# k2kobayashi/crank

Hardware: AMD Instinct MI355X
Metric: train frames/sec (higher is better)
Workload: dtype bf16; 1 GPU; vqvae trainer step (all sub-updates), VCC2020-shaped synthetic 80-dim mlfb, 64 utterances x 500 frames per GPU, 14 speakers; trainer=vqvae, global_batch=64, batch_len=500, parallelism=dp1

## Files before the change

crank_amd/_lib.py:

```python
import ctypes
import os
from .config import cfg
from ctypes import c_char_p, c_double, c_float, c_int, c_longlong, c_ulonglong, c_void_p

_HERE = os.path.dirname(os.path.abspath(__file__))
LIB_PATH = cfg.lib_path or os.path.join(_HERE, "libcrank_hip.so")
_lib = None

ERRORS = {1: "invalid argument", 2: "HIP runtime error", 3: "unsupported shape/configuration"}


class NetDesc(ctypes.Structure):
    _fields_ = [
        ("kind", c_int), ("in_ch", c_int), ("out_ch", c_int), ("kernel_size", c_int), ("layers", c_int),
        ("stacks", c_int), ("res_ch", c_int), ("gate_ch", c_int), ("skip_ch", c_int), ("aux_ch", c_int),
        ("conv_ch", c_int), ("causal", c_int), ("use_bias", c_int), ("slope", c_float), ("dropout", c_float),
    ]


COLLATE_MAX_STREAMS = 8


class CollateStream(ctypes.Structure):
    _fields_ = [("src", c_void_p), ("ld", c_int), ("col0", c_int), ("ncols", c_int), ("dst", c_void_p)]


class CollateDesc(ctypes.Structure):
    _fields_ = [
        ("n_streams", c_int), ("streams", CollateStream * COLLATE_MAX_STREAMS), ("utt_start", c_void_p),
        ("utt_spk", c_void_p), ("n_utt", c_int), ("n_spk", c_int), ("lcf0_raw", c_void_p),
        ("spk_lcf0_mean", c_void_p), ("spk_lcf0_std", c_void_p), ("raw", c_void_p), ("raw_start", c_void_p),
        ("fftl", c_int), ("hop", c_int),
    ]


P, I, LL, ULL, F, D = c_void_p, c_int, c_longlong, c_ulonglong, c_float, c_double

SIGNATURES = {
    "crk_net_create": (P, [ctypes.POINTER(NetDesc)]),
    "crk_net_destroy": (None, [P]),
    "crk_net_param_count": (LL, [P]),
    "crk_net_conv_count": (I, [P]),
    "crk_net_conv_info": (I, [P, I, ctypes.POINTER(c_longlong)]),
    "crk_net_saved_bytes": (LL, [P, I, I]),
    "crk_net_reserve": (I, [P, I, I]),
    "crk_net_scratch_bytes": (LL, [P, I, I]),
    "crk_debug_alloc_count": (LL, []),
    "crk_debug_net_paths": (I, [P, I, I]),
    "crk_seed_next": (I, [P, P, P]),
    "crk_nets_wnorm_bwd": (I, [I, P, P]),
    "crk_nets_prepare": (I, [I, P, P, ULL, P, P]),
    "crk_net_forward": (I, [P, P, ULL, P, I, P, I, P, I, P, I, I, I, ULL, P]),
    "crk_net_backward": (I, [P, P, ULL, P, P, I, P, I, P, I, P, I, F, P, I, P, I, I, I, ULL, P]),
    "crk_net_backward_scaled": (I, [P, P, ULL, P, P, I, P, I, P, I, P, I, F, P, I, P, I, I, I, ULL, P, P, P]),
    "crk_net_embed_grad_supported": (I, [P, I, I, I]),
    "crk_net_backward_embed": (I, [P, P, ULL, P, P, I, P, I, P, I, P, I, F, P, I, I, I, ULL, P, LL, I, I, I, P, P]),
    "crk_vq_forward": (I, [P, I, P, I, I, I, P, P, I, P, I, P]),
    "crk_vq_forward_fused": (I, [P, I, P, I, P, I, P, I, I, I, P, P, I, P, I, P, P, P, P, P]),
    "crk_vq_image_bytes": (LL, [I, I]),
    "crk_vq_image_build_multi": (I, [I, P, P, I, P, P]),
    "crk_vq_ema_scratch_bytes": (LL, [I, I, I]),
    "crk_vq_ema_stats": (I, [P, I, P, I, I, I, P, P, P, P]),
    "crk_vq_ema_apply": (I, [P, P, P, P, P, I, I, D, D, P]),
    "crk_vq_ema_partial": (I, [P, I, P, I, I, I, P, P]),
    "crk_vq_ema_reduce_multi": (I, [I, P, P, P, P, P, P, P]),
    "crk_vq_ema_apply_multi": (I, [I, P, P, P, P, P, P, P, D, D, P]),
    "crk_vq_ema_partial_multi": (I, [I, P, P, P, P, P, P, P, P]),
    "crk_vq_ema_reduce_size_multi": (I, [I, P, P, P, P, P, P, P, D, D, P]),
    "crk_vq_ema_blend_multi": (I, [I, P, P, P, P, P, P, D, P]),
    "crk_vq_ema_blend_image_multi": (I, [I, P, P, P, P, P, P, D, P, P]),
    "crk_stft_loss_multi_fwd": (I, [P, I, P, I, I, I, I, I, P, P, P, P, F, P, P, P]),
    "crk_stft_loss_multi_fwd_grad": (I, [P, I, P, I, I, I, I, I, P, P, P, P, F, P, P, I, P, P]),
    "crk_stft_loss_multi_bwd": (I, [P, I, P, I, I, I, I, I, P, P, P, P, F, P, P, I, P]),
    "crk_loss_scratch_floats": (I, []),
    "crk_masked_loss_fwd": (I, [P, I, P, I, F, P, LL, I, I, P, P, P]),
    "crk_masked_loss_bwd": (I, [P, I, P, I, F, P, LL, I, I, P, P, P, I, P, I, P]),
    "crk_masked_loss_both_fwd": (I, [P, I, P, I, P, LL, I, P, P, P]),
    "crk_weighted_sum": (I, [I, P, P, F, P, P]),
    "crk_weighted_sum_bwd": (I, [I, P, P, P, P]),
    "crk_recon_supported": (I, [I, I, P, P, P]),
    "crk_stft_twiddle_floats": (LL, [I, I]),
    "crk_stft_twiddles": (I, [I, I, P, P, P]),
    "crk_recon_grad_floats": (LL, [I, I, I, I, P, P]),
    "crk_recon_loss_fwd": (I, [P, I, P, I, P, I, I, I, I, P, P, P, P, F, P, P, P, P]),
    "crk_recon_loss_bwd": (I, [P, I, P, I, P, I, I, I, I, P, P, P, P, P, P, P, P, P, I, P]),
    "crk_masked_loss_bwd_acc": (I, [P, I, P, I, F, P, LL, I, I, P, P, P, I, P, I, P, I, P, P]),
    "crk_vq_commit_bwd": (I, [P, I, P, I, P, LL, I, P, P, P, I, P, I, P, I, P, I, P, I, P]),
    "crk_ce_fwd": (I, [P, I, P, LL, I, I, P, P, P, P]),
    "crk_ce_bwd": (I, [P, LL, I, P, P, P, P]),
    "crk_stft_loss_fwd": (I, [P, I, P, I, I, I, I, I, I, I, P, F, F, I, P, P, P]),
    "crk_stft_loss_bwd": (I, [P, I, P, I, I, I, I, I, I, I, P, F, F, P, P, I, P]),
    "crk_adam_step": (I, [P, P, P, P, LL, P, P, F, F, F, I, P]),
    "crk_radam_step": (I, [P, P, P, P, LL, P, P, D, D, D, I, P]),
    "crk_lamb_step": (I, [P, P, P, P, P, P, I, P, I, P, P, P, P, D, D, D, I, P]),
    "crk_lamb_tile": (I, []),
    "crk_concat_embed": (I, [P, I, I, P, I, I, P, I, P, LL, P, I, P]),
    "crk_embed_bwd_scratch_floats": (LL, [LL, I, I]),
    "crk_embed_bwd": (I, [P, I, I, I, P, LL, I, P, P, P]),
    "crk_concat_embed_run": (I, [P, I, I, P, I, I, P, I, P, LL, LL, P, I, P]),
    "crk_embed_bwd_run": (I, [P, I, I, I, P, LL, LL, I, P, P, P]),
    "crk_logmel_fwd": (I, [P, I, I, I, I, I, I, I, P, P, I, F, P, P, P, I, I, P]),
    "crk_scaler_apply": (I, [P, I, P, I, LL, I, P, P, I, P]),
    "crk_scaler_workspace_bytes": (LL, [I, I]),
    "crk_scaler_moments": (I, [P, I, I, I, LL, P, P, I, P, LL, P]),
    "crk_scaler_merge": (I, [P, LL, I, I, P, P, P, P, I, P, P, P, P]),
    "crk_collate_batch": (I, [ctypes.POINTER(CollateDesc), P, I, I, P, P, P, P, P, P, P, P, P]),
    "crk_decode_f0": (I, [P, P, I, I, P, P, D, D, I, P, P, P, P, P, P]),
    "crk_mcd_scratch_bytes": (LL, [I, I, I, I, I]),
    "crk_mcd_fastdtw": (I, [P, P, P, P, I, I, I, I, I, P, P, P, LL, P, P, P]),
    "crk_voc_create": (P, [I, I, I, I, P, I, P]),
    "crk_voc_destroy": (None, [P]),
    "crk_voc_workspace_bytes": (LL, [P, I, I]),
    "crk_voc_forward": (I, [P, P, P, I, I, P, P, P, LL, I, P]),
    "crk_voc_upsample": (I, [P, P, P, I, I, P, P, LL, P]),
    "crk_world_create": (P, [I, I, D, D, I, I, I]),
    "crk_world_destroy": (None, [P]),
    "crk_world_reserve": (I, [P, LL]),
    "crk_world_workspace_bytes": (LL, [P, I, LL, LL]),
    "crk_world_synthesis": (I, [P, P, P, P, P, I, I, P, P, I, LL, LL, LL, P, P, P, LL, P]),
    "crk_world_frames": (I, [P, P, P, P, I, I, LL, P, P, P, LL, P]),
    "crk_world_pulses": (I, [P, P, P, P, I, P, P, P, P, P]),
    "crk_wana_create": (P, [I, I, D, D, I]),
    "crk_wana_destroy": (None, [P]),
    "crk_wana_reserve": (I, [P, LL]),
    "crk_wana_workspace_bytes": (LL, [I, LL, LL]),
    "crk_wana_lowcut": (I, [P, P, P, I, P, I, LL, P, P]),
    "crk_wana_lowcut_tile": (I, []),
    "crk_wana_cheaptrick": (I, [P, P, P, P, P, I, LL, LL, LL, P, P, LL, P]),
    "crk_wana_mcep": (I, [P, P, P, P, P, I, LL, LL, LL, I, P, P, P, LL, P]),
    "crk_wana_npow": (I, [P, P, P, I, LL, P, P, LL, P]),
    "crk_wana_frame_shapes": (I, [P, P, P, I, LL, P, P, P]),
    "crk_f0_create": (P, [I, I, P]),
    "crk_f0_destroy": (None, [P]),
    "crk_f0_reserve": (I, [P, LL]),
    "crk_f0_workspace_bytes": (LL, [I, LL, LL, LL]),
    "crk_f0_harvest": (I, [P, P, P, P, P, P, I, LL, LL, LL, LL, LL, P, P, P, LL, P]),
    "crk_f0_decimate": (I, [P, P, P, I, LL, P, P, LL, P]),
    "crk_f0_raw_candidates": (I, [P, P, P, P, P, P, I, LL, LL, LL, P, P, P, LL, P]),
    "crk_f0_candidates": (I, [P, P, P, I, LL, P, P, LL, P]),
    "crk_f0_refine": (I, [P, P, P, P, P, I, LL, P, P, P]),
    "crk_f0_contour": (I, [P, P, P, P, I, LL, P, P, LL, P]),
    "crk_f0_continuous": (I, [P, P, I, LL, P, P, P, P, P, P, P]),
    "crk_gl_create": (I, [I, I, I, I, I, P, ctypes.POINTER(c_void_p)]),
    "crk_gl_destroy": (None, [P]),
    "crk_gl_workspace_bytes": (LL, [I, LL, LL]),
    "crk_gl_linear_spectrum": (I, [P, P, LL, I, P, P]),
    "crk_gl_run": (I, [P, P, P, P, P, I, LL, LL, I, I, P, P, LL, P]),
    "crk_gl_stft": (I, [P, P, P, P, I, LL, LL, P, P]),
    "crk_gl_istft": (I, [P, P, P, P, I, LL, LL, P, P, LL, P]),
    "crk_prof_enable": (I, [I]),
    "crk_prof_report": (I, [I, ctypes.POINTER(c_longlong), ctypes.POINTER(c_double), ctypes.POINTER(c_double)]),
    "crk_prof_report_bytes": (I, [I, ctypes.POINTER(c_double)]),
    "crk_debug_vq_set_f16": (I, [I]),
    "crk_debug_flush_before": (I, [c_longlong]),
    "crk_debug_vq_flags": (I, [ctypes.POINTER(c_ulonglong), I]),
    "crk_version": (c_char_p, []),
}


def lib():
    global _lib
    if _lib is None:
        if not os.path.exists(LIB_PATH):
            raise RuntimeError(
                f"{LIB_PATH} is missing: build it with `python -c 'import __graft_entry__ as g; g.build()'` "
                "(or `make -C crank_amd/csrc`).  crank_amd has no fallback compute path."
            )
        cdll = ctypes.CDLL(LIB_PATH)
        for name, (res, args) in SIGNATURES.items():
            fn = getattr(cdll, name)
            fn.restype = res
            fn.argtypes = args
        _lib = cdll
    return _lib


def check(rc, what):
    if rc != 0:
        raise RuntimeError(f"libcrank_hip: {what} failed: {ERRORS.get(rc, rc)}")


_raw_stream = None


def stream_ptr():
    global _raw_stream
    if _raw_stream is None:
        import torch

        get_stream = getattr(torch._C, "_cuda_getCurrentRawStream", None)
        get_dev = getattr(torch._C, "_cuda_getDevice", None)
        if get_stream is not None and get_dev is not None:
            _raw_stream = lambda: get_stream(get_dev())
        else:
            _raw_stream = lambda: torch.cuda.current_stream().cuda_stream
    return _raw_stream()


def ptr(t):
    return 0 if t is None else t.data_ptr()
```

crank_amd/config.py:

```python
import contextlib
import os
import types

_get = os.environ.get


def _flag(name, default):
    v = _get(name)
    return default if v is None else v not in ("0", "")


def _read():
    return types.SimpleNamespace(
        precision=_get("CRANK_AMD_PRECISION", "bf16"),
        lib_path=_get("CRANK_AMD_LIB") or None,
        default_yaml=_get("CRANK_DEFAULT_YAML") or None,
        overlap_c=int(_get("CRANK_AMD_OVERLAP_C", "1") or 0),
        separate_ce=_flag("CRANK_AMD_SEPARATE_CE", False),
        separate_commit=_flag("CRANK_AMD_SEPARATE_COMMIT", False),
        recon_dense=_flag("CRANK_AMD_RECON_DENSE", False),
        stft_two_pass=_flag("CRANK_AMD_STFT_TWO_PASS", False),
        cond_sums=_flag("CRANK_AMD_COND_SUMS", True),
        force_dist=_flag("CRANK_AMD_FORCE_DIST", False),
        dist_backend=_get("CRANK_AMD_DIST_BACKEND") or None,
        dp_graph_collectives=_flag("CRANK_AMD_DP_GRAPH_COLLECTIVES", True),
        capture_mode=_get("CRANK_AMD_CAPTURE_MODE", "thread_local"),
        test_refuse_capture_rank=_get("CRANK_AMD_TEST_REFUSE_CAPTURE_RANK"),
    )


cfg = _read()


def reload():
    cfg.__dict__.update(_read().__dict__)


def torchrun():
    r = _get("RANK")
    return (None if r is None else int(r)), int(_get("LOCAL_RANK", "0")), int(_get("WORLD_SIZE", "1"))


@contextlib.contextmanager
def override(**kw):
    unknown = [k for k in kw if not hasattr(cfg, k)]
    if unknown:
        raise AttributeError(f"unknown switch(es): {unknown}")
    old = {k: getattr(cfg, k) for k in kw}
    cfg.__dict__.update(kw)
    try:
        yield cfg
    finally:
        cfg.__dict__.update(old)
```

crank_amd/csrc/conv_kernels.h:

```cpp
#pragma once
#include <vector>

#include "common.h"
#include "switches.h"

#define CRK_TM 128

enum { MODE_PLAIN = 0, MODE_RESFWD = 1, MODE_BWDA = 2 };

struct ConvP {
  const float* xa; int lda; int cinA; float scaleA;
  const float* xb; int ldb; int cinB; float scaleB;
  int act_in; float slope;
  float drop_p; unsigned long long drop_seed;
  const unsigned long long* drop_seed_ptr;
  int cin, cin_pad;
  const float* xc; int ldc; int cinC; int cinC_pad;
  const uint16_t* w_hi; const uint16_t* w_lo;
  const uint16_t* wc_hi; const uint16_t* wc_lo;
  const uint16_t* w2_hi; const uint16_t* w2_lo;
  const float* bias; const float* bias2a; const float* bias2b;
  int cout, cout_pad, ktaps, dil, off0;
  int B, T, tiles_per_utt;
  float* y; int ldy; int accumulate; int act_out; float out_scale;
  const float* dmask; int ldm; int dmask_act;
  const float* res; int ldr; float res_scale;
  float epi_drop_p; unsigned long long epi_drop_seed;
  float* skip; int skip_init; float* sv_ta; float* sv_sb; float* sv_z;
  const float* ta; const float* sb;
  int xs_stride, cs_stride, ws_stride, zs_stride;
  int o_xlo, o_chi, o_clo, o_whi, o_wlo, o_zhi, o_zlo;
  int lds_bytes;
  int dbg;
};

struct WgradP {
  const float* a1; int lda1; int ca1; float sa1;
  const float* a2; int lda2; int ca2; float sa2;
  int ca, ca_pad;
  const float* x; int ldx; int cx; int cx_pad; float sx; int act_in; float slope;
  float drop_p; unsigned long long drop_seed; const unsigned long long* drop_seed_ptr;
  const float* xc; int ldc; int cc; int cc_pad; int has_aux;
  int ktaps, dil, off0;
  int B, T;
  float* partial;
  float* partial_aux;
  float* bias_partial;
  int grp_tap0, grp_ntap, grp_aux;
  int cpg, ngroups;
  int dbg;
};

struct ConvEntry {
  int cout, cin, k;
  long long off_g, off_v, off_b;
  long long fw_off; int fw_rows, fw_kp, fw_row0;
  long long bw_off; int bw_rows, bw_kp, bw_col0;
  long long pt_off; int pt_rows, pt_row0, pt_cx, pt_taps, pt_tap0; float pt_scale;
  int pt_groups;
  long long pb_off;
  long long norm_off;
  long long fr_off; int fr_mode;
  long long bfr_off; int bfr_mode;
};

struct StackLayer {
  long long f_conv, f_aux, f_os;
  long long w_conv, w_aux, w_os;
  long long b_conv, b_out, b_skip;
  int dil, off0;
};
struct StackP {
  const float* x0;
  const float* c; int ldc; int aux_ch, aux_pad;
  float* saved;
  uint16_t *xb_hi, *xb_lo;
  uint16_t *zb_hi, *zb_lo;
  uint16_t *tb_hi, *tb_lo, *sg_hi, *sg_lo;
  uint16_t *cb_hi, *cb_lo;
  float* skip;
  const float* params;
  const uint16_t* whi; const uint16_t* wlo;
  const StackLayer* layers;
  int B, T, L, ktaps;
  int hl, hr, max_off;
  int tmo, tiles_per_utt;
  float drop_p; unsigned long long drop_seed; const unsigned long long* drop_seed_ptr;
  int o_xlo, o_zhi, o_zlo, o_chi, o_clo, o_whi, o_wlo, o_bias, o_tab, w_bytes, lds_bytes;
  int nw;
  int dbg;
  int ft, fh;
  int ft1;
  int o_zs, o_cs;
  int o_xf;
  const float* x_in; int ldx_in, in_ch, kp_first;
  long long f_first, b_first;
  long long f_h1, b_h1, f_h2, b_h2;
  float* y; int ldy, out_ch; float head_scale;
  uint16_t* fin_hi; uint16_t* head_hi;
  long long ts_stride;
  int cs_stride;
};
struct PsLayer {
  long long w_off;
  long long b_off;
  int rows, rows_pad;
  int kp;
  int k, dil, off0;
  int epi;
  int mask_w;
  long long mask_plane;
  long long save_plane;
  long long f_off;
};
struct PsP {
  const float* x; int ldx, cin; float in_scale; int in_act;
  float* y; int ldy; float out_scale;
  const float* params; const uint16_t *whi, *wlo;
  uint16_t *save_hi, *save_lo;
  const uint16_t* mask_hi;
  const PsLayer* layers; int L;
  int tail;
  int B, T; float slope;
  int hl, hr, tmo, tiles_per_utt, nw, os;
  int o_olo, o_whi, o_wlo, o_bias, o_tab, w_bytes, lds_bytes;
  double algo_bytes;
  int os_b;
  const float* in_num; const float* in_den;
  long long l0_f_off, l0_save_plane; int l0_k, l0_kp, l0_rows_pad;
};
struct PwLayer {
  long long a_hi, a_lo;
  long long b_hi, b_lo;
  int wa, wb;
  int ca, cb;
  int k, dil, off0;
  long long pt, pb;
};
#define CRK_MAX_NETS_PW 8
struct PwP {
  const PwLayer* layers;
  const uint16_t* abase;
  const uint16_t* bbase;
  float* partials;
  int B, T, cpg, G;
};
struct PwMP { PwP q[CRK_MAX_NETS_PW]; int first[CRK_MAX_NETS_PW + 1]; int n; };
int launch_pstack_wgrad_multi(const PwMP& m, int total_layers, int max_G, int max_wa, int max_wb, int max_tiles, double flops,
                              double bytes, hipStream_t s);
int pstack_wgrad_supported(int ca, int cb, int wa, int wb, int k, int dil);
int launch_pstack_wgrad(const PwP& p, int nlayers, int max_wa, int max_wb, bool precise, double flops, hipStream_t s, int max_tiles = 0);
int pstack_plan(PsP& p, const PsLayer* host_layers, bool precise);
int launch_pstack(const PsP& p, bool precise, double flops, hipStream_t s);
int pstack2_plan(PsP& p, const PsLayer* host_layers);
int launch_pstack2(const PsP& p, double flops, hipStream_t s);
int pstack2x_plan(PsP& p, const PsLayer* host_layers);
int launch_pstack2x(const PsP& p, double flops, hipStream_t s);

struct StackBLayer {
  long long w_os, w_conv, w_aux;
  int dil, off0;
  long long f_os, f_conv, f_aux;
};
struct StackBP {
  const float* dS;
  const float* saved;
  const uint16_t *tb_hi, *tb_lo, *sg_hi, *sg_lo;
  float* dX0;
  uint16_t *gb_hi, *gb_lo;
  uint16_t *dxb_hi, *dxb_lo;
  uint16_t *dsb_hi, *dsb_lo;
  float* dc; int lddc; int aux_ch;
  const uint16_t* whi; const uint16_t* wlo;
  const StackBLayer* layers;
  int B, T, L, ktaps;
  int hl, hr, max_off;
  int tmo, tiles_per_utt;
  float drop_p; unsigned long long drop_seed; const unsigned long long* drop_seed_ptr;
  int mask_l0; float slope;
  int o_glo, o_whi, o_wlo, w_bytes, lds_bytes, nw;
  const float* dy; int lddy, out_ch, kp_y;
  long long w_h2, w_h1, w_first;
  const uint16_t* hmask_hi;
  uint16_t* hb_hi;
  float head_scale;
  float* dx; int lddx, in_ch, in_rows; float dx_scale;
  long long f_h2, f_h1, f_first;
  int ft, o_dx, o_tab;
  long long ts_stride;
  int rec;
  int dbg;
};
struct StackWLayer {
  long long pt_conv, pb_conv, pt_os, pb_os, pt_aux;
  int dil, off0;
};
struct StackWP {
  const uint16_t *xb_hi, *xb_lo, *zb_hi, *zb_lo, *cb_hi, *cb_lo;
  const uint16_t *gb_hi, *gb_lo, *dxb_hi, *dxb_lo, *dsb_hi, *dsb_lo;
  const StackWLayer* layers;
  float* partials;
  int B, T, L, ktaps, aux_ch, aux_pad, cpg, G;
  int rec_g;
  float* usums; int nseg;
};
int stack_wgrad_supported(int ktaps, int max_dil, int aux_ch);
int launch_stack_wgrad(const StackWP& p, bool precise, hipStream_t s);
struct CondEmbedP {
  const float* usums; int nseg, cpg;
  const uint16_t *whi, *wlo;
  const StackBLayer* layers;
  const long long* idx; long long run;
  int B, T, L, c0, E, n_rows;
  float* dtable;
};
int launch_cond_embed_bwd(const CondEmbedP& p, hipStream_t s);
int stack_bwd_plan(StackBP& p, bool precise);
int stack2_bwd_plan(StackBP& p);
int launch_stack2_bwd(const StackBP& p, hipStream_t s);
int stack_bwd_waves(bool precise);
int launch_stack_bwd(const StackBP& p, bool precise, hipStream_t s);
int stack_fwd_plan(StackP& p, bool precise);
int launch_stack_fwd(const StackP& p, bool precise, hipStream_t s);
int stack2_fwd_plan(StackP& p);
int launch_stack2_fwd(const StackP& p, hipStream_t s);
int stack2x_fwd_plan(StackP& p);
int launch_stack2x_fwd(const StackP& p, hipStream_t s);
#define CRK_PROF_CLASSES 9
void conv_prof_begin(int cls, double flops, hipStream_t s);
void conv_prof_end(int cls, hipStream_t s);
void conv_prof_bytes(int cls, double bytes);

void conv_fill_lds(ConvP& p, int mode, bool precise);
int launch_conv(const ConvP& p, int mode, bool precise, hipStream_t s);
int wgrad_expand(const WgradP& job, bool precise, std::vector<WgradP>& out);
int launch_wgrad_table(const WgradP* d_jobs, const std::vector<WgradP>& h_jobs, int B, int T, int max_groups, bool precise,
                       hipStream_t s);
#define CRK_MAX_NETS 8
struct NetRef {
  const ConvEntry* ents; const float* params; float* grads; const float* partials; float* norms;
  uint16_t *whi, *wlo;
  int n_ents, first;
};
struct NetRefs { NetRef r[CRK_MAX_NETS]; int n; float* bump; };
int launch_weight_prep_multi(const NetRefs& R, int total_entries, int nmax, hipStream_t s);
int launch_step_bump(float* step, hipStream_t s);
int launch_wnorm_bwd_multi(const NetRefs& R, int total_entries, hipStream_t s);
int launch_weight_prep(const ConvEntry* d_entries, int n_entries, int nmax, const float* params, uint16_t* wprep_hi,
                       uint16_t* wprep_lo, float* norms, hipStream_t s);
int launch_wnorm_bwd(const ConvEntry* d_entries, int n_entries, const float* params, float* grads,
                     const float* partials, const float* norms, hipStream_t s);
int conv_kernels_init();
```

crank_amd/csrc/conv_kernels.hip:

```cpp
#include "conv_kernels.h"

#include <vector>

static inline int al16(int x) { return (x + 15) & ~15; }

static int sw_int(const char* name, int dflt) { const char* e = getenv(name); return e ? atoi(e) : dflt; }
const CrkSwitches& crk_sw() {
  static const CrkSwitches s = [] {
    CrkSwitches v;
    v.sk_v = sw_int("CRK_SK_V", 2); v.skb_v = sw_int("CRK_SKB_V", 2); v.ps_v = sw_int("CRK_PS_V", 2);
    v.no_fuse = sw_int("CRK_NO_FUSE", 0); v.s2x = sw_int("CRK_S2X", 1); v.disc_split = sw_int("CRK_DISC_SPLIT", 1);
    v.s2_cfg = sw_int("CRK_S2_CFG", 0);
    const int nw = sw_int("CRK_SK_NW", 0);
    v.sk_nw_fwd = nw > 10 ? nw / 10 : nw; v.sk_nw_bwd = nw > 10 ? nw % 10 : nw;
    v.ps_nw = sw_int("CRK_PS_NW", 0);
    v.wg_groups = sw_int("CRK_WG_GROUPS", 32); if (v.wg_groups < 1) v.wg_groups = 32;
    v.wg_cpg = sw_int("CRK_WG_CPG", 0); v.wg_fill = sw_int("CRK_WG_FILL", 1) != 0;
    v.vq_f16 = sw_int("CRK_VQ_F16", 1) != 0; v.vq_lc = sw_int("CRK_VQ_LC", 2); v.logmel_wave = sw_int("CRK_LOGMEL_WAVE", 1);
    return v;
  }();
  return s;
}

struct ProfClass {
// ... 570 lines not shown
    const int l = wgrad_entry_lds(e, precise);
    if (l > lds) lds = l;
    fl += 2.0 * (double)B * T * e.ca * (e.grp_aux ? (double)e.cc : (double)e.cx * e.grp_ntap);
  }
  static bool attr_set = false;
  if (!attr_set) {
    if (hipFuncSetAttribute((const void*)wgrad_kernel<true>, hipFuncAttributeMaxDynamicSharedMemorySize, 152 * 1024) != hipSuccess ||
        hipFuncSetAttribute((const void*)wgrad_kernel<false>, hipFuncAttributeMaxDynamicSharedMemorySize, 152 * 1024) != hipSuccess)
      return CRK_ERR_HIP;
    attr_set = true;
  }
  dim3 grid(max_groups, (unsigned)h_jobs.size()), block(256);
  prof_begin(3, fl, s);
  if (precise) hipLaunchKernelGGL(wgrad_kernel<true>, grid, block, lds, s, d_jobs, B, T);
  else hipLaunchKernelGGL(wgrad_kernel<false>, grid, block, lds, s, d_jobs, B, T);
  prof_end(3, s);
  CRK_CHECK_LAUNCH();
  return CRK_OK;
}

__device__ __forceinline__ float wave_sum(float v) {
#pragma unroll
  for (int o = 32; o > 0; o >>= 1) v += __shfl_xor(v, o, 64);
  return v;
}

#define WP_BAND 16
typedef unsigned wp_u32x4 __attribute__((ext_vector_type(4)));
template <int BAND = WP_BAND>
__device__ __forceinline__ void weight_prep_band(const ConvEntry& e, int band, const float* params, uint16_t* whi,
                                                 uint16_t* wlo, float* norms, unsigned* ws) {
  const int co0 = band * BAND;
  if (co0 >= e.cout) return;
  const int nrow = e.cout - co0 < BAND ? e.cout - co0 : BAND;
  const int k = e.k, cin = e.cin, n = cin * k;
  const int tid = threadIdx.x, lane = tid & 63, wave = tid >> 6;
  {
    const float* v0 = params + e.off_v + (long long)co0 * n;
    const int tot = nrow * n;
    constexpr int WPQ = 28;
    for (int i0 = 0; i0 < tot; i0 += 256 * WPQ) {
      float t[WPQ];
#pragma unroll
      for (int u = 0; u < WPQ; u++) { const int i = i0 + u * 256 + tid; t[u] = i < tot ? v0[i] : 0.f; }
#pragma unroll
      for (int u = 0; u < WPQ; u++) { const int i = i0 + u * 256 + tid; if (i < tot) ws[i] = __builtin_bit_cast(unsigned, t[u]); }
    }
  }
  float gv[BAND / 4];
#pragma unroll
  for (int q = 0; q < BAND / 4; q++) { const int r = wave + 4 * q; gv[q] = r < nrow ? params[e.off_g + co0 + r] : 0.f; }
  __syncthreads();
#pragma unroll
  for (int q = 0; q < BAND / 4; q++) {
    const int r = wave + 4 * q;
    if (r < nrow) {
      unsigned* row = ws + r * n;
      float ss = 0.f;
      for (int i = lane; i < n; i += 64) { const float x = __builtin_bit_cast(float, row[i]); ss += x * x; }
      ss = wave_sum(ss);
      const float nrm = sqrtf(ss);
      if (lane == 0) norms[e.norm_off + co0 + r] = nrm;
      const float sc = gv[q] / nrm;
      for (int i = lane; i < n; i += 64) {
        const float w = __builtin_bit_cast(float, row[i]) * sc;
        uint16_t h, l;
        split_bf(w, h, l);
        row[i] = (unsigned)h | ((unsigned)l << 16);
      }
    }
  }
  __syncthreads();
  {
    const int nc8 = e.fw_kp >> 3, per_tap = nrow * nc8, total = k * per_tap;
    const float i_pt = 1.f / (float)per_tap, i_nc = 1.f / (float)nc8;
    for (int pidx = tid; pidx < total; pidx += 256) {
      const int tap = (int)(((float)pidx + 0.5f) * i_pt), rem = pidx - tap * per_tap;
      const int r = (int)(((float)rem + 0.5f) * i_nc), c8 = rem - r * nc8;
      const int co = co0 + r, ci0 = c8 * 8;
      unsigned wv[8];
#pragma unroll
      for (int j = 0; j < 8; j++) wv[j] = ci0 + j < cin ? ws[r * n + (ci0 + j) * k + tap] : 0u;
      const wp_u32x4 hp = {(wv[0] & 0xffffu) | (wv[1] << 16), (wv[2] & 0xffffu) | (wv[3] << 16), (wv[4] & 0xffffu) | (wv[5] << 16),
                           (wv[6] & 0xffffu) | (wv[7] << 16)};
      const wp_u32x4 lp = {(wv[0] >> 16) | (wv[1] & 0xffff0000u), (wv[2] >> 16) | (wv[3] & 0xffff0000u),
                           (wv[4] >> 16) | (wv[5] & 0xffff0000u), (wv[6] >> 16) | (wv[7] & 0xffff0000u)};
      const long long fi = e.fw_off + ((long long)tap * e.fw_rows + e.fw_row0 + co) * e.fw_kp + ci0;
      *reinterpret_cast<wp_u32x4*>(whi + fi) = hp;
      *reinterpret_cast<wp_u32x4*>(wlo + fi) = lp;
      if (e.fr_mode) {
        const int kc = ci0 >> 4, lh = 32 * ((ci0 & 15) >> 3);
        long long fo;
        if (e.fr_mode == 6) fo = ((((long long)(co >> 5) * k + tap) * (e.fw_kp >> 4) + kc) * 64 + (co & 31) + lh) * 8;
        else if (e.fr_mode == 5) fo = ((((long long)tap * (e.fw_rows >> 5) + (co >> 5)) * (e.fw_kp >> 4) + kc) * 64 + (co & 31) + lh) * 8;
        else {
          int mt, row;
          if (e.fr_mode <= 2) { const int hc = co & 63; mt = hc >> 4; row = (hc & 15) + (co >= 64 ? 16 : 0); }
          else { mt = (co >> 5) + (e.fr_mode == 4 ? 2 : 0); row = co & 31; }
          const int tp = e.fr_mode == 1 ? tap : 0;
          fo = ((((long long)tp * 4 + mt) * 4 + kc) * 64 + row + lh) * 8;
        }
        *reinterpret_cast<wp_u32x4*>(whi + e.fr_off + fo) = hp;
        *reinterpret_cast<wp_u32x4*>(wlo + e.fr_off + fo) = lp;
      }
    }
  }
  if (e.bw_off >= 0) {
    const int ext = ((e.cout + 15) & ~15) - co0;
    const int no8 = ((co0 + BAND >= e.cout) ? ext : (ext < BAND ? ext : BAND)) >> 3;
    const int per_tap = cin * no8, total = k * per_tap;
    const float i_pt = 1.f / (float)per_tap, i_no = 1.f / (float)no8;
    for (int pidx = tid; pidx < total; pidx += 256) {
      const int tap = (int)(((float)pidx + 0.5f) * i_pt), rem = pidx - tap * per_tap;
      const int ci = (int)(((float)rem + 0.5f) * i_no), o8 = rem - ci * no8;
      unsigned wv[8];
#pragma unroll
      for (int j = 0; j < 8; j++) wv[j] = o8 * 8 + j < nrow ? ws[(o8 * 8 + j) * n + ci * k + tap] : 0u;
      const wp_u32x4 hp = {(wv[0] & 0xffffu) | (wv[1] << 16), (wv[2] & 0xffffu) | (wv[3] << 16), (wv[4] & 0xffffu) | (wv[5] << 16),
                           (wv[6] & 0xffffu) | (wv[7] << 16)};
      const wp_u32x4 lp = {(wv[0] >> 16) | (wv[1] & 0xffff0000u), (wv[2] >> 16) | (wv[3] & 0xffff0000u),
                           (wv[4] >> 16) | (wv[5] & 0xffff0000u), (wv[6] >> 16) | (wv[7] & 0xffff0000u)};
      const int kcol = e.bw_col0 + co0 + o8 * 8, tf = k - 1 - tap;
      const long long bi = e.bw_off + ((long long)tf * e.bw_rows + ci) * e.bw_kp + kcol;
      *reinterpret_cast<wp_u32x4*>(whi + bi) = hp;
      *reinterpret_cast<wp_u32x4*>(wlo + bi) = lp;
      if (e.bfr_off >= 0) {
        const int ln = (ci & 31) + 32 * ((kcol & 15) >> 3);
        const long long fo = e.bfr_mode == 1
            ? ((((long long)(ci >> 5) * k + tf) * (e.bw_kp >> 4) + (kcol >> 4)) * 64 + ln) * 8
            : ((((long long)tf * (e.bw_rows >> 5) + (ci >> 5)) * (e.bw_kp >> 4) + (kcol >> 4)) * 64 + ln) * 8;
        *reinterpret_cast<wp_u32x4*>(whi + e.bfr_off + fo) = hp;
      }
    }
  }
}

__global__ __launch_bounds__(256) void weight_prep_kernel(const ConvEntry* ents, const float* params, uint16_t* whi,
                                                          uint16_t* wlo, float* norms) {
  extern __shared__ unsigned wp_ws[];
  const ConvEntry e = ents[blockIdx.x];
  weight_prep_band(e, blockIdx.y, params, whi, wlo, norms, wp_ws);
}

__device__ __forceinline__ int net_of_block(const NetRefs& R, int bx) {
  int r = 0;
  while (r + 1 < R.n && bx >= R.r[r + 1].first) r++;
  return r;
}
template <int BAND>
__global__ __launch_bounds__(256) void weight_prep_multi_kernel(const NetRefs R) {
  extern __shared__ unsigned wp_ws[];
  const NetRef& q = R.r[net_of_block(R, blockIdx.x)];
  const ConvEntry e = q.ents[blockIdx.x - q.first];
  if (R.bump && blockIdx.x == 0 && blockIdx.y == 0 && threadIdx.x == 0) R.bump[0] += 1.f;
  weight_prep_band<BAND>(e, blockIdx.y, q.params, q.whi, q.wlo, q.norms, wp_ws);
}
__global__ void step_bump_kernel(float* step) { step[0] += 1.f; }
int launch_step_bump(float* step, hipStream_t s) {
  hipLaunchKernelGGL(step_bump_kernel, dim3(1), dim3(1), 0, s, step);
  CRK_CHECK_LAUNCH();
  return CRK_OK;
}
static int wp_set_lds(const void* fn, size_t lds) {
  if (lds > 64 * 1024 && hipFuncSetAttribute(fn, hipFuncAttributeMaxDynamicSharedMemorySize, 160 * 1024) != hipSuccess) return CRK_ERR_HIP;
  return CRK_OK;
}
int launch_weight_prep_multi(const NetRefs& R, int total_entries, int nmax, hipStream_t s) {
  const size_t lds = (size_t)WP_BAND * nmax * 4;
  if (lds > 160 * 1024) return CRK_ERR_UNSUPPORTED;
  if (total_entries <= 16) {
    if (wp_set_lds((const void*)weight_prep_multi_kernel<8>, lds / 2) != CRK_OK) return CRK_ERR_HIP;
    hipLaunchKernelGGL(weight_prep_multi_kernel<8>, dim3(total_entries, 128 / 8), dim3(256), lds / 2, s, R);
    CRK_CHECK_LAUNCH();
    return CRK_OK;
  }
  if (wp_set_lds((const void*)weight_prep_multi_kernel<WP_BAND>, lds) != CRK_OK) return CRK_ERR_HIP;
  hipLaunchKernelGGL(weight_prep_multi_kernel<WP_BAND>, dim3(total_entries, 128 / WP_BAND), dim3(256), lds, s, R);
  CRK_CHECK_LAUNCH();
  return CRK_OK;
}

int launch_weight_prep(const ConvEntry* d_entries, int n_entries, int nmax, const float* params, uint16_t* wprep_hi,
                       uint16_t* wprep_lo, float* norms, hipStream_t s) {
  const size_t lds = (size_t)WP_BAND * nmax * 4;
  if (lds > 160 * 1024) return CRK_ERR_UNSUPPORTED;
  if (wp_set_lds((const void*)weight_prep_kernel, lds) != CRK_OK) return CRK_ERR_HIP;
  dim3 grid(n_entries, 128 / WP_BAND), block(256);
  hipLaunchKernelGGL(weight_prep_kernel, grid, block, lds, s, d_entries, params, wprep_hi, wprep_lo, norms);
  CRK_CHECK_LAUNCH();
  return CRK_OK;
}

#ifndef WN_RB
#define WN_RB 8
#endif
#ifndef WN_IF
#define WN_IF 16
#endif
template <int RB> struct WnormShared { float dw[RB][128 * 8]; };
template <int RB, int IF>
__device__ __forceinline__ void wnorm_bwd_body(const ConvEntry& e, int band, const float* params, float* grads,
                                               const float* partials, const float* norms, WnormShared<RB>& sh) {
  const int co0 = band * RB;
  if (co0 >= e.cout) return;
  const int nrow = e.cout - co0 < RB ? e.cout - co0 : RB;
  const int G = e.pt_groups, k = e.k, cin = e.cin, cx = e.pt_cx;
  const int n = cin * k;
  const int tid = threadIdx.x;
  const long long gstride = (long long)e.pt_taps * e.pt_rows * e.pt_cx;
  const long long tstride = (long long)e.pt_rows * e.pt_cx;
  const float* base = partials + e.pt_off + (long long)(e.pt_row0 + co0) * cx;
  const int r = tid >> 5, l32 = tid & 31;
  const bool on = r < nrow;
  const int co = co0 + r;
  const float* __restrict__ v = params + e.off_v + (long long)co * n;
  float* __restrict__ gv = grads + e.off_v + (long long)co * n;
  constexpr int WN_PV = (128 * 8) / 32;
  float vr[WN_PV], go[WN_PV];
#pragma unroll
  for (int q = 0; q < WN_PV; q++) {
    const int i = l32 + 32 * q;
    const bool ok = on && i < n;
    vr[q] = ok ? v[i] : 0.f;
    go[q] = ok ? gv[i] : 0.f;
  }
  float sb = 0.f;
  if (on && e.off_b >= 0)
    for (int g = l32; g < e.pt_groups; g += 32) sb += partials[e.pb_off + (long long)g * e.pt_rows + e.pt_row0 + co];
  const float nrm = on ? norms[e.norm_off + co] : 1.f;
  const float gval = on ? params[e.off_g + co] : 0.f;
  const float g_old = (on && l32 == 0) ? grads[e.off_g + co] : 0.f;
  const float b_old = (on && l32 == 0 && e.off_b >= 0) ? grads[e.off_b + co] : 0.f;
  const int run = nrow * cx;
  if ((cx & 3) == 0 && ((((uintptr_t)base) & 15) == 0) && ((gstride | tstride) & 3) == 0) {
    const int run4 = run >> 2;
    for (int it = tid; it < k * run4; it += 256) {
      const int tap = it / run4, i4 = it - tap * run4;
      const float* src = base + tap * tstride + 4 * i4;
      f32x4 s4 = {0.f, 0.f, 0.f, 0.f};
      int g = 0;
      for (; g + IF <= G; g += IF) {
        f32x4 t[IF];
#pragma unroll
        for (int u = 0; u < IF; u++) t[u] = *reinterpret_cast<const f32x4*>(src + (long long)(g + u) * gstride);
#pragma unroll
        for (int u = 0; u < IF; u++) s4 += t[u];
      }
      if (IF > 16) {
        for (; g + 16 <= G; g += 16) {
          f32x4 t[16];
#pragma unroll
          for (int u = 0; u < 16; u++) t[u] = *reinterpret_cast<const f32x4*>(src + (long long)(g + u) * gstride);
#pragma unroll
          for (int u = 0; u < 16; u++) s4 += t[u];
        }
      }
      for (; g + 4 <= G; g += 4) {
        f32x4 t[4];
#pragma unroll
        for (int u = 0; u < 4; u++) t[u] = *reinterpret_cast<const f32x4*>(src + (long long)(g + u) * gstride);
#pragma unroll
        for (int u = 0; u < 4; u++) s4 += t[u];
      }
      for (; g < G; g++) s4 += *reinterpret_cast<const f32x4*>(src + (long long)g * gstride);
      const int r = (4 * i4) / cx, ci = 4 * i4 - r * cx;
#pragma unroll
      for (int j = 0; j < 4; j++) sh.dw[r][(ci + j) * k + tap] = s4[j] * e.pt_scale;
    }
  } else {
    for (int tap = 0; tap < k; tap++) {
      for (int i = tid; i < run; i += 256) {
        const float* src = base + tap * tstride + i;
        float sv = 0.f;
        int g = 0;
        for (; g + 8 <= G; g += 8) {
          float t[8];
#pragma unroll
          for (int u = 0; u < 8; u++) t[u] = src[(long long)(g + u) * gstride];
#pragma unroll
          for (int u = 0; u < 8; u++) sv += t[u];
        }
        for (; g < G; g++) sv += src[(long long)g * gstride];
        const int r = i / cx, ci = i - r * cx;
        sh.dw[r][ci * k + tap] = sv * e.pt_scale;
      }
    }
  }
  __syncthreads();
  float dot = 0.f;
#pragma unroll
  for (int q = 0; q < WN_PV; q++) {
    const int i = l32 + 32 * q;
    if (on && i < n) dot += sh.dw[r][i] * vr[q];
  }
#pragma unroll
  for (int o = 16; o > 0; o >>= 1) { dot += __shfl_xor(dot, o, 64); sb += __shfl_xor(sb, o, 64); }
  if (on) {
    const float inv = 1.f / nrm;
    if (l32 == 0) {
      grads[e.off_g + co] = g_old + dot * inv;
      if (e.off_b >= 0) grads[e.off_b + co] = b_old + sb * e.pt_scale;
    }
    const float c1 = gval * inv, c2 = dot * inv * inv;
#pragma unroll
    for (int q = 0; q < WN_PV; q++) {
      const int i = l32 + 32 * q;
      if (i < n) gv[i] = go[q] + c1 * (sh.dw[r][i] - c2 * vr[q]);
    }
  }
}

__global__ __launch_bounds__(256) void wnorm_bwd_kernel(const ConvEntry* ents, const float* params, float* grads,
// ... 29 lines not shown
```

crank_amd/csrc/loss_kernels.hip:

```cpp
#include <algorithm>
#include <type_traits>

#include "common.h"

__device__ __forceinline__ float block_sum_256(float v, float* sh) {
#pragma unroll
  for (int o = 32; o > 0; o >>= 1) v += __shfl_xor(v, o, 64);
  const int tid = threadIdx.x;
  __syncthreads();
  if ((tid & 63) == 0) sh[tid >> 6] = v;
  __syncthreads();
  return sh[0] + sh[1] + sh[2] + sh[3];
}

template <int NC>
__device__ __forceinline__ void sum_partials(const float* part, int stride, int n, float (&s)[NC], float* sh) {
#pragma unroll
  for (int j = 0; j < NC; j++) s[j] = 0.f;
  for (int i = threadIdx.x; i < n; i += 256) {
#pragma unroll
    for (int j = 0; j < NC; j++) s[j] += part[stride * i + j];
  }
#pragma unroll
  for (int j = 0; j < NC; j++) s[j] = block_sum_256(s[j], sh);
// ... 913 lines not shown
  CRK_CHECK_LAUNCH();
  return CRK_OK;
}

struct ReconBRes { const float* gc; int hop, lo, span, nf; };
struct ReconBP {
  const float* x; const float* y; const unsigned char* mask;
  int ldx, ldy, T, D, nres;
  long N;
  const float* stat; const float* g1; const float* g2; const float* g3;
  float* dx; int lddx;
  ReconBRes r[LOSS_MAX_RES];
};
template <int V>
__global__ __launch_bounds__(256) void recon_bwd_kernel(const ReconBP p) {
  const float g1 = p.g1 ? p.g1[0] / p.stat[1] : 0.f;
  const float g2 = p.g2 ? p.g2[0] / p.stat[3] : 0.f;
  const float g3 = p.g3 ? p.g3[0] : 0.f;
  const int DV = p.D / V;
  const long total = p.N * DV;
  for (long i = (long)blockIdx.x * 256 + threadIdx.x; i < total; i += (long)gridDim.x * 256) {
    const long n = i / DV;
    const int d = (int)(i - n * DV) * V;
    const int b = (int)(n / p.T), t = (int)(n - (long)b * p.T);
    float v[V];
#pragma unroll
    for (int j = 0; j < V; j++) v[j] = 0.f;
    if (p.g3) {
#pragma unroll
      for (int k = 0; k < LOSS_MAX_RES; k++) {
        if (k >= p.nres) break;
        const ReconBRes& r = p.r[k];
        const int u = t + r.lo, fr = u / r.hop, off = u - fr * r.hop;
        if (off < r.span && fr < r.nf) {
          const float* gp = r.gc + ((size_t)((long)b * r.nf + fr) * r.span + off) * p.D + d;
          if (V == 4) {
            const float4 a = *reinterpret_cast<const float4*>(gp);
            v[0] += a.x * g3; v[1 % V] += a.y * g3; v[2 % V] += a.z * g3; v[3 % V] += a.w * g3;
          } else {
            v[0] += gp[0] * g3;
          }
        }
      }
    }
    if (!p.mask || p.mask[n]) {
      float xv[V], yv[V];
      if (V == 4) {
        const float4 a = *reinterpret_cast<const float4*>(p.x + n * p.ldx + d);
        const float4 c = *reinterpret_cast<const float4*>(p.y + n * p.ldy + d);
        xv[0] = a.x; xv[1 % V] = a.y; xv[2 % V] = a.z; xv[3 % V] = a.w;
        yv[0] = c.x; yv[1 % V] = c.y; yv[2 % V] = c.z; yv[3 % V] = c.w;
      } else {
        xv[0] = p.x[n * p.ldx + d]; yv[0] = p.y[n * p.ldy + d];
      }
#pragma unroll
      for (int j = 0; j < V; j++) {
        const float df = xv[j] - yv[j];
        if (p.g1) v[j] += df > 0.f ? g1 : (df < 0.f ? -g1 : 0.f);
        if (p.g2) v[j] += 2.f * df * g2;
      }
    }
    if (V == 4) *reinterpret_cast<float4*>(p.dx + n * p.lddx + d) = make_float4(v[0], v[1 % V], v[2 % V], v[3 % V]);
    else p.dx[n * p.lddx + d] = v[0];
  }
}

extern "C" int crk_recon_loss_bwd(const float* x, int ldx, const float* y, int ldy, const unsigned char* mask, int B, int T,
                                  int D, int nres, const int* n_fft, const int* hop_length, const int* win_length,
                                  const float* out5, const float* grad, const float* g1, const float* g2, const float* g3,
                                  float* dx, int lddx, void* stream) {
  if (!x || !y || !out5 || !dx || B < 1 || T < 1 || D < 1) return CRK_ERR_ARG;
  if (g3 && (!grad || !crk_recon_supported(T, nres, n_fft, hop_length, win_length))) return CRK_ERR_ARG;
  ReconBP p;
  p.x = x; p.y = y; p.mask = mask; p.ldx = ldx; p.ldy = ldy; p.T = T; p.D = D; p.nres = g3 ? nres : 0;
  p.N = (long)B * T; p.stat = out5; p.g1 = g1; p.g2 = g2; p.g3 = g3; p.dx = dx; p.lddx = lddx;
  const float* g = grad;
  for (int r = 0; r < p.nres; r++) {
    ReconBRes& q = p.r[r];
    q.hop = hop_length[r]; q.span = win_length[r] + RC_SPAN_EXTRA; q.nf = 1 + T / q.hop;
    q.lo = n_fft[r] / 2 - (n_fft[r] - win_length[r]) / 2 + 1;
    q.gc = g;
    g += (size_t)B * q.nf * q.span * D;
  }
  const bool v4 = !((((uintptr_t)x) | ((uintptr_t)y) | ((uintptr_t)dx) | ((uintptr_t)grad)) & 15) && !((D | ldx | ldy | lddx) & 3);
  if (v4) hipLaunchKernelGGL(recon_bwd_kernel<4>, dim3(loss_blocks(p.N * (D / 4))), dim3(256), 0, (hipStream_t)stream, p);
  else hipLaunchKernelGGL(recon_bwd_kernel<1>, dim3(loss_blocks(p.N * D)), dim3(256), 0, (hipStream_t)stream, p);
  CRK_CHECK_LAUNCH();
  return CRK_OK;
}

#define WS_MAX 16
struct WsumP { const float* t[WS_MAX]; float w[WS_MAX]; int n; float c; float* out; const float* g; };
__global__ void weighted_sum_kernel(const WsumP p) {
  float s = 0.f;
#pragma unroll
  for (int i = 0; i < WS_MAX; i++)
    if (i < p.n) s += p.w[i] * p.t[i][0];
  p.out[0] = s + p.c;
}
__global__ void weighted_sum_bwd_kernel(const WsumP p) {
  const float g = p.g[0];
#pragma unroll
  for (int i = 0; i < WS_MAX; i++)
    if (i < p.n) p.out[i] = p.w[i] * g;
}
extern "C" int crk_weighted_sum(int n, const float* const* terms, const float* weights, float constant, float* out, void* stream) {
  if (n < 1 || n > WS_MAX || !terms || !weights || !out) return CRK_ERR_ARG;
  WsumP p{};
  for (int i = 0; i < n; i++) { if (!terms[i]) return CRK_ERR_ARG; p.t[i] = terms[i]; p.w[i] = weights[i]; }
  p.n = n; p.c = constant; p.out = out;
  hipLaunchKernelGGL(weighted_sum_kernel, dim3(1), dim3(1), 0, (hipStream_t)stream, p);
  CRK_CHECK_LAUNCH();
  return CRK_OK;
}
extern "C" int crk_weighted_sum_bwd(int n, const float* weights, const float* gout, float* grads, void* stream) {
  if (n < 1 || n > WS_MAX || !weights || !gout || !grads) return CRK_ERR_ARG;
  WsumP p{};
  for (int i = 0; i < n; i++) p.w[i] = weights[i];
  p.n = n; p.g = gout; p.out = grads;
  hipLaunchKernelGGL(weighted_sum_bwd_kernel, dim3(1), dim3(1), 0, (hipStream_t)stream, p);
  CRK_CHECK_LAUNCH();
  return CRK_OK;
}

template <bool CLEAR>
__global__ __launch_bounds__(256) void adam_kernel(float* __restrict__ p, float* __restrict__ g,
                                                   float* __restrict__ m, float* __restrict__ v, long n,
                                                   const float* __restrict__ lr_dev, float* __restrict__ step_dev,
                                                   float beta1, float beta2, float eps) {
  const AdamCoef c = adam_coef(lr_dev, step_dev, beta1, beta2, eps);
  for (long i = (long)blockIdx.x * 256 + threadIdx.x; i < n; i += (long)gridDim.x * 256) adam_elem<CLEAR>(p, g, m, v, i, c);
}

__global__ void adam_bump_kernel(float* step_dev) { step_dev[0] += 1.f; }

extern "C" int crk_adam_step(float* params, float* grads, float* exp_avg, float* exp_avg_sq, long long n,
                             const float* lr_dev, float* step_dev, float beta1, float beta2, float eps, int clear_grads,
                             void* stream) {
  if (!params || !grads || !exp_avg || !exp_avg_sq || !lr_dev || !step_dev) return CRK_ERR_ARG;
  hipStream_t s = (hipStream_t)stream;
  long b = (n + 255) / 256;
  if (b > 2048) b = 2048;
  if (clear_grads & 1)
    hipLaunchKernelGGL(adam_kernel<true>, dim3((int)b), dim3(256), 0, s, params, grads, exp_avg, exp_avg_sq, (long)n, lr_dev,
                       step_dev, beta1, beta2, eps);
  else
    hipLaunchKernelGGL(adam_kernel<false>, dim3((int)b), dim3(256), 0, s, params, grads, exp_avg, exp_avg_sq, (long)n, lr_dev,
                       step_dev, beta1, beta2, eps);
  if (!(clear_grads & 2)) hipLaunchKernelGGL(adam_bump_kernel, dim3(1), dim3(1), 0, s, step_dev);
  CRK_CHECK_LAUNCH();
  return CRK_OK;
}

struct RAdamCoef { float step_size; bool rect; };
__device__ __forceinline__ RAdamCoef radam_coef(const float* lr_dev, const float* step_dev, double b1, double b2) {
  const double t = (double)step_dev[0] + 1.0;
  const double b2t = pow(b2, t), bc1 = 1.0 - pow(b1, t);
  const double nmax = 2.0 / (1.0 - b2) - 1.0;
  const double nsma = nmax - 2.0 * t * b2t / (1.0 - b2t);
  RAdamCoef c;
  c.rect = nsma >= 5.0;
  const double lr = (double)lr_dev[0];
  c.step_size = (float)(c.rect ? lr * sqrt((1.0 - b2t) * (nsma - 4.0) / (nmax - 4.0) * (nsma - 2.0) / nsma * nmax / (nmax - 2.0)) / bc1
                               : lr / bc1);
  return c;
}
struct MomentCoef { float b1, omb1, b2, omb2, eps; };
static MomentCoef moment_coef(double beta1, double beta2, double eps) {
  MomentCoef k;
  k.b1 = (float)beta1; k.omb1 = (float)(1.0 - beta1); k.b2 = (float)beta2; k.omb2 = (float)(1.0 - beta2); k.eps = (float)eps;
  return k;
}
template <bool CLEAR>
__global__ __launch_bounds__(256) void radam_kernel(float* __restrict__ p, float* __restrict__ g, float* __restrict__ m,
                                                    float* __restrict__ v, long n, const float* __restrict__ lr_dev,
                                                    float* __restrict__ step_dev, double beta1, double beta2, MomentCoef k) {
#pragma clang fp contract(off)
  const RAdamCoef c = radam_coef(lr_dev, step_dev, beta1, beta2);
  for (long i = (long)blockIdx.x * 256 + threadIdx.x; i < n; i += (long)gridDim.x * 256) {
    const float gi = g[i];
    if (CLEAR) g[i] = 0.f;
    const float vi = v[i] * k.b2 + k.omb2 * gi * gi;
    const float mi = m[i] * k.b1 + k.omb1 * gi;
    v[i] = vi; m[i] = mi;
    if (c.rect) p[i] -= c.step_size * (mi / (sqrtf(vi) + k.eps));
    else p[i] -= c.step_size * mi;
  }
}

extern "C" int crk_radam_step(float* params, float* grads, float* exp_avg, float* exp_avg_sq, long long n,
                              const float* lr_dev, float* step_dev, double beta1, double beta2, double eps, int clear_grads,
                              void* stream) {
  if (!params || !grads || !exp_avg || !exp_avg_sq || !lr_dev || !step_dev) return CRK_ERR_ARG;
  hipStream_t s = (hipStream_t)stream;
  long b = (n + 255) / 256;
  if (b > 2048) b = 2048;
  if (b < 1) b = 1;
  const MomentCoef k = moment_coef(beta1, beta2, eps);
  if (clear_grads & 1)
    hipLaunchKernelGGL(radam_kernel<true>, dim3((int)b), dim3(256), 0, s, params, grads, exp_avg, exp_avg_sq, (long)n, lr_dev,
                       step_dev, beta1, beta2, k);
  else
    hipLaunchKernelGGL(radam_kernel<false>, dim3((int)b), dim3(256), 0, s, params, grads, exp_avg, exp_avg_sq, (long)n, lr_dev,
                       step_dev, beta1, beta2, k);
  if (!(clear_grads & 2)) hipLaunchKernelGGL(adam_bump_kernel, dim3(1), dim3(1), 0, s, step_dev);
  CRK_CHECK_LAUNCH();
  return CRK_OK;
}

#define LAMB_TILE 2048
__global__ __launch_bounds__(256) void lamb_moments_kernel(const float* __restrict__ p, float* __restrict__ g,
                                                           float* __restrict__ m, float* __restrict__ v,
                                                           float* __restrict__ upd, const int4* __restrict__ tiles,
                                                           float* __restrict__ part, MomentCoef k, int clear) {
#pragma clang fp contract(off)
  __shared__ float sh[4];
  const int4 tl = tiles[blockIdx.x];
  float sw = 0.f, su = 0.f;
  for (int j = threadIdx.x; j < tl.y; j += 256) {
    const long i = (long)tl.x + j;
    const float gi = g[i];
    if (clear) g[i] = 0.f;
    const float mi = m[i] * k.b1 + k.omb1 * gi;
    const float vi = v[i] * k.b2 + k.omb2 * gi * gi;
    m[i] = mi; v[i] = vi;
    const float u = mi / (sqrtf(vi) + k.eps);
    upd[i] = u;
    const float w = p[i];
    sw += w * w; su += u * u;
  }
  sw = block_sum_256(sw, sh);
  su = block_sum_256(su, sh);
  if (threadIdx.x == 0) { part[2 * blockIdx.x] = sw; part[2 * blockIdx.x + 1] = su; }
}

__global__ __launch_bounds__(256) void lamb_apply_kernel(float* __restrict__ p, const float* __restrict__ upd,
                                                         const int4* __restrict__ tiles, const int2* __restrict__ tensors,
                                                         const float* __restrict__ part, const float* __restrict__ lr_dev,
                                                         float* __restrict__ ratio_out) {
#pragma clang fp contract(off)
  __shared__ float sr;
  const int4 tl = tiles[blockIdx.x];
  if (threadIdx.x == 0) {
    const int2 ts = tensors[tl.z];
    double sw = 0.0, su = 0.0;
    for (int t = ts.x; t < ts.x + ts.y; t++) { sw += (double)part[2 * t]; su += (double)part[2 * t + 1]; }
    const float wn = fminf((float)sqrt(sw), 10.f), un = (float)sqrt(su);
    const float r = (wn == 0.f || un == 0.f) ? 1.f : wn / un;
    sr = r;
    if (ratio_out && blockIdx.x == ts.x) ratio_out[tl.z] = r;
  }
  __syncthreads();
  const float sc = lr_dev[0] * sr;
  for (int j = threadIdx.x; j < tl.y; j += 256) {
    const long i = (long)tl.x + j;
    p[i] -= sc * upd[i];
  }
}

extern "C" int crk_lamb_step(float* params, float* grads, float* exp_avg, float* exp_avg_sq, float* upd, const int* tiles,
                             int n_tiles, const int* tensors, int n_tensors, float* part, float* ratio_out,
                             const float* lr_dev, float* step_dev, double beta1, double beta2, double eps, int clear_grads,
                             void* stream) {
  if (!params || !grads || !exp_avg || !exp_avg_sq || !upd || !tiles || !tensors || !part || !lr_dev || !step_dev ||
      n_tiles < 0 || n_tensors < 0)
    return CRK_ERR_ARG;
  hipStream_t s = (hipStream_t)stream;
  if (n_tiles > 0) {
    hipLaunchKernelGGL(lamb_moments_kernel, dim3(n_tiles), dim3(256), 0, s, params, grads, exp_avg, exp_avg_sq, upd,
                       reinterpret_cast<const int4*>(tiles), part, moment_coef(beta1, beta2, eps), clear_grads & 1);
    hipLaunchKernelGGL(lamb_apply_kernel, dim3(n_tiles), dim3(256), 0, s, params, upd, reinterpret_cast<const int4*>(tiles),
                       reinterpret_cast<const int2*>(tensors), part, lr_dev, ratio_out);
  }
  if (!(clear_grads & 2)) hipLaunchKernelGGL(adam_bump_kernel, dim3(1), dim3(1), 0, s, step_dev);
  CRK_CHECK_LAUNCH();
  return CRK_OK;
}
extern "C" int crk_lamb_tile() { return LAMB_TILE; }

__global__ __launch_bounds__(256) void concat_embed_kernel(const float* __restrict__ a, int lda, int ca,
                                                           const float* __restrict__ b2, int ldb, int cb2,
                                                           const float* __restrict__ table, int E,
                                                           const long long* __restrict__ idx, long run, long N,
                                                           float* __restrict__ out, int ldo) {
  const int C = ca + cb2 + E;
  const long total = N * C;
  for (long i = (long)blockIdx.x * 256 + threadIdx.x; i < total; i += (long)gridDim.x * 256) {
    const long n = i / C;
    const int c = (int)(i - n * C);
    float v;
    if (c < ca) v = a[n * lda + c];
    else if (c < ca + cb2) v = b2[n * ldb + (c - ca)];
    else v = table[idx[run > 1 ? n - n % run : n] * E + (c - ca - cb2)];
    out[n * ldo + c] = v;
  }
}

extern "C" int crk_concat_embed_run(const float* a, int lda, int ca, const float* b, int ldb, int cb, const float* table,
                                    int E, const long long* idx, long long run, long long N, float* out, int ldo,
                                    void* stream) {
  if (!out || run < 1 || (ca > 0 && !a) || (cb > 0 && !b) || (E > 0 && (!table || !idx))) return CRK_ERR_ARG;
  const long total = N * (ca + cb + E);
  hipLaunchKernelGGL(concat_embed_kernel, dim3(loss_blocks(total)), dim3(256), 0, (hipStream_t)stream, a, lda, ca, b, ldb,
                     cb, table, E, idx, (long)run, (long)N, out, ldo);
  CRK_CHECK_LAUNCH();
  return CRK_OK;
// ... 91 lines not shown
```

crank_amd/csrc/net.hip:

```cpp
#include <math.h>
#include <stdlib.h>
#include <string.h>

#include <deque>
#include <vector>

#include "conv_kernels.h"

struct crk_net_desc {
  int kind;
  int in_ch, out_ch, kernel_size, layers, stacks;
  int res_ch, gate_ch, skip_ch, aux_ch;
  int conv_ch;
  int causal;
  int use_bias;
  float slope;
  float dropout;
};

enum { ROLE_FIRST = 0, ROLE_CONV = 1, ROLE_AUX = 2, ROLE_OUT = 3, ROLE_SKIP = 4, ROLE_LAST1 = 5, ROLE_LAST2 = 6, ROLE_PLAIN = 7 };

struct ConvMeta {
  int role, layer, dilation;
};
// ... 782 lines not shown
    p.sv_ta = a.saved + lay.ta + l * P; p.sv_sb = a.saved + lay.sb + l * P; p.sv_z = a.saved + lay.z + l * P;
    RUN(conv_go(p, MODE_RESFWD, k.precise, a.s));
  }
  ConvP h1 = conv_fw(n, a.B, a.T, n->ents[n->idx_last1], a.params, SKIP, 64, H1, 64);
  h1.scaleA = (float)sqrt(1.0 / L); h1.act_in = head_act;
  RUN(conv_go(h1, MODE_PLAIN, k.precise, a.s));
  ConvP h2 = conv_fw(n, a.B, a.T, n->ents[n->idx_last2], a.params, H1, 64, a.y, a.ldy);
  h2.act_in = head_act;
  return conv_go(h2, MODE_PLAIN, k.precise, a.s);
}
extern "C" int crk_net_forward(void* h, const float* params, unsigned long long version, const float* x, int ldx,
                               const float* c, int ldc, float* y, int ldy, float* saved, int B, int T, int flags,
                               unsigned long long seed, void* stream) {
  Net* n = (Net*)h;
  if (!n || !params || !x || !y || B <= 0 || T <= 0) return CRK_ERR_ARG;
  const FwdIo a = {.params = params, .x = x, .ldx = ldx, .c = c, .ldc = ldc, .y = y, .ldy = ldy, .saved = saved, .B = B, .T = T,
                   .s = (hipStream_t)stream};
  const Call k = call_facts(flags, seed, true, x, ldx, y, ldy, nullptr, nullptr);
  const Shape* r = find_shape(n, B, T);
  if (!r) return not_reserved("crk_net_forward");
  const Route& rt = r->route[k.precise];
  const bool x3f = k.mode == 2 && r->route[0].x3f;
  RUN(ensure_prepared(n, params, version, a.s));
  tag_forward(n, saved, B, T, k, x3f);
  if (n->d.kind != 2 && (!saved || (n->d.aux_ch > 0 && !c))) return CRK_ERR_ARG;
  int form;
  RUN(fwd_form(n, rt, k, x3f, &form));
  switch (form) {
    case FWD_CHAIN: return fwd_chain(n, r, k, a);
    case FWD_CHAIN_LAYERS: return fwd_chain_layers(n, k, a);
    case FWD_FOLDED: return fwd_folded(n, rt, k, a, x3f);
    case FWD_FUSED: return fwd_fused(n, r, k, a);
  }
  return fwd_layers(n, k, a);
}

static int stack_cpg(const Net* n, int B, int T) {
  const int ncpu = (T + 63) / 64;
  const int groups = crk_sw().wg_groups;
  const int gsz = (B + groups - 1) / groups;
  int cpg = gsz * ncpu;
  if (crk_sw().wg_fill && n->d.kind != 2 && n->L > 0 && 256 / n->L > groups) {
    const int fill = 256 / n->L;
    const int c = (B * ncpu + fill - 1) / fill;
    if (c >= 1 && c < cpg) cpg = c;
  }
  return cpg < 1 ? 1 : cpg;
}
static int stack_groups(const Net* n, int B, int T) {
  const int total = B * ((T + 63) / 64), cpg = stack_cpg(n, B, T);
  return (total + cpg - 1) / cpg;
}

static int usum_nseg(const Net* n, int B, int T) {
  const int ncpu = (T + 63) / 64;
  return (stack_cpg(n, B, T) + 2 * ncpu - 2) / ncpu;
}
static long long usum_floats(const Net* n, int B, int T) {
  if (n->d.kind == 2 || n->d.aux_ch <= 0) return 0;
  return (long long)stack_groups(n, B, T) * usum_nseg(n, B, T) * n->L * 128;
}
static long long usum_off(const Net* n, long long N) { return gated_f32(n, N).scratch_total + (gated_s16(n, N).total + 1) / 2; }
static ShapeNeed shape_need(const Net* n, int B, int T) {
  ShapeNeed q;
  const long long N = (long long)B * T;
  const long long cw = n->d.conv_ch > n->d.out_ch ? n->d.conv_ch : n->d.out_ch;
  q.need_s = n->d.kind == 2 ? (long long)n->L * N * cw + N * plain_gplanes_w(n)
                            : usum_off(n, N) + usum_floats(n, B, T);
  q.Gs = stack_groups(n, B, T); q.cpg_s = stack_cpg(n, B, T); q.nseg = usum_nseg(n, B, T);
  const int total_chunks = B * ((T + 63) / 64);
  const int groups = (n->d.kind == 2 && n->ents.size() <= 4) ? 64 : 32;
  q.cpg = (total_chunks + groups - 1) / groups;
  if (crk_sw().wg_cpg > 0) q.cpg = crk_sw().wg_cpg;
  q.Gg = (total_chunks + q.cpg - 1) / q.cpg;
  q.need_p = n->pt_floats_stack * q.Gs + n->pt_floats_gen * q.Gg;
  return q;
}
static int grow(Net* n, float** buf, long long* cap, long long need) {
  if (need <= *cap) return CRK_OK;
  if (*buf) n->retired.push_back(*buf);
  *buf = nullptr; *cap = 0;
  if (NET_MALLOC(buf, need * 4) != hipSuccess) return CRK_ERR_HIP;
  *cap = need;
  return CRK_OK;
}
static int build_shape(Net* n, Shape& r) {
  const crk_net_desc& d = n->d;
  r.abs = n->ents;
  for (auto& e : r.abs) {
    const bool stack = e.pt_groups != 0;
    const long long base = stack ? 0 : n->pt_floats_stack * r.q.Gs;
    const int G = stack ? r.q.Gs : r.q.Gg;
    e.pt_off = base + e.pt_off * G; e.pb_off = base + e.pb_off * G; e.pt_groups = G;
  }
  RUN(upload(&r.d_ents, r.abs.data(), r.abs.size()));
  if (n->L <= PS_MAXL) {
    ps_build(n, (long long)r.B * r.T, r.abs.data(), r.ps);
    RUN(upload(&r.d_ps, &r.ps.t[0][0], 4 * PS_MAXL));
    RUN(upload(&r.d_pw, r.ps.w, PS_MAXL));
  }
  if (d.kind != 2) {
    std::vector<StackWLayer> wt(n->L);
    for (int l = 0; l < n->L; l++) {
      const ConvEntry& ec = n->ents[n->idx_conv[l]];
      const ConvEntry& eo = n->ents[n->idx_out[l]];
      const ConvEntry& ac = r.abs[n->idx_conv[l]];
      const ConvEntry& ao = r.abs[n->idx_out[l]];
      StackWLayer& y = wt[l];
      y.pt_conv = ac.pt_off; y.pb_conv = ec.off_b >= 0 ? ac.pb_off : -1;
      y.pt_os = ao.pt_off; y.pb_os = eo.off_b >= 0 ? ao.pb_off : -1;
      y.pt_aux = d.aux_ch > 0 ? r.abs[n->idx_aux[l]].pt_off : 0;
      y.dil = n->meta[n->idx_conv[l]].dilation;
      y.off0 = fwd_off0(n, ec.k, y.dil);
    }
    RUN(upload(&r.d_wlayers, wt.data(), wt.size()));
  }
  return CRK_OK;
}
extern "C" int crk_net_reserve(void* h, int B, int T) {
  Net* n = (Net*)h;
  if (!n || B <= 0 || T <= 0) return CRK_ERR_ARG;
  if (find_shape(n, B, T)) return CRK_OK;
  AllocScope may_allocate;
  Shape r{};
  r.B = B; r.T = T; r.q = shape_need(n, B, T);
  r.route[0] = route_of(n, B, T, false);
  r.route[1] = route_of(n, B, T, true);
  RUN(grow(n, &n->scratch, &n->scratch_cap, r.q.need_s));
  RUN(grow(n, &n->partials, &n->partial_cap, r.q.need_p));
  if (!n->d_jobs && NET_MALLOC(&n->d_jobs, sizeof(WgradP) * 256) != hipSuccess) return CRK_ERR_HIP;
  const int rc = build_shape(n, r);
  if (rc != CRK_OK) {
    free_shape(r);
    return rc;
  }
  n->shapes.push_back(r);
  return CRK_OK;
}
extern "C" long long crk_net_scratch_bytes(void* h, int B, int T) {
  Net* n = (Net*)h;
  if (!n || B <= 0 || T <= 0) return -1;
  const ShapeNeed q = shape_need(n, B, T);
  return (q.need_s + q.need_p) * 4;
}
extern "C" long long crk_debug_alloc_count(void) { return g_net_allocs; }
long long crk_count_alloc_(void) { return ++g_net_allocs; }
extern "C" int crk_debug_net_paths(void* h, int B, int T) {
  Net* n = (Net*)h;
  if (!n || B <= 0 || T <= 0) return -1;
  const Route r = route_at(n, B, T, false);
  return (int)r.gen_split | (int)r.x3f << 1 | (int)r.disc_split << 2 | (int)(n->d.kind == 2 && r.fused) << 3;
}

static WgradP base_wgrad(const Net* n, int B, int T) {
  WgradP w;
  memset(&w, 0, sizeof(w));
  w.sa1 = w.sa2 = w.sx = 1.f; w.slope = n->d.slope;
  w.B = B; w.T = T; w.ktaps = 1; w.dil = 1; w.off0 = 0;
  w.dbg = 0;
  return w;
}
static void wgrad_slots(const Net* n, const Shape* r, int ei, WgradP& w) {
  const ConvEntry& a = r->abs[ei];
  const bool stack = n->ents[ei].pt_groups != 0;
  w.partial = n->partials + a.pt_off;
  w.bias_partial = a.off_b >= 0 ? n->partials + a.pb_off : nullptr;
  w.ngroups = a.pt_groups;
  w.cpg = stack ? r->q.cpg_s : r->q.cpg;
}
static int wgrad_go(Net* n, WgradP& w, bool precise) {
  w.ca_pad = pad32(w.ca); w.cx_pad = pad32(w.cx); w.cc_pad = w.has_aux ? pad32(w.cc) : 0;
  return wgrad_expand(w, precise, n->jobs);
}
static int wgrad_conv(Net* n, const Shape* r, int ei, const float* a1, int lda1, const float* x, int ldx, int act_in, float sx, bool precise) {
  const ConvEntry& e = n->ents[ei];
  WgradP w = base_wgrad(n, r->B, r->T);
  w.a1 = a1; w.lda1 = lda1; w.ca1 = e.cout; w.ca = e.cout;
  w.x = x; w.ldx = ldx; w.cx = e.cin; w.sx = sx; w.act_in = act_in;
  w.ktaps = e.k; w.dil = n->meta[ei].dilation; w.off0 = -((e.k - 1) / 2) * w.dil;
  wgrad_slots(n, r, ei, w);
  return wgrad_go(n, w, precise);
}
static int wgrad_flush(Net* n, int B, int T, bool precise, hipStream_t s) {
  if (n->jobs.empty()) return CRK_OK;
  if (n->jobs.size() > 256) return CRK_ERR_UNSUPPORTED;
  const int k = n->slot_next;
  n->slot_next = (k + 1) & 3;
  if (!n->h_slot[k]) {
    if (hipHostMalloc((void**)&n->h_slot[k], sizeof(WgradP) * 256, hipHostMallocDefault) != hipSuccess) return CRK_ERR_HIP;
    if (hipEventCreateWithFlags(&n->slot_ev[k], hipEventDisableTiming) != hipSuccess) return CRK_ERR_HIP;
  } else if (hipEventSynchronize(n->slot_ev[k]) != hipSuccess) {
    return CRK_ERR_HIP;
  }
  memcpy(n->h_slot[k], n->jobs.data(), sizeof(WgradP) * n->jobs.size());
  if (hipMemcpyAsync(n->d_jobs, n->h_slot[k], sizeof(WgradP) * n->jobs.size(), hipMemcpyHostToDevice, s) != hipSuccess)
    return CRK_ERR_HIP;
  if (hipEventRecord(n->slot_ev[k], s) != hipSuccess) return CRK_ERR_HIP;
  int mg = 0;
  for (const auto& j : n->jobs) if (j.ngroups > mg) mg = j.ngroups;
  int rc = launch_wgrad_table(n->d_jobs, n->jobs, B, T, mg, precise, s);
  n->jobs.clear();
  return rc;
}

static PwP plain_wgrad_params(const Net* n, const Shape* r, const uint16_t* abase, const uint16_t* bbase) {
  PwP wp; memset(&wp, 0, sizeof(wp));
  wp.layers = r->d_pw; wp.abase = abase; wp.bbase = bbase; wp.partials = n->partials;
  wp.B = r->B; wp.T = r->T; wp.cpg = r->q.cpg; wp.G = r->q.Gg;
  return wp;
}
static int launch_plain_wgrad(const Shape* r, const PwP& wp, bool precise, hipStream_t s) {
  const PsTables& Tb = r->ps;
  return launch_pstack_wgrad(wp, Tb.nw, Tb.max_wa, Tb.max_wb, precise, Tb.wflops_per_frame * r->B * r->T, s, Tb.max_tiles);
}
static int flush_pending_plain_wgrad(Net* n, hipStream_t s) {
  if (!n->pw_shape) return CRK_OK;
  const Shape* r = n->pw_shape;
  n->pw_shape = nullptr;
  return launch_plain_wgrad(r, n->pw_params, false, s);
}

struct CondEmbed { const long long* idx; long long run; int c0, E, n_rows; float* dtable; };
struct BwdIo {
  const float* params; float* grads; const float* x; int ldx; const float* c; int ldc; const float* dy; int lddy;
  float* dx; int lddx; float dx_scale; float* dc; int lddc; const float* saved; int B, T;
  const float* dy_num; const float* dy_den; const CondEmbed* ce; hipStream_t s;
};
enum { BWD_CHAIN, BWD_CHAIN_LAYERS, BWD_FOLDED_SPLIT, BWD_FOLDED, BWD_FUSED_SPLIT, BWD_FUSED, BWD_LAYERS };
static int bwd_form(const Net* n, const Route& rt, const Call& k, bool planes_precise, int* form) {
  if (n->d.kind == 2) { *form = rt.fused ? BWD_CHAIN : BWD_CHAIN_LAYERS; return CRK_OK; }
  if (!rt.fused) { *form = BWD_LAYERS; return CRK_OK; }
  const bool ok_x = k.out16 && (!k.want_dx || n->d.in_ch % 4 == 0);
  if (rt.gen_split && !planes_precise) {
    if (!k.in4 || !ok_x) {
      fprintf(stderr, "[crank_hip] crk_net_backward: dy / dx must be 16-byte aligned with row strides that are multiples of 4 floats\n");
      return CRK_ERR_ARG;
    }
    *form = BWD_FOLDED_SPLIT;
  } else if (rt.disc_split && !planes_precise) *form = BWD_FUSED_SPLIT;
  else *form = (rt.fold_bwd_fs && k.in16 && ok_x) ? BWD_FOLDED : BWD_FUSED;
  return CRK_OK;
}

static int bwd_chain(Net* n, const Shape* r, const Call& k, const BwdIo& a) {
  if (!a.saved) return CRK_ERR_ARG;
  const crk_net_desc& d = n->d;
  const PsTables& Tb = r->ps;
  const long long N = (long long)a.B * a.T;
  const long long cw = d.conv_ch > d.out_ch ? d.conv_ch : d.out_ch;
  const uint16_t* f16 = reinterpret_cast<const uint16_t*>(a.saved + saved_f32_floats(n, N));
  uint16_t* g16 = reinterpret_cast<uint16_t*>(n->scratch + (long long)n->L * N * cw);
  PsP p = ps_base(n, a.B, a.T, a.params);
  p.x = a.dy; p.ldx = a.lddy; p.cin = d.out_ch; p.y = a.dx; p.ldy = a.lddx; p.out_scale = a.dx_scale;
  p.in_num = a.dy_num; p.in_den = a.dy_den;
  p.save_hi = g16; p.save_lo = g16 + N * plain_gplanes_w(n); p.mask_hi = f16;
  p.layers = r->d_ps + PS_MAXL; p.L = Tb.L[1];
  if (!k.want_dx && p.L >= 2) { p.L -= 1; p.tail = 1; }
  if (r->route[k.precise].ps_bwd[p.tail] == CHAIN_PS2) {
    RUN(pstack2_plan(p, Tb.t[1]));
    RUN(launch_pstack2(p, ps_flops(Tb.t[1], p.L, N), a.s));
  } else RUN(pstack_go(r, 1, p, k.precise, a.s));
  if (k.want_w) RUN(launch_plain_wgrad(r, plain_wgrad_params(n, r, g16, f16), k.precise, a.s));
  return CRK_OK;
}
static int bwd_chain_layers(Net* n, const Shape* r, const Call& k, const BwdIo& a) {
  const crk_net_desc& d = n->d;
  const long long N = (long long)a.B * a.T;
  const long long cw = d.conv_ch > d.out_ch ? d.conv_ch : d.out_ch;
  const float* dcur = a.dy; int ldcur = a.lddy;
  for (int i = n->L - 1; i >= 0; i--) {
    const int ei = n->idx_plain[i];
    const ConvEntry& e = n->ents[ei];
    const int dil = n->meta[ei].dilation;
    const float* in = (i == 0) ? a.x : a.saved + (long long)(i - 1) * N * d.conv_ch;
    const int ldin = (i == 0) ? a.ldx : d.conv_ch;
    if (k.want_w) RUN(wgrad_conv(n, r, ei, dcur, ldcur, in, ldin, (i == 0) ? ACT_NONE : ACT_LRELU, 1.f, k.precise));
    if (i == 0 && !k.want_dx) break;
    float* out = i > 0 ? n->scratch + (long long)i * N * cw : a.dx;
    ConvP p = conv_bw(n, a.B, a.T, e, dcur, ldcur, out, i > 0 ? d.conv_ch : a.lddx);
    p.ktaps = e.k; p.dil = dil; p.off0 = -(-((e.k - 1) / 2) * dil) - (e.k - 1) * dil;
    if (i > 0) { p.dmask = in; p.ldm = ldin; p.dmask_act = ACT_LRELU; }
    else p.out_scale = a.dx_scale;
    RUN(conv_go(p, MODE_PLAIN, k.precise, a.s));
    dcur = out; ldcur = d.conv_ch;
  }
  return CRK_OK;
}

struct GatedPlanes { const uint16_t* f16; uint16_t* s16; GatedB16 gf; GatedS16 gs; };
static GatedPlanes gated_planes(const Net* n, const float* saved, long long N) {
  return {reinterpret_cast<const uint16_t*>(saved + saved_f32_floats(n, N)),
          reinterpret_cast<uint16_t*>(n->scratch + gated_f32(n, N).scratch_total), gated_b16(n, N), gated_s16(n, N)};
}
static int stack_bwd_params(const Net* n, const Call& k, const BwdIo& a, StackBP& bp) {
  const crk_net_desc& d = n->d;
  const long long N = (long long)a.B * a.T;
  const GatedF32 lay = gated_f32(n, N);
  const GatedPlanes q = gated_planes(n, a.saved, N);
  bp = stack_bwd_shape(n, a.B, a.T);
  bp.dS = n->scratch + lay.ds; bp.saved = a.saved; bp.dX0 = n->scratch + lay.dx;
  bp.tb_hi = q.f16 + q.gf.tb_hi; bp.tb_lo = q.f16 + q.gf.tb_lo; bp.sg_hi = q.f16 + q.gf.sg_hi; bp.sg_lo = q.f16 + q.gf.sg_lo;
  bp.gb_hi = q.s16 + q.gs.gb_hi; bp.gb_lo = q.s16 + q.gs.gb_lo; bp.dxb_hi = q.s16 + q.gs.dxb_hi; bp.dxb_lo = q.s16 + q.gs.dxb_lo;
  bp.dsb_hi = q.s16 + q.gs.dsb_hi; bp.dsb_lo = q.s16 + q.gs.dsb_lo;
  bp.dc = (k.want_dc && d.aux_ch > 0) ? a.dc : nullptr; bp.lddc = a.lddc;
  bp.whi = n->whi; bp.wlo = n->wlo; bp.layers = n->d_blayers;
  if (d.dropout > 0.f) { bp.drop_p = d.dropout; bp.drop_seed = k.seed_val; bp.drop_seed_ptr = k.seed_ptr; }
  bp.mask_l0 = d.kind == 1; bp.slope = d.slope;
  return stack_bwd_plan(bp, k.precise);
}
static int stack_bwd_go(const Net* n, const Shape* r, const Call& k, const BwdIo& a, StackBP& bp, bool split) {
  const long long N = (long long)a.B * a.T;
  if (split) { bp.ts_stride = ts_plane_stride(N); RUN(stack2_bwd_plan(bp)); }
  bp.rec = (split && N % 4 == 0) ? 1 : 0;
  if (split) RUN(launch_stack2_bwd(bp, a.s));
  else RUN(launch_stack_bwd(bp, k.precise, a.s));
  if (!k.want_w) return CRK_OK;
  const crk_net_desc& d = n->d;
  const GatedPlanes q = gated_planes(n, a.saved, N);
  StackWP wp;
  memset(&wp, 0, sizeof(wp));
  wp.xb_hi = q.f16 + q.gf.xb_hi; wp.xb_lo = q.f16 + q.gf.xb_lo; wp.zb_hi = q.f16 + q.gf.zb_hi; wp.zb_lo = q.f16 + q.gf.zb_lo;
  wp.aux_pad = stack_aux_pad(n);
  if (d.aux_ch > 0) { wp.cb_hi = q.f16 + q.gf.cb_hi; wp.cb_lo = q.f16 + q.gf.cb_lo; }
  wp.gb_hi = bp.gb_hi; wp.gb_lo = bp.gb_lo; wp.dxb_hi = bp.dxb_hi; wp.dxb_lo = bp.dxb_lo;
  wp.dsb_hi = bp.dsb_hi; wp.dsb_lo = bp.dsb_lo;
  wp.layers = r->d_wlayers; wp.partials = n->partials;
  wp.B = a.B; wp.T = a.T; wp.L = n->L; wp.ktaps = d.kernel_size; wp.aux_ch = d.aux_ch > 0 ? d.aux_ch : 0;
  wp.cpg = r->q.cpg_s; wp.G = r->q.Gs;
  wp.rec_g = bp.rec;
  if (a.ce) { wp.usums = n->scratch + usum_off(n, N); wp.nseg = r->q.nseg; }
  RUN(launch_stack_wgrad(wp, k.precise, a.s));
  if (!a.ce) return CRK_OK;
  CondEmbedP ep;
  memset(&ep, 0, sizeof(ep));
  ep.usums = wp.usums; ep.nseg = wp.nseg; ep.cpg = wp.cpg;
  ep.whi = n->whi; ep.wlo = k.precise ? n->wlo : nullptr; ep.layers = n->d_blayers;
  ep.idx = a.ce->idx; ep.run = a.ce->run;
  ep.B = a.B; ep.T = a.T; ep.L = n->L; ep.c0 = a.ce->c0; ep.E = a.ce->E; ep.n_rows = a.ce->n_rows; ep.dtable = a.ce->dtable;
  return launch_cond_embed_bwd(ep, a.s);
}
static int gated_plain_wgrad(Net* n, const Shape* r, const Call& k, const BwdIo& a) {
  if (!k.want_w) return CRK_OK;
  const GatedPlanes q = gated_planes(n, a.saved, (long long)a.B * a.T);
  const PwP wp = plain_wgrad_params(n, r, q.s16, q.f16);
  if (k.defer_wn && !k.precise) { n->pw_shape = r; n->pw_params = wp; return CRK_OK; }
  return launch_plain_wgrad(r, wp, k.precise, a.s);
}
static int bwd_folded(Net* n, const Shape* r, const Call& k, const BwdIo& a, bool split) {
  const crk_net_desc& d = n->d;
  const GatedPlanes q = gated_planes(n, a.saved, (long long)a.B * a.T);
  const ConvEntry& ef = n->ents[n->idx_first];
  const ConvEntry& e1 = n->ents[n->idx_last1];
  const ConvEntry& e2 = n->ents[n->idx_last2];
  StackBP bp;
  RUN(stack_bwd_params(n, k, a, bp));
  if (!split && bp.nw != 8) return CRK_ERR_UNSUPPORTED;
  bp.dy = a.dy; bp.lddy = a.lddy; bp.out_ch = d.out_ch; bp.kp_y = e2.bw_kp;
  bp.w_h2 = e2.bw_off; bp.w_h1 = e1.bw_off; bp.w_first = ef.bw_off;
  bp.hmask_hi = q.f16 + q.gf.head_hi; bp.hb_hi = q.s16 + q.gs.hb_hi; bp.head_scale = (float)sqrt(1.0 / n->L);
  bp.dx = a.dx; bp.lddx = a.lddx; bp.in_ch = d.in_ch; bp.in_rows = ef.bw_rows; bp.dx_scale = a.dx_scale;
  bp.f_h2 = e2.bfr_off; bp.f_h1 = e1.bfr_off; bp.f_first = ef.bfr_off;
  RUN(stack_bwd_go(n, r, k, a, bp, split));
  return gated_plain_wgrad(n, r, k, a);
}
static int bwd_fused(Net* n, const Shape* r, const Call& k, const BwdIo& a, bool split) {
  const long long N = (long long)a.B * a.T;
  const GatedF32 lay = gated_f32(n, N);
  const GatedPlanes q = gated_planes(n, a.saved, N);
  PsP h = ps_base(n, a.B, a.T, a.params);
  h.x = a.dy; h.ldx = a.lddy; h.cin = n->d.out_ch; h.y = n->scratch + lay.ds; h.ldy = 64; h.out_scale = (float)sqrt(1.0 / n->L);
  h.save_hi = q.s16 + q.gs.hb_hi; h.save_lo = q.s16 + q.gs.hb_lo;
  h.mask_hi = q.f16 + q.gf.head_hi; h.L = 2;
  RUN(pstack_go(r, 2, h, k.precise, a.s));
  StackBP bp;
  RUN(stack_bwd_params(n, k, a, bp));
  if (!bp.dS) return CRK_ERR_ARG;
  RUN(stack_bwd_go(n, r, k, a, bp, split));
  if (k.want_dx) {
    PsP p = ps_base(n, a.B, a.T, a.params);
    p.x = n->scratch + lay.dx; p.ldx = 64; p.cin = 64; p.y = a.dx; p.ldy = a.lddx; p.out_scale = a.dx_scale; p.L = 1;
    RUN(pstack_go(r, 3, p, k.precise, a.s));
  }
  return gated_plain_wgrad(n, r, k, a);
}
static int bwd_layers(Net* n, const Shape* r, const Call& k, const BwdIo& a) {
  const crk_net_desc& d = n->d;
  const int L = n->L;
  const long long N = (long long)a.B * a.T, P = N * 64;
  const GatedF32 lay = gated_f32(n, N);
  const float *X = a.saved + lay.x, *SKIP = a.saved + lay.skip, *H1 = a.saved + lay.h1;
  float *dS = n->scratch + lay.ds, *dH1 = n->scratch + lay.dh1;
  const int head_act = d.kind == 1 ? ACT_LRELU : ACT_RELU;
  const float sL = (float)sqrt(1.0 / L), rs = 0.70710678118654752440f;
  if (k.want_w) RUN(wgrad_conv(n, r, n->idx_last2, a.dy, a.lddy, H1, 64, head_act, 1.f, k.precise));
  ConvP h2 = conv_bw(n, a.B, a.T, n->ents[n->idx_last2], a.dy, a.lddy, dH1, 64);
  h2.dmask = H1; h2.ldm = 64; h2.dmask_act = head_act;
  RUN(conv_go(h2, MODE_PLAIN, k.precise, a.s));
  if (k.want_w) RUN(wgrad_conv(n, r, n->idx_last1, dH1, 64, SKIP, 64, head_act, sL, k.precise));
  ConvP h1 = conv_bw(n, a.B, a.T, n->ents[n->idx_last1], dH1, 64, dS, 64);
  h1.dmask = SKIP; h1.ldm = 64; h1.dmask_act = head_act; h1.out_scale = sL;
  RUN(conv_go(h1, MODE_PLAIN, k.precise, a.s));
  const float* dxo = nullptr;
  for (int l = L - 1; l >= 0; l--) {
    const ConvEntry& ec = n->ents[n->idx_conv[l]];
    const ConvEntry& eo = n->ents[n->idx_out[l]];
    const int dil = n->meta[n->idx_conv[l]].dilation;
    const int off0 = fwd_off0(n, ec.k, dil);
    float* dG = n->scratch + lay.dg + (long long)l * 2 * P;
    {
      ConvP p = base_conv(n, a.B, a.T);
      p.w_hi = n->whi + eo.bw_off; p.w_lo = n->wlo + eo.bw_off;
      p.cin = 128; p.cin_pad = 128; p.cout = 64; p.cout_pad = 64;
      p.xa = dxo; p.lda = 64; p.cinA = 64; p.scaleA = rs;
      p.xb = dS; p.ldb = 64; p.cinB = 64;
      p.ta = a.saved + lay.ta + l * P; p.sb = a.saved + lay.sb + l * P;
      p.y = dG; p.ldy = 128;
      RUN(conv_go(p, MODE_BWDA, k.precise, a.s));
    }
    if (k.want_w) {
      WgradP w = base_wgrad(n, a.B, a.T);
      w.a1 = dG; w.lda1 = 128; w.ca1 = 128; w.ca = 128;
      w.x = X + l * P; w.ldx = 64; w.cx = 64;
      if (d.dropout > 0.f) { w.drop_p = d.dropout; w.drop_seed = layer_seed(k.seed_val, l); w.drop_seed_ptr = k.seed_ptr; }
      w.ktaps = ec.k; w.dil = dil; w.off0 = off0;
      wgrad_slots(n, r, n->idx_conv[l], w);
      if (d.aux_ch > 0) {
        const ConvEntry& ea = n->ents[n->idx_aux[l]];
        w.has_aux = 1; w.xc = a.c; w.ldc = a.ldc; w.cc = ea.cin; w.partial_aux = n->partials + r->abs[n->idx_aux[l]].pt_off;
      }
      RUN(wgrad_go(n, w, k.precise));
      WgradP v = base_wgrad(n, a.B, a.T);
      v.a1 = dxo; v.lda1 = 64; v.ca1 = 64; v.a2 = dS; v.lda2 = 64; v.ca2 = 64; v.ca = 128;
      v.x = a.saved + lay.z + l * P; v.ldx = 64; v.cx = 64;
      wgrad_slots(n, r, n->idx_out[l], v);
      RUN(wgrad_go(n, v, k.precise));
    }
    if (k.want_dc && d.aux_ch > 0) {
      const ConvEntry& ea = n->ents[n->idx_aux[l]];
      ConvP p = conv_bw(n, a.B, a.T, ea, dG, 128, a.dc, a.lddc);
      p.accumulate = (l != L - 1);
      RUN(conv_go(p, MODE_PLAIN, k.precise, a.s));
    }
    {
      float* out = n->scratch + lay.dx + (long long)l * P;
      ConvP p = conv_bw(n, a.B, a.T, ec, dG, 128, out, 64);
      p.ktaps = ec.k; p.dil = dil; p.off0 = -off0 - (ec.k - 1) * dil;
      if (d.dropout > 0.f) { p.epi_drop_p = d.dropout; p.epi_drop_seed = layer_seed(k.seed_val, l); p.drop_seed_ptr = k.seed_ptr; }
      if (dxo) { p.res = dxo; p.ldr = 64; p.res_scale = rs; }
      if (l == 0 && d.kind == 1) { p.dmask = X; p.ldm = 64; p.dmask_act = ACT_LRELU; }
      RUN(conv_go(p, MODE_PLAIN, k.precise, a.s));
      dxo = out;
    }
  }
  if (k.want_w) RUN(wgrad_conv(n, r, n->idx_first, dxo, 64, a.x, a.ldx, ACT_NONE, 1.f, k.precise));
  if (!k.want_dx) return CRK_OK;
  ConvP p = conv_bw(n, a.B, a.T, n->ents[n->idx_first], dxo, 64, a.dx, a.lddx);
  p.out_scale = a.dx_scale;
  return conv_go(p, MODE_PLAIN, k.precise, a.s);
}
static int net_backward_impl(void* h, unsigned long long version, int flags, unsigned long long seed, const BwdIo& a) {
  Net* n = (Net*)h;
  if (!n || !a.params || !a.x || !a.dy || a.B <= 0 || a.T <= 0) return CRK_ERR_ARG;
  const Shape* r = find_shape(n, a.B, a.T);
  if (!r) return not_reserved("crk_net_backward");
  const Call k = call_facts(flags, seed, false, a.dy, a.lddy, a.dx, a.lddx, a.dc, a.grads);
  const Route& rt = r->route[k.precise];
  if (a.ce && !rt.usums) return CRK_ERR_UNSUPPORTED;
  if (a.dy_num && !(n->d.kind == 2 && rt.fused)) return CRK_ERR_UNSUPPORTED;
  const bool expects_x3f = k.mode == 2 && r->route[0].x3f;
  const bool planes_precise = k.precise || (k.mode == 2 && !expects_x3f);
  RUN(check_forward_tag(n, a.saved, a.B, a.T, flags, k.mode, expects_x3f));
  RUN(flush_pending_wnorm(n, a.s));
  RUN(ensure_prepared(n, a.params, version, a.s));
  n->jobs.clear();
  if (n->d.kind != 2 && !a.saved) return CRK_ERR_ARG;
  int form;
  RUN(bwd_form(n, rt, k, planes_precise, &form));
  switch (form) {
    case BWD_CHAIN: RUN(bwd_chain(n, r, k, a)); break;
    case BWD_CHAIN_LAYERS: RUN(bwd_chain_layers(n, r, k, a)); break;
    case BWD_FOLDED_SPLIT: case BWD_FOLDED: RUN(bwd_folded(n, r, k, a, form == BWD_FOLDED_SPLIT)); break;
    case BWD_FUSED_SPLIT: case BWD_FUSED: RUN(bwd_fused(n, r, k, a, form == BWD_FUSED_SPLIT)); break;
    default: RUN(bwd_layers(n, r, k, a));
  }
  if (k.want_w) {
    RUN(wgrad_flush(n, a.B, a.T, k.precise, a.s));
    RUN(finish_wnorm(n, r, a.params, a.grads, k.defer_wn, a.s));
  }
  return CRK_OK;
}
extern "C" int crk_net_backward(void* h, const float* params, unsigned long long version, float* grads, const float* x,
                                int ldx, const float* c, int ldc, const float* dy, int lddy, float* dx, int lddx,
                                float dx_scale, float* dc, int lddc, const float* saved, int B, int T, int flags,
                                unsigned long long seed, void* stream) {
  const BwdIo a = {.params = params, .grads = grads, .x = x, .ldx = ldx, .c = c, .ldc = ldc, .dy = dy, .lddy = lddy, .dx = dx, .lddx = lddx,
                   .dx_scale = dx_scale, .dc = dc, .lddc = lddc, .saved = saved, .B = B, .T = T, .dy_num = nullptr, .dy_den = nullptr, .ce = nullptr,
                   .s = (hipStream_t)stream};
  return net_backward_impl(h, version, flags, seed, a);
}
extern "C" int crk_net_backward_scaled(void* h, const float* params, unsigned long long version, float* grads, const float* x,
                                       int ldx, const float* c, int ldc, const float* dy, int lddy, float* dx, int lddx,
                                       float dx_scale, float* dc, int lddc, const float* saved, int B, int T, int flags,
                                       unsigned long long seed, const float* dy_num, const float* dy_den, void* stream) {
  if (!h || !dy_num || !dy_den) return CRK_ERR_ARG;
  const BwdIo a = {.params = params, .grads = grads, .x = x, .ldx = ldx, .c = c, .ldc = ldc, .dy = dy, .lddy = lddy, .dx = dx, .lddx = lddx,
                   .dx_scale = dx_scale, .dc = dc, .lddc = lddc, .saved = saved, .B = B, .T = T, .dy_num = dy_num, .dy_den = dy_den, .ce = nullptr,
                   .s = (hipStream_t)stream};
  return net_backward_impl(h, version, flags, seed, a);
}
extern "C" int crk_net_embed_grad_supported(void* h, int B, int T, int flags) {
  Net* n = (Net*)h;
  if (!n || B <= 0 || T <= 0) return 0;
  return route_at(n, B, T, flags & CRK_FLAG_PRECISE).usums ? 1 : 0;
}
extern "C" int crk_net_backward_embed(void* h, const float* params, unsigned long long version, float* grads, const float* x,
                                      int ldx, const float* c, int ldc, const float* dy, int lddy, float* dx, int lddx,
                                      float dx_scale, const float* saved, int B, int T, int flags, unsigned long long seed,
                                      const long long* idx, long long run, int c0, int E, int n_rows, float* dtable,
                                      void* stream) {
  Net* n = (Net*)h;
  if (!n || !idx || !dtable || !grads || run != T || c0 < 0 || E < 1 || n_rows < 1 || c0 + E > n->d.aux_ch ||
      (flags & CRK_FLAG_NO_PARAM_GRAD))
    return CRK_ERR_ARG;
  const CondEmbed ce = {idx, run, c0, E, n_rows, dtable};
  const BwdIo a = {.params = params, .grads = grads, .x = x, .ldx = ldx, .c = c, .ldc = ldc, .dy = dy, .lddy = lddy, .dx = dx, .lddx = lddx,
                   .dx_scale = dx_scale, .dc = nullptr, .lddc = 0, .saved = saved, .B = B, .T = T, .dy_num = nullptr, .dy_den = nullptr, .ce = &ce,
                   .s = (hipStream_t)stream};
  return net_backward_impl(h, version, flags, seed, a);
}

__global__ void seed_next_kernel(unsigned long long* state, unsigned long long* out) {
  unsigned long long z = (*state += 0x9E3779B97F4A7C15ull);
  z = (z ^ (z >> 30)) * 0xBF58476D1CE4E5B9ull;
  z = (z ^ (z >> 27)) * 0x94D049BB133111EBull;
  *out = (z ^ (z >> 31)) & 0x3fffffffffffffffull;
}
extern "C" int crk_seed_next(unsigned long long* state, unsigned long long* out, void* stream) {
  if (!state || !out) return CRK_ERR_ARG;
  hipLaunchKernelGGL(seed_next_kernel, dim3(1), dim3(1), 0, (hipStream_t)stream, state, out);
  CRK_CHECK_LAUNCH();
  return CRK_OK;
}

static int flush_plain_wgrads(int n_nets, void* const* nets, hipStream_t s) {
  {
    PwMP M; memset(&M, 0, sizeof(M));
    int layers = 0, max_G = 0, max_wa = 0, max_wb = 0, max_tiles = 0;
    double flops = 0.0, bytes = 0.0;
    for (int i = 0; i < n_nets; i++) {
      Net* n = (Net*)nets[i];
      if (!n) return CRK_ERR_ARG;
      const Shape* r = n->pw_shape;
      if (!r) continue;
      if (M.n == CRK_MAX_NETS_PW) { RUN(flush_pending_plain_wgrad(n, s)); continue; }
      const PsTables& Tb = r->ps;
      M.q[M.n] = n->pw_params;
      M.first[M.n] = layers;
      layers += Tb.nw;
      if (n->pw_params.G > max_G) max_G = n->pw_params.G;
      if (Tb.max_wa > max_wa) max_wa = Tb.max_wa;
      if (Tb.max_wb > max_wb) max_wb = Tb.max_wb;
      if (Tb.max_tiles > max_tiles) max_tiles = Tb.max_tiles;
      flops += Tb.wflops_per_frame * r->B * r->T;
      bytes += 2.0 * (Tb.max_wa + Tb.max_wb) * (double)r->B * r->T * Tb.nw;
      M.n++;
      n->pw_shape = nullptr;
    }
    M.first[M.n] = layers;
    if (M.n > 0) RUN(launch_pstack_wgrad_multi(M, layers, max_G, max_wa, max_wb, max_tiles, flops, bytes, s));
  }
  return CRK_OK;
}
extern "C" int crk_nets_wnorm_bwd(int n_nets, void* const* nets, void* stream) {
  if (n_nets < 0 || (n_nets > 0 && !nets)) return CRK_ERR_ARG;
  hipStream_t s = (hipStream_t)stream;
  RUN(flush_plain_wgrads(n_nets, nets, s));
  NetRefs R; memset(&R, 0, sizeof(R));
  int total = 0;
  for (int i = 0; i < n_nets; i++) {
    Net* n = (Net*)nets[i];
    if (!n) return CRK_ERR_ARG;
    if (!n->wn_shape) continue;
    if (R.n == CRK_MAX_NETS) {
      RUN(flush_pending_wnorm(n, s));
      continue;
    }
    NetRef& q = R.r[R.n++];
    q.ents = n->wn_shape->d_ents; q.n_ents = (int)n->ents.size(); q.first = total;
    q.params = n->wn_params; q.grads = n->wn_grads; q.partials = n->partials; q.norms = n->norms;
    total += q.n_ents;
    n->wn_shape = nullptr;
  }
  if (R.n == 0) return CRK_OK;
  return launch_wnorm_bwd_multi(R, total, s);
}

extern "C" int crk_nets_prepare(int n_nets, void* const* nets, const float* const* params, unsigned long long version,
                                float* bump_step, void* stream) {
  if (n_nets < 0 || (n_nets > 0 && (!nets || !params))) return CRK_ERR_ARG;
  hipStream_t s = (hipStream_t)stream;
  NetRefs R; memset(&R, 0, sizeof(R));
  int total = 0, nmax = 1;
  for (int i = 0; i < n_nets; i++) {
    Net* n = (Net*)nets[i];
    if (!n || !params[i]) return CRK_ERR_ARG;
    if (n->prepared_version == version && n->prepared_params == params[i]) continue;
    if (net_nmax(n) > nmax) nmax = net_nmax(n);
    if (R.n == CRK_MAX_NETS) { RUN(ensure_prepared(n, params[i], version, s)); continue; }
    NetRef& q = R.r[R.n++];
    q.ents = n->d_ents; q.n_ents = (int)n->ents.size(); q.first = total;
    q.params = params[i]; q.whi = n->whi; q.wlo = n->wlo; q.norms = n->norms;
    total += q.n_ents;
    n->prepared_version = version; n->prepared_params = params[i];
  }
  if (R.n == 0) return bump_step ? launch_step_bump(bump_step, s) : CRK_OK;
  R.bump = bump_step;
  return launch_weight_prep_multi(R, total, nmax, s);
}
```

crank_amd/csrc/pstack_kernels.hip:

```cpp
#include "conv_kernels.h"
#include "stack_common.h"


#ifndef PS_ABL
#define PS_ABL 0
#endif
#ifdef PS_PROF
__device__ unsigned long long ps_prof_buf[256 * 8 * 8];
__device__ unsigned long long ps_prof_res[1024 * 2];
extern "C" int crk_debug_ps_prof(unsigned long long* out, unsigned long long* res) {
  if (hipMemcpyFromSymbol(out, HIP_SYMBOL(ps_prof_buf), sizeof(unsigned long long) * 256 * 8 * 8) != hipSuccess) return 2;
  return hipMemcpyFromSymbol(res, HIP_SYMBOL(ps_prof_res), sizeof(unsigned long long) * 1024 * 2) == hipSuccess ? 0 : 2;
}
#define PS_T(i) { const unsigned long long t_ = __builtin_readcyclecounter(); pacc_[i] += t_ - plast_; plast_ = t_; }
#else
#define PS_T(i)
#endif
#define PS_WFRAG(ptr) ((PS_ABL & 4) ? xb : lds_frag(ptr))
#define PS_XFRAG(ptr) ((PS_ABL & 8) ? x0 : lds_frag(ptr))
#define PS_MAXP(NT) ((NT) == 512 ? 4 : 8)
__host__ __device__ __forceinline__ int ps_tpc(int k, int rows_pad, int kp, int cap_pieces, int w_bytes) {
  int t = cap_pieces / (rows_pad * (kp >> 3));
  const int tl = w_bytes / (rows_pad * (kp * 2 + 16));
  if (tl < t) t = tl;
// ... 499 lines not shown
      const bool ok = idx < nb;
      lb[u] = ok ? r * RB + cc * 16 : -1; gb[u] = (r * LY.wb + cc * 8) * 2; qb[u] = ok ? r : (1 << 24);
    }
    int fu = c_beg / ncpu, ff = (c_beg - fu * ncpu) * PW_FR, fc = c_beg;
    sk_u32x4 sa0[4], sb0[6], sa1[4], sb1[6];
#define PW_FETCH2(SA, SB)                                                                                    \
  {                                                                                                          \
    const bool live_ = fc < c_end;                                                                           \
    const int basea_ = (int)(((long)fu * p.T + ff) * LY.wa * 2), baseb_ = (int)(((long)fu * p.T + ff + LY.off0) * LY.wb * 2); \
    const int hia_ = live_ ? p.T - ff : 0, lob_ = -(ff + LY.off0), hib_ = live_ ? p.T - ff - LY.off0 : lob_;   \
    _Pragma("unroll") for (int u = 0; u < 4; u++)                                                            \
      SA[u] = __builtin_amdgcn_raw_buffer_load_b128(rA, qa[u] < hia_ ? basea_ + ga[u] : SK_OOB, 0, 0);        \
    _Pragma("unroll") for (int u = 0; u < 6; u++)                                                            \
      SB[u] = __builtin_amdgcn_raw_buffer_load_b128(rB, (qb[u] >= lob_ && qb[u] < hib_) ? baseb_ + gb[u] : SK_OOB, 0, 0); \
    fc++; ff += PW_FR;                                                                                       \
    if (ff >= p.T) { ff = 0; fu++; }                                                                         \
  }
#define PW_COMMIT2(SA, SB)                                                                                   \
  {                                                                                                          \
    _Pragma("unroll") for (int u = 0; u < 4; u++)                                                            \
      if (la[u] >= 0) *reinterpret_cast<sk_u32x4*>(at_hi + la[u]) = SA[u];                                    \
    _Pragma("unroll") for (int u = 0; u < 6; u++)                                                            \
      if (lb[u] >= 0) *reinterpret_cast<sk_u32x4*>(bt_hi + lb[u]) = SB[u];                                    \
  }
#define PW_COMPUTE(SA)                                                                                       \
  {                                                                                                          \
    constexpr int NB = MAXT <= 4 ? 2 : 1, NA = (SA) ? 1 : MAXT;                                              \
    bf16x8 fa[NB][NA], fb[NB][MAXT];                                                                         \
    _Pragma("unroll") for (int m = 0; m < MAXT; m++) {                                                       \
      if (m < NA) fa[0][m] = sw_tr_frag(at_hi + a_off[m], RA);                                               \
      fb[0][m] = sw_tr_frag(bt_hi + b_off[m], RB);                                                           \
    }                                                                                                        \
    _Pragma("unroll") for (int kc = 0; kc < PW_FR / 16; kc++) {                                              \
      if (NB == 2 && kc + 1 < PW_FR / 16) {                                                                  \
        _Pragma("unroll") for (int m = 0; m < MAXT; m++) {                                                   \
          if (m < NA) fa[(kc + 1) % NB][m] = sw_tr_frag(at_hi + a_off[m] + (kc + 1) * 16 * RA, RA);          \
          fb[(kc + 1) % NB][m] = sw_tr_frag(bt_hi + b_off[m] + (kc + 1) * 16 * RB, RB);                      \
        }                                                                                                    \
      }                                                                                                      \
      __builtin_amdgcn_sched_barrier(0);                                                                     \
      _Pragma("unroll") for (int m = 0; m < MAXT; m++) acc[m] = mfma_bf16(fa[kc % NB][(SA) ? 0 : m], fb[kc % NB][m], acc[m]); \
      if (bias_wave) bsum += sw_sum8(fa[kc % NB][0]);                                                        \
      __builtin_amdgcn_sched_barrier(0);                                                                     \
      if (NB == 1 && kc + 1 < PW_FR / 16) {                                                                  \
        _Pragma("unroll") for (int m = 0; m < MAXT; m++) {                                                   \
          if (m < NA) fa[0][m] = sw_tr_frag(at_hi + a_off[m] + (kc + 1) * 16 * RA, RA);                      \
          fb[0][m] = sw_tr_frag(bt_hi + b_off[m] + (kc + 1) * 16 * RB, RB);                                  \
        }                                                                                                    \
      }                                                                                                      \
    }                                                                                                        \
  }
    PW_FETCH2(sa0, sb0)
    PW_FETCH2(sa1, sb1)
    PW_T(0)
    for (int c = c_beg; c < c_end; c += 2) {
      __syncthreads();
      PW_COMMIT2(sa0, sb0)
      __syncthreads();
      PW_T(1)
      PW_FETCH2(sa0, sb0)
      PW_T(2)
      PW_COMPUTE(SA)
      PW_T(3)
      __syncthreads();
      PW_COMMIT2(sa1, sb1)
      __syncthreads();
      PW_T(1)
      PW_FETCH2(sa1, sb1)
      PW_T(2)
      PW_COMPUTE(SA)
      PW_T(3)
    }
#undef PW_FETCH2
#undef PW_COMMIT2
#undef PW_COMPUTE
  }
  if (PRECISE && c_end > c_beg) PW_FETCH(c_beg)
  for (int c = c_beg; PRECISE && c < c_end; c++) {
    __syncthreads();
    PW_COMMIT()
    __syncthreads();
    if (c + 1 < c_end) PW_FETCH(c + 1)
#pragma unroll
    for (int kc = 0; kc < PW_FR / 16; kc++) {
#pragma unroll
      for (int m = 0; m < MAXT; m++) {
        if (wave + 4 * m < ntiles) {
          const bf16x8 a_hi = sw_tr_frag(at_hi + a_off[m] + kc * 16 * RA, RA);
          const bf16x8 b_hi = sw_tr_frag(bt_hi + b_off[m] + kc * 16 * RB, RB);
          acc[m] = mfma_bf16(a_hi, b_hi, acc[m]);
          if (m == 0 && bias_wave) bsum += sw_sum8(a_hi);
          if (PRECISE) {
            const bf16x8 a_lo = sw_tr_frag(at_hi + plane + a_off[m] + kc * 16 * RA, RA);
            const bf16x8 b_lo = sw_tr_frag(bt_hi + plane + b_off[m] + kc * 16 * RB, RB);
            acc[m] = mfma_bf16(a_lo, b_hi, acc[m]);
            acc[m] = mfma_bf16(a_hi, b_lo, acc[m]);
            if (m == 0 && bias_wave) bsum += sw_sum8(a_lo);
          }
        }
      }
    }
  }

#pragma unroll
  for (int m = 0; m < MAXT; m++) {
    const int j = wave + 4 * m;
    if (j < ntiles) {
      const int ct = j % nct, it = (j / nct) % nit, tap = j / (nct * nit);
      const int ci = it * 32 + l31;
      float* out = p.partials + LY.pt + ((long)g * LY.k + tap) * LY.ca * LY.cb;
      if (ci < LY.cb) {
#pragma unroll
        for (int i = 0; i < 16; i++) {
          const int co = ct * 32 + (i & 3) + 8 * (i >> 2) + 4 * half;
          if (co < LY.ca) out[(long)co * LY.cb + ci] = acc[m][i];
        }
      }
    }
  }
  if (bias_wave) {
    const float tot = bsum + __shfl_xor(bsum, 32);
    const int co = wave * 32 + l31;
    if (half == 0 && co < LY.ca) p.partials[LY.pb + (long)g * LY.ca + co] = tot;
  }
#ifdef PW_PROF
  PW_T(4)
  pacc_[5] = __builtin_readcyclecounter() - pstart_;
  {
    const int wg = blockIdx.y * gridDim.x + blockIdx.x;
    if (wg < 512 && lane == 0) {
#pragma unroll
      for (int i = 0; i < 8; i++) pw_prof_buf[(wg * 4 + wave) * 8 + i] = pacc_[i];
    }
  }
#endif
}

template <bool PRECISE, int MAXT = PW_MAXT>
__global__ __launch_bounds__(256) void pstack_wgrad_kernel(const PwP p) {
  extern __shared__ __attribute__((aligned(16))) unsigned char smem[];
  if (!PRECISE && MAXT > 5) {
    const PwLayer& Y = p.layers[blockIdx.y];
    const int per = (((Y.ca + 31) >> 5) * ((Y.cb + 31) >> 5) * Y.k + 3) >> 2;
    const bool sa = (4 % ((Y.ca + 31) >> 5)) == 0;
    if (per <= 3) { if (sa) pstack_wgrad_body<PRECISE, 3, true>(p, blockIdx.x, blockIdx.y, smem); else pstack_wgrad_body<PRECISE, 3>(p, blockIdx.x, blockIdx.y, smem); return; }
    if (per <= 5) { if (sa) pstack_wgrad_body<PRECISE, 5, true>(p, blockIdx.x, blockIdx.y, smem); else pstack_wgrad_body<PRECISE, 5>(p, blockIdx.x, blockIdx.y, smem); return; }
  }
  if (!PRECISE) {
    const PwLayer& Y = p.layers[blockIdx.y];
    if ((4 % ((Y.ca + 31) >> 5)) == 0) { pstack_wgrad_body<PRECISE, MAXT, !PRECISE>(p, blockIdx.x, blockIdx.y, smem); return; }
  }
  pstack_wgrad_body<PRECISE, MAXT>(p, blockIdx.x, blockIdx.y, smem);
}
template <int MAXT>
__global__ __launch_bounds__(256) void pstack_wgrad_multi_kernel(const PwMP m) {
  extern __shared__ __attribute__((aligned(16))) unsigned char smem[];
  int r = 0;
  while (r + 1 < m.n && (int)blockIdx.y >= m.first[r + 1]) r++;
  const PwP& p = m.q[r];
  if ((int)blockIdx.x >= p.G) return;
  pstack_wgrad_body<false, MAXT>(p, blockIdx.x, blockIdx.y - m.first[r], smem);
}
int launch_pstack_wgrad_multi(const PwMP& m, int total_layers, int max_G, int max_wa, int max_wb, int max_tiles, double flops,
                              double bytes, hipStream_t s) {
  const int RA = ((max_wa + 31) & ~31) * 2 + 64, RB = ((max_wb + 31) & ~31) * 2 + 64;
  const int lds = PW_FR * RA + (PW_FR + PW_SPAN) * RB;
  static bool attr_set = false;
  if (!attr_set) {
    if (hipFuncSetAttribute((const void*)pstack_wgrad_multi_kernel<2>, hipFuncAttributeMaxDynamicSharedMemorySize, 160 * 1024) != hipSuccess ||
        hipFuncSetAttribute((const void*)pstack_wgrad_multi_kernel<PW_MAXT>, hipFuncAttributeMaxDynamicSharedMemorySize, 160 * 1024) != hipSuccess)
      return CRK_ERR_HIP;
    attr_set = true;
  }
  conv_prof_bytes(6, bytes);
  conv_prof_begin(6, flops, s);
  if (max_tiles <= 8) hipLaunchKernelGGL(pstack_wgrad_multi_kernel<2>, dim3(max_G, total_layers), dim3(256), lds, s, m);
  else hipLaunchKernelGGL(pstack_wgrad_multi_kernel<PW_MAXT>, dim3(max_G, total_layers), dim3(256), lds, s, m);
  conv_prof_end(6, s);
  CRK_CHECK_LAUNCH();
  return CRK_OK;
}

int pstack_wgrad_supported(int ca, int cb, int wa, int wb, int k, int dil) {
  const int nct = (ca + 31) / 32, nit = (cb + 31) / 32;
  return nct * nit * k <= 4 * PW_MAXT && (k - 1) * dil <= PW_SPAN && wa <= 128 && wb <= 128 && (wa & 15) == 0 &&
         (wb & 15) == 0 && ca <= wa && cb <= wb;
}

int launch_pstack_wgrad(const PwP& p, int nlayers, int max_wa, int max_wb, bool precise, double flops, hipStream_t s, int max_tiles) {
  const int RA = ((max_wa + 31) & ~31) * 2 + 64, RB = ((max_wb + 31) & ~31) * 2 + 64;
  const int lds = (precise ? 2 : 1) * (PW_FR * RA + (PW_FR + PW_SPAN) * RB);
  static bool attr_set = false;
  if (!attr_set) {
    const void* fns[6] = {(const void*)pstack_wgrad_kernel<true>, (const void*)pstack_wgrad_kernel<false>, (const void*)pstack_wgrad_kernel<false, 3>,
                          (const void*)pstack_wgrad_kernel<false, 4>, (const void*)pstack_wgrad_kernel<false, 5>, (const void*)pstack_wgrad_kernel<false, 6>};
    for (int i = 0; i < 6; i++)
      if (hipFuncSetAttribute(fns[i], hipFuncAttributeMaxDynamicSharedMemorySize, 160 * 1024) != hipSuccess) return CRK_ERR_HIP;
    attr_set = true;
  }
  dim3 grid(p.G, nlayers);
  conv_prof_bytes(6, 2.0 * (max_wa + max_wb) * (double)p.B * p.T * nlayers);
  conv_prof_begin(6, flops, s);
  const int per = max_tiles > 0 ? (max_tiles + 3) / 4 : PW_MAXT;
  if (precise) hipLaunchKernelGGL(pstack_wgrad_kernel<true>, grid, dim3(256), lds, s, p);
  else if (per <= 3) hipLaunchKernelGGL((pstack_wgrad_kernel<false, 3>), grid, dim3(256), lds, s, p);
  else if (per == 4) hipLaunchKernelGGL((pstack_wgrad_kernel<false, 4>), grid, dim3(256), lds, s, p);
  else if (per == 5) hipLaunchKernelGGL((pstack_wgrad_kernel<false, 5>), grid, dim3(256), lds, s, p);
  else if (per == 6) hipLaunchKernelGGL((pstack_wgrad_kernel<false, 6>), grid, dim3(256), lds, s, p);
  else hipLaunchKernelGGL(pstack_wgrad_kernel<false>, grid, dim3(256), lds, s, p);
  conv_prof_end(6, s);
  CRK_CHECK_LAUNCH();
  return CRK_OK;
}
```

crank_amd/net/trainer/trainer_vqvae.py:

```python

import torch

from ... import parallel
from ...config import cfg
from .basetrainer import BaseTrainer
from .utils import clip_grad_norm as flat_clip_grad_norm


def _one_like(t):
    if t.is_cuda:
        from ... import ops
        return ops.one_like(t)
    key = (t.device, t.dtype, tuple(t.shape))
    if key not in _ONES:
        _ONES[key] = torch.ones_like(t)
    return _ONES[key]


_ONES = {}


def _scaled(w, t):
    return t if float(w) == 1.0 else w * t


class VQVAETrainer(BaseTrainer):
    def __init__(self, *args, **kwargs):
        super().__init__(*args, **kwargs)
        self.cycle_flag = False
        self._check_cycle_start()

    def check_custom_start(self):
        self._check_cycle_start()

    def train(self, batch, phase="train"):
        self._cond_cache = None
        self._label_cache = None
        self._open_arena()
        loss = self._get_loss_dict(batch)
        self._G_tail = None
        self._defer_G_tail = (phase == "train" and parallel.is_dist() and self.conf["use_spkr_classifier"]
                              and self._G_step_is_last_of_main_update())
        self._C_tail = None
        self._defer_C_tail = self._defer_G_tail and self.conf["use_spkradv_training"]
        side = self._classifier_stream(batch, phase)
        late = cfg.overlap_c == 2

        def fork_classifier(loss):
            side.wait_stream(torch.cuda.current_stream())
            with torch.cuda.stream(side):
                return self.forward_spkrclassifier(batch, loss, phase=phase)

        if side is not None and not late:
            loss = fork_classifier(loss)
        loss = self._main_update(batch, loss, phase)
        if side is not None and late:
            loss = fork_classifier(loss)
        if self._G_tail is not None:
            self._defer_G_tail = False
            loss = self.forward_spkrclassifier(batch, loss, phase=phase)
            tail, self._G_tail = self._G_tail, None
            tail()
            loss = self.forward_spkradv(batch, loss, phase=phase)
        else:
            self._defer_G_tail = False
            loss = self.forward_spkradv(batch, loss, phase=phase)
            if side is None:
                loss = self.forward_spkrclassifier(batch, loss, phase=phase)
        if self._C_tail is not None:
            tail, self._C_tail = self._C_tail, None
            tail()
        self._defer_C_tail = False
        if side is not None:
            torch.cuda.current_stream().wait_stream(side)
        values = self._parse_loss(loss)
        self._flush_writer(loss, phase)
        self._pending_choices = None
        self._close_arena()
        return values

    def _classifier_is_independent(self):
        return not self.cycle_flag

    def _classifier_stream(self, batch, phase):
        if not (phase == "train" and self.conf["use_spkr_classifier"] and not parallel.is_dist()
                and self._classifier_is_independent() and batch["in_feats"].is_cuda
                and cfg.overlap_c != 0):
            return None
        if getattr(self, "_c_stream", None) is None:
            self._c_stream = torch.cuda.Stream(device=batch["in_feats"].device)
        return self._c_stream

    def _main_update(self, batch, loss, phase):
        return self.forward_cycle(batch, loss, phase) if self.cycle_flag else self.forward_vqvae(batch, loss, phase)

    @torch.no_grad()
    def dev(self, batch):
        return self.train(batch, phase="dev")

    @torch.no_grad()
    def eval(self, batch):
        feats = self._feats(batch)
        out = {}
        for name in self.spkrs.keys():
            enc_h = self._get_enc_h(batch)
            dec_h, spkrvec = self._get_dec_h(batch, cv_spkr_name=name)
            out[name] = self.model["G"](feats, enc_h, dec_h, spkrvec=spkrvec)["decoded"]
        return out

    @torch.no_grad()
    def reconstruction(self, batch, tdir="reconstruction"):
        enc_h = self._get_enc_h(batch)
        dec_h, spkrvec = self._get_dec_h(batch, cv_spkr_name=None)
        return self.model["G"].forward(self._feats(batch), enc_h, dec_h, spkrvec=spkrvec)["decoded"]

    def _feats(self, batch):
        return batch["raw"] if self.conf["use_raw"] else batch["in_feats"]

    def _cond(self, batch, cv=False):
        cache = getattr(self, "_cond_cache", None)
        if cache is None or cache[0] is not batch:
            cache = self._cond_cache = (batch, {})
        if cv not in cache[1]:
            enc_h = self._get_enc_h(batch, use_cvfeats=cv)
            dec_h, spkrvec = self._get_dec_h(batch, use_cvfeats=cv)
            cache[1][cv] = (enc_h, dec_h, spkrvec)
        return cache[1][cv]

    def _discard_grads(self, name, flag):
        m = self.model.get(name)
        if m is not None and hasattr(m, "skip_param_grads"):
            m.skip_param_grads = flag

    def _classify(self, x):
        return self.model["C"](x.transpose(1, 2)).transpose(1, 2)

    def _ce(self, logits, target):
        return self.criterion["ce"](logits.reshape(-1, logits.size(2)), target.reshape(-1))

    def _fused_ce_ok(self, model):
        ce = self.criterion["ce"]
        return hasattr(model, "forward_ce") and getattr(ce, "ignore_index", None) == -100 and \
            not cfg.separate_ce

    def _classify_ce(self, x, target):
        C = self.model["C"]
        if self._fused_ce_ok(C):
            return self._dp_ce(C.forward_ce(x.transpose(1, 2), target), target)
        return self._ce(self._classify(x), target)

    def _dp_ce(self, value, target):
        ce = self.criterion["ce"]
        return ce.scale_ce(value, target.reshape(-1)) if hasattr(ce, "scale_ce") else value

    def _spkradv_ce(self, encoded, target, detach=False):
        S = self.model["SPKRADV"]
        if self._fused_ce_ok(S):
            return self._dp_ce(S.forward_ce(encoded, target, detach=detach), target)
        return self._ce(S.forward(encoded, detach=detach) if detach else S.forward(encoded), target)

    def step_model(self, loss, model="G"):
        m = self.model[model]
        self.optimizer[model].zero_grad()
        total = loss[model]
        grouped = (getattr(self, "group_stack_maintenance", True)
                   and hasattr(m, "finish_grads"))
        if grouped:
            m.defer_wnorm = True
        try:
            torch.autograd.backward(total, _one_like(total))
        finally:
            if grouped:
                m.defer_wnorm = False
                m.finish_grads()
        if model == "G" and getattr(self, "_defer_G_tail", False) and hasattr(self.optimizer[model], "reduce_grads_start"):
            self.optimizer[model].reduce_grads_start()
            self._G_tail = lambda: self._finish_step(model, m, grouped)
            return
        if model == "C" and getattr(self, "_defer_C_tail", False) and hasattr(self.optimizer[model], "mark_reduced"):
            self._C_tail = lambda: self._finish_step(model, m, grouped)
            return
        if model == "SPKRADV" and getattr(self, "_C_tail", None) is not None and hasattr(self.optimizer[model], "mark_reduced"):
            from ... import ops
            parallel.all_reduce_many([m.grad_flat, self.model["C"].grad_flat])
            self.optimizer[model].mark_reduced()
            self.optimizer["C"].mark_reduced()
            self._finish_step(model, m, grouped)
            tail, self._C_tail = self._C_tail, None
            tail()
            return
        self._finish_step(model, m, grouped)

    def _G_step_is_last_of_main_update(self):
        return True

    def _finish_step(self, model, m, grouped):
        clip = self.conf["optim"][model]["clip_grad_norm"]
        if clip != 0:
            if hasattr(self.optimizer[model], "reduce_grads"):
                self.optimizer[model].reduce_grads()
            if hasattr(m, "grad_flat"):
                flat_clip_grad_norm(m, clip)
            else:
                torch.nn.utils.clip_grad_norm_(m.parameters(), clip)
        opt = self.optimizer[model]
        if grouped and hasattr(opt, "step_dev"):
            opt.step(defer_bump=True)
            m.prepare_nets(bump_step=opt.step_dev)
        else:
            opt.step()

    def forward_vqvae(self, batch, loss, phase="train"):
        enc_h, dec_h, spkrvec = self._cond(batch)
        G = self.model["G"]
        kw = ({"want_commit": True, "commit_mask": batch["encoder_mask"]}
              if getattr(G, "can_commit", False) and self.conf["ema_flag"]
              and not cfg.separate_commit else {})
        outputs = G.forward(self._feats(batch), enc_h, dec_h, spkrvec=spkrvec, **kw)
        loss = self.calculate_vqvae_loss(batch, outputs, loss)
        self._discard_grads("SPKRADV", True)
        if self.conf["use_spkradv_training"]:
            loss = self.calculate_spkradv_loss(batch, outputs, loss, label="org", phase=phase)
        loss.add("objective", 1.0, loss["G"])
        if phase == "train":
            self.step_model(loss, model="G")
        self._discard_grads("SPKRADV", False)
        return loss

    def forward_cycle(self, batch, loss, phase="train"):
        enc_h, dec_h, spkrvec = self._cond(batch)
        enc_h_cv, dec_h_cv, spkrvec_cv = self._cond(batch, cv=True)
        outs = self.model["G"].cycle_forward(self._feats(batch), enc_h, dec_h, enc_h_cv, dec_h_cv, spkrvec, spkrvec_cv)
        self._discard_grads("SPKRADV", True)
        self._discard_grads("C", True)
        if self.conf["use_vqvae_loss"]:
            loss = self.calculate_vqvae_loss(batch, outs[0]["org"], loss)
        loss = self.calculate_cyclevqvae_loss(batch, outs, loss)
        if self.conf["use_spkradv_training"]:
            for label in ["cv", "recon"]:
                loss = self.calculate_spkradv_loss(batch, outs[0][label], loss, label=label, phase=phase)
        loss.add("objective", 1.0, loss["G"])
        if phase == "train":
            self.step_model(loss, model="G")
        self._discard_grads("SPKRADV", False)
        self._discard_grads("C", False)
        return loss

    def forward_spkradv(self, batch, loss, phase="train"):
        if not self.conf["use_spkradv_training"]:
            return loss
        enc_h, dec_h, spkrvec = self._cond(batch)
        grad_on = torch.is_grad_enabled()
        G = self.model["G"]
        kw = {"need_decoded": False} if getattr(G, "can_skip_decoder", False) else {}
        with torch.no_grad():
            outputs = G.forward(self._feats(batch), enc_h, dec_h, spkrvec=spkrvec, **kw)
        er = self.model["G"].encoder_receptive_size if self.conf["causal"] else 0
        encoded = [e[:, er:] for e in outputs["encoded_unmod"]] if er else outputs["encoded_unmod"]
        with torch.set_grad_enabled(grad_on):
            loss["SPKRADV"] = _scaled(self.conf["alpha"]["ce"], self._spkradv_ce(encoded, batch["org_h"][:, er:], detach=True))
            if phase == "train":
                self.step_model(loss, model="SPKRADV")
        return loss

    def forward_spkrclassifier(self, batch, loss, phase="train"):
        if not self.conf["use_spkr_classifier"]:
            return loss
        loss["C_real"] = self._classify_ce(batch["in_feats"], batch["org_h"])
        loss.add("C", self.conf["alpha"]["ce"], loss["C_real"])
        if phase == "train":
            self.step_model(loss, model="C")
        return loss

    def _commit_terms(self, outputs, emask, loss, suffix=""):
        fused = outputs.get("commit") if suffix == "" else None
        for n in range(self.conf["n_vq_stacks"]):
            enc, emb = outputs["encoded"][n], outputs["emb_idx"][n]
            if fused is not None:
                loss[f"G_commit{n}{suffix}"] = parallel.scale_masked_mean(fused[n], emask)
                continue
            loss[f"G_commit{n}{suffix}"] = self.criterion["fmse"](enc, emb.detach(), mask=emask)
            if not self.conf["ema_flag"]:
                loss[f"G_dict{n}{suffix}"] = self.criterion["fmse"](emb, enc.detach(), mask=emask)
        return loss

    def calculate_vqvae_loss(self, batch, outputs, loss):
        cs = self.conf["causal_size"]
        decoded, target, dmask = outputs["decoded"], batch["out_feats"], batch["decoder_mask"]
        fl1 = self.criterion["fl1"]
        three = fl1.recon(decoded, target, dmask, cs, self.criterion["fstft"]) if hasattr(fl1, "recon") else None
        if three is not None:
            loss["G_l1"], loss["G_mse"], loss["G_stft"] = three
        else:
            loss["G_l1"] = fl1(decoded, target, mask=dmask, causal_size=cs)
            loss["G_mse"] = self.criterion["fmse"](decoded, target, mask=dmask, causal_size=cs)
            loss["G_stft"] = self.criterion["fstft"](decoded, target, causal_size=cs)
        loss = self._commit_terms(outputs, batch["encoder_mask"], loss)
        a = self.conf["alpha"]
        for k in ["l1", "mse", "stft"]:
            loss.add("G", a[k], loss[f"G_{k}"])
        for k in ["commit"] + ([] if self.conf["ema_flag"] else ["dict"]):
            for n in range(self.conf["n_vq_stacks"]):
                loss.add("G", a[k], loss[f"G_{k}{n}"])
        return loss

    def calculate_cyclevqvae_loss(self, batch, outputs, loss):
        a = self.conf["alpha"]
        cs = self.conf["causal_size"] * 2 if self.conf["causal"] else 0
        for c in range(self.conf["n_cycles"]):
            for io in ["cv", "recon"]:
                lbl = f"{c}cyc_{io}"
                o = outputs[c][io]
                if io == "cv":
                    emask = batch["encoder_mask"]
                    loss[f"C_fake_{lbl}"] = self._classify_ce(o["decoded"], batch["cv_h"])
                else:
                    emask, dmask = batch["cycle_encoder_mask"], batch["cycle_decoder_mask"]
                    tgt = batch["in_feats"]
                    fl1 = self.criterion["fl1"]
                    three = (fl1.recon(o["decoded"], tgt, dmask, cs, self.criterion["fstft"]) if hasattr(fl1, "recon")
                             else None)
                    if three is not None:
                        loss[f"G_l1_{lbl}"], loss[f"G_mse_{lbl}"], loss[f"G_stft_{lbl}"] = three
                    else:
                        loss[f"G_l1_{lbl}"] = fl1(o["decoded"], tgt, mask=dmask, causal_size=cs)
                        loss[f"G_mse_{lbl}"] = self.criterion["fmse"](o["decoded"], tgt, mask=dmask, causal_size=cs)
                        loss[f"G_stft_{lbl}"] = self.criterion["fstft"](o["decoded"], tgt, causal_size=cs)
                loss = self._commit_terms(o, emask, loss, suffix=f"_{lbl}")
        for c in range(self.conf["n_cycles"]):
            for io in ["cv", "recon"]:
                lbl = f"{c}cyc_{io}"
                for n in range(self.conf["n_vq_stacks"]):
                    loss.add("G", a["cycle"] * a["commit"], loss[f"G_commit{n}_{lbl}"])
                    if not self.conf["ema_flag"]:
                        loss.add("G", a["cycle"] * a["dict"], loss[f"G_dict{n}_{lbl}"])
                if io == "recon":
                    for k in ["l1", "mse", "stft"]:
                        loss.add("G", a["cycle"] * a[k], loss[f"G_{k}_{lbl}"])
                else:
                    loss.add("G", a["cycle"] * a["ce"], loss[f"C_fake_{lbl}"])
        return loss

    def calculate_spkradv_loss(self, batch, outputs, loss, label="org", phase="train"):
        er = self.model["G"].encoder_receptive_size if self.conf["causal"] else 0
        encoded = [e[:, er:] for e in outputs["encoded_unmod"]] if er else outputs["encoded_unmod"]
        loss[f"G_spkradv_{label}"] = self._spkradv_ce(encoded, batch["org_h"][:, er:])
        w = self.conf["alpha"]["ce"] * (self.conf["alpha"]["cycle"] if label == "recon" else 1)
        loss.add("G", w, loss[f"G_spkradv_{label}"])
        return loss

    def _check_cycle_start(self):
        if self.conf["use_cyclic_training"] and self.steps > self.conf["n_steps_cycle_start"]:
            self.cycle_flag = True
        if self.conf["use_cyclic_training"] and not self.conf["use_spkr_classifier"]:
            raise ValueError("use_cyclic_training requires use_spkr_classifier to be true")
```

crank_amd/net/trainer/utils.py:

```python
import torch
from torch import nn

from ... import ops, parallel
from ..module.loss import CrossEntropyLoss, CustomFeatureLoss, MeanLoss


def get_criterion(conf, device="cuda"):
    return {
        "mse": MeanLoss("mse"),
        "l1": MeanLoss("l1"),
        "ce": CrossEntropyLoss(ignore_index=-100),
        "kld": nn.KLDivLoss(reduction="mean"),
        "fmse": CustomFeatureLoss(loss_type="mse", causal=conf["causal"], device=device),
        "fl1": CustomFeatureLoss(loss_type="l1", causal=conf["causal"], device=device),
        "fstft": CustomFeatureLoss(loss_type="stft", stft_params=conf["stft_params"], causal=conf["causal"],
                                   device=device),
    }


class FlatAdam:

    def __init__(self, model, lr, betas=(0.9, 0.999), eps=1e-8, grad_reduce_fn=None):
        self.model = model
        self.base_lr = float(lr)
        self.betas, self.eps = betas, eps
        dev = model.flat.device
        self.lr_dev = torch.tensor([lr], device=dev, dtype=torch.float32)
        self.step_dev = torch.zeros(1, device=dev, dtype=torch.float32)
        self.exp_avg = torch.zeros_like(model.flat.data)
        self.exp_avg_sq = torch.zeros_like(model.flat.data)
        self.grad_reduce_fn = grad_reduce_fn
        self._reduced = False
        self._inflight = None
        self.clear_grads = True
        self.param_groups = [{"lr": float(lr), "params": [model.flat]}]

    def state_dict(self):
        return {"exp_avg": self.exp_avg.clone(), "exp_avg_sq": self.exp_avg_sq.clone(), "step": self.step_dev.clone(),
                "lr": self.param_groups[0]["lr"]}

    def load_state_dict(self, sd):
        self.exp_avg.copy_(sd["exp_avg"])
        self.exp_avg_sq.copy_(sd["exp_avg_sq"])
        self.step_dev.copy_(sd["step"])
        self.set_lr(sd["lr"])
        for off, n in getattr(self.model, "ema_codebook_ranges", lambda: [])():
            if bool(self.exp_avg[off: off + n].any()) or bool(self.exp_avg_sq[off: off + n].any()):
                self.model._trained_codebooks = True

    def set_lr(self, lr):
        if float(lr) != self.param_groups[0]["lr"]:
            self.param_groups[0]["lr"] = float(lr)
            self.lr_dev.fill_(float(lr))

    def zero_grad(self, set_to_none=False):
        self.model.zero_grad()

    def reduce_grads_start(self):
        if self.grad_reduce_fn is not None and not self._reduced and self._inflight is None:
            self._inflight = parallel.grad_allreduce_start(self.model.grad_flat)

    def mark_reduced(self):
        if self.grad_reduce_fn is not None:
            self._reduced = True

    def reduce_grads(self):
        if self._inflight is not None:
            self._inflight.finish()
            self._inflight, self._reduced = None, True
        if self.grad_reduce_fn is not None and not self._reduced:
            self.grad_reduce_fn(self.model.grad_flat)
            self._reduced = True

    def step(self, defer_bump=False):
        m = self.model
        self.reduce_grads()
        self._reduced = False
        self._update(m, defer_bump)
        if self.clear_grads:
            m.grads_clean = True
        m.touch(by_optimizer=True)

    def _update(self, m, defer_bump):
        ops.adam_step(m.flat.data, m.grad_flat, self.exp_avg, self.exp_avg_sq, self.lr_dev, self.step_dev,
                      self.betas[0], self.betas[1], self.eps, clear_grads=self.clear_grads, defer_bump=defer_bump)


class FlatRAdam(FlatAdam):

    def _update(self, m, defer_bump):
        ops.radam_step(m.flat.data, m.grad_flat, self.exp_avg, self.exp_avg_sq, self.lr_dev, self.step_dev,
                       self.betas[0], self.betas[1], self.eps, clear_grads=self.clear_grads, defer_bump=defer_bump)


class FlatLamb(FlatAdam):

    def __init__(self, model, lr, betas=(0.9, 0.999), eps=1e-6, grad_reduce_fn=None):
        super().__init__(model, lr, betas=betas, eps=eps, grad_reduce_fn=grad_reduce_fn)
        n = model.flat.numel()
        spans, pos = [], 0
        for _, off, shp in sorted(model._entries, key=lambda e: e[1]):
            size = 1
            for d in shp:
                size *= int(d)
            if off > pos:
                spans.append((pos, off - pos))
            if size:
                spans.append((off, size))
            pos = max(pos, off + size)
        if pos < n:
            spans.append((pos, n - pos))
        tile = ops.lamb_tile()
        tiles, tensors = [], []
        for s, (off, size) in enumerate(spans):
            first = len(tiles)
            for o in range(0, size, tile):
                tiles.append((off + o, min(tile, size - o), s, 0))
            tensors.append((first, len(tiles) - first))
        dev = model.flat.device
        self.tensor_spans = spans
        self.tiles = torch.tensor(tiles, dtype=torch.int32, device=dev).reshape(-1, 4).contiguous()
        self.tensors = torch.tensor(tensors, dtype=torch.int32, device=dev).reshape(-1, 2).contiguous()
        self.upd = torch.zeros(n, device=dev, dtype=torch.float32)
        self.part = torch.zeros(2 * max(1, len(tiles)), device=dev, dtype=torch.float32)
        self.trust_ratio = torch.ones(max(1, len(tensors)), device=dev, dtype=torch.float32)

    def _update(self, m, defer_bump):
        ops.lamb_step(m.flat.data, m.grad_flat, self.exp_avg, self.exp_avg_sq, self.upd, self.tiles, self.tensors, self.part,
                      self.trust_ratio, self.lr_dev, self.step_dev, self.betas[0], self.betas[1], self.eps,
                      clear_grads=self.clear_grads, defer_bump=defer_bump)


_OPTIMIZERS = {"adam": FlatAdam, "radam": FlatRAdam, "lamb": FlatLamb}


def get_optimizer(conf, model, grad_reduce_fn=None):
    optimizer = {}
    for m in ["G", "D", "C", "SPKRADV"]:
        if m in model:
            t = conf["optim"][m]["type"]
            if t not in _OPTIMIZERS:
                raise ValueError("Invalid optimizer type")
            optimizer[m] = _OPTIMIZERS[t](model[m], conf["optim"][m]["lr"], grad_reduce_fn=grad_reduce_fn)
    return optimizer


class StepLR:

    def __init__(self, optimizer, step_size, gamma):
        self.optimizer, self.step_size, self.gamma = optimizer, int(step_size), float(gamma)
        self.last_epoch = 0

    def step(self, steps=None):
        self.last_epoch = self.last_epoch + 1 if steps is None else int(steps)
        self.optimizer.set_lr(self.optimizer.base_lr * self.gamma ** (self.last_epoch // self.step_size))

    def get_last_lr(self):
        return [self.optimizer.param_groups[0]["lr"]]


def get_scheduler(conf, optimizer):
    scheduler = {}
    for m in ["G", "D", "C", "SPKRADV"]:
        if m in optimizer:
            scheduler[m] = StepLR(optimizer[m], conf["optim"][m]["decay_step_size"], conf["optim"][m]["decay_size"])
    return scheduler


def clip_grad_norm(model, max_norm):
    g = model.grad_flat
    total = torch.linalg.vector_norm(g)
    g.mul_(torch.clamp(max_norm / (total + 1e-6), max=1.0))
    return total


def get_dataloader(conf, scp, scaler, flag="train", n_jobs=0, reader=None, device="cuda"):
    from .dataset import BaseDataset, DeviceLoader, calculate_maxflen

    if flag in ["train", "reconstruction"]:
        feats = list(scp["train"]["feats"].values()) + list(scp["dev"]["feats"].values())
    elif flag in ["eval"]:
        feats = list(scp["eval"]["feats"].values())
    else:
        raise ValueError(f"unknown flag {flag}")
    if flag in ["reconstruction", "eval"]:
        token_size = conf["batch_len"] * conf["batch_size"]
        conf["batch_len"] = calculate_maxflen(feats, reader=reader)
        conf["batch_size"] = token_size // conf["batch_len"]
    spkrs = dict(zip(scp["train"]["spkrs"], range(len(scp["train"]["spkrs"]))))
    out = {"spkrs": spkrs}
    for phase, shuffle in (("train", True), ("dev", True), ("eval", False)):
        if phase in scp and scp[phase].get("feats"):
            dset = BaseDataset(conf, scp, scaler, phase=phase, reader=reader, device=device)
            out[phase] = DeviceLoader(dset, conf["batch_size"], shuffle=shuffle, rank=parallel.rank() if phase != "eval" else 0,
                                      world_size=parallel.world_size() if phase != "eval" else 1)
    return out
```

crank_amd/ops.py:

```python
import ctypes

import torch

from . import _lib
from .config import cfg
from ._lib import check, ptr, stream_ptr

_PRECISION = cfg.precision


def set_precision(name):
    global _PRECISION
    if name not in ("bf16", "bf16x3", "bf16x3f"):
        raise ValueError(f"unknown precision {name!r} (bf16 | bf16x3 | bf16x3f)")
    _PRECISION = name


def get_precision():
    return _PRECISION


CRK_FLAG_PRECISE = 1
CRK_FLAG_NO_PARAM_GRAD = 2
CRK_FLAG_NO_SAVE = 4
# ... 118 lines not shown

class _NetFn(torch.autograd.Function):

    @staticmethod
    def forward(ctx, x, c, flat, net, owner, offset, dx_scale, no_save=False, ybuf=None, ycol=0, emb=None):
        L = _lib.lib()
        B, T = x.shape[0], x.shape[1]
        if emb is not None and not (c is not None and emb.run == T and net.embed_grad_supported(B, T)):
            raise RuntimeError("conditioning built by concat_embed_owned fed to a net that cannot own its table gradient")
        xk, ldx = _rows(x)
        ck, ldc = (None, 0) if c is None else _rows(c)
        if ybuf is None:
            y = torch.empty(B, T, net.out_ch, device=x.device, dtype=torch.float32)
        else:
            y = ybuf[..., ycol: ycol + net.out_ch]
        ldy = y.stride(1)
        nbytes = net.saved_bytes(B, T)
        saved = torch.empty(max(nbytes // 4, 1), device=x.device, dtype=torch.float32)
        seed_t = net.next_seed() if net.dropout > 0 else None
        params = flat.data_ptr() + 4 * offset
        check(
            L.crk_net_forward(net.handle, params, owner.version, ptr(xk), ldx, ptr(ck), ldc, ptr(y), ldy,
                              ptr(saved), B, T, _flags(no_save=no_save) | (CRK_FLAG_SEED_ON_DEVICE if seed_t is not None else 0), ptr(seed_t),
                              stream_ptr()),
            "crk_net_forward",
        )
        ctx.net, ctx.owner, ctx.offset, ctx.dx_scale, ctx.seed = net, owner, offset, dx_scale, seed_t
        ctx.precision = _PRECISION
        ctx.ld = (ldx, ldc)
        ctx.version = owner.version
        ctx.save_for_backward(xk, ck if ck is not None else torch.empty(0, device=x.device), flat)
        ctx.saved_ws = saved
        ctx.has_c = c is not None
        ctx.emb = emb
        return y

    @staticmethod
    def backward(ctx, dy):
        L = _lib.lib()
        net, owner = ctx.net, ctx.owner
        xk, ck, flat = ctx.saved_tensors
        if not ctx.has_c:
            ck = None
        ldx, ldc = ctx.ld
        B, T = xk.shape[0], xk.shape[1]
        dyk, lddy = _rows(dy)
        dx = torch.empty(B, T, net.in_ch, device=dy.device, dtype=torch.float32) if ctx.needs_input_grad[0] else None
        dc = None
        if ctx.has_c and ctx.needs_input_grad[1]:
            dc = torch.empty(B, T, net.aux_ch, device=dy.device, dtype=torch.float32)
        if ctx.version != owner.version:
            raise RuntimeError("parameters were modified between forward and backward of a crank_amd net")
        skip = owner.skip_param_grads
        defer = (not skip) and getattr(owner, "defer_wnorm", False)
        if not skip:
            owner.grads_clean = False
            if defer:
                owner._wnorm_pending = True
                owner._keepalive.append(ctx.saved_ws)
        params = flat.data_ptr() + 4 * ctx.offset
        grads = owner.grad_flat.data_ptr() + 4 * ctx.offset
        flags = (_flags(skip, precision=ctx.precision, defer_wnorm=defer, backward=True)
                 | (CRK_FLAG_SEED_ON_DEVICE if ctx.seed is not None else 0))
        emb = ctx.emb
        if emb is not None and not skip and not emb.owner.skip_param_grads:
            emb.owner.grads_clean = False
            g = emb.owner.grad_flat[emb.tab_offset: emb.tab_offset + emb.rows * emb.E]
            check(
                L.crk_net_backward_embed(net.handle, params, owner.version, grads, ptr(xk), ldx, ptr(ck), ldc, ptr(dyk), lddy,
                                         ptr(dx), net.in_ch, float(ctx.dx_scale), ptr(ctx.saved_ws), B, T, flags,
                                         ptr(ctx.seed), ptr(emb.idx), emb.run, emb.c0, emb.E, emb.rows, ptr(g), stream_ptr()),
                "crk_net_backward_embed",
            )
            return dx, None, None, None, None, None, None, None, None, None, None
        check(
            L.crk_net_backward(net.handle, params, owner.version, grads, ptr(xk), ldx, ptr(ck), ldc, ptr(dyk), lddy,
                               ptr(dx), net.in_ch, float(ctx.dx_scale), ptr(dc), net.aux_ch, ptr(ctx.saved_ws), B, T,
                               flags, ptr(ctx.seed), stream_ptr()),
            "crk_net_backward",
        )
        return dx, dc, None, None, None, None, None, None, None, None, None


class _NetCEFn(torch.autograd.Function):

    @staticmethod
    def forward(ctx, x, flat, net, owner, offset, dx_scale, target, ignore_index, no_save=False):
        L = _lib.lib()
        B, T = x.shape[0], x.shape[1]
        xk, ldx = _rows(x)
        C = net.out_ch
        y = torch.empty(B, T, C, device=x.device, dtype=torch.float32)
        saved = torch.empty(max(net.saved_bytes(B, T) // 4, 1), device=x.device, dtype=torch.float32)
        params = flat.data_ptr() + 4 * offset
        check(L.crk_net_forward(net.handle, params, owner.version, ptr(xk), ldx, None, 0, ptr(y), C, ptr(saved), B, T,
                                _flags(no_save=no_save), 0, stream_ptr()), "crk_net_forward")
        tk = target.reshape(-1).contiguous()
        assert tk.numel() == B * T, (tk.shape, B, T)
        out = _scalars(2, x.device)
        dl = torch.empty(B * T, C, device=x.device, dtype=torch.float32)
        check(L.crk_ce_fwd(ptr(y), C, ptr(tk), B * T, C, int(ignore_index), ptr(out), ptr(dl), ptr(_loss_scratch(x.device)),
                           stream_ptr()), "crk_ce_fwd")
        ctx.net, ctx.owner, ctx.offset, ctx.dx_scale = net, owner, offset, dx_scale
        ctx.precision = _PRECISION
        ctx.ldx, ctx.version = ldx, owner.version
        ctx.save_for_backward(xk, flat, dl, out)
        ctx.saved_ws = saved
        return out[0]

    @staticmethod
    def backward(ctx, g):
        L = _lib.lib()
        net, owner = ctx.net, ctx.owner
        xk, flat, dl, out = ctx.saved_tensors
        B, T = xk.shape[0], xk.shape[1]
        C = net.out_ch
        dx = torch.empty(B, T, net.in_ch, device=g.device, dtype=torch.float32) if ctx.needs_input_grad[0] else None
        if ctx.version != owner.version:
            raise RuntimeError("parameters were modified between forward and backward of a crank_amd net")
        skip = owner.skip_param_grads
        defer = (not skip) and getattr(owner, "defer_wnorm", False)
        if not skip:
            owner.grads_clean = False
            if defer:
                owner._wnorm_pending = True
                owner._keepalive.append(ctx.saved_ws)
        params = flat.data_ptr() + 4 * ctx.offset
        grads = owner.grad_flat.data_ptr() + 4 * ctx.offset
        gk = g.contiguous().reshape(1)
        flags = _flags(skip, precision=ctx.precision, defer_wnorm=defer, backward=True)
        rc = L.crk_net_backward_scaled(net.handle, params, owner.version, grads, ptr(xk), ctx.ldx, None, 0, ptr(dl), C, ptr(dx),
                                       net.in_ch, float(ctx.dx_scale), None, 0, ptr(ctx.saved_ws), B, T, flags, 0, ptr(gk),
                                       ptr(out), stream_ptr())
        if rc == 3:
            res = torch.empty_like(dl)
            check(L.crk_ce_bwd(ptr(dl), B * T, C, ptr(out), ptr(gk), ptr(res), stream_ptr()), "crk_ce_bwd")
            rc = L.crk_net_backward(net.handle, params, owner.version, grads, ptr(xk), ctx.ldx, None, 0, ptr(res), C, ptr(dx),
                                    net.in_ch, float(ctx.dx_scale), None, 0, ptr(ctx.saved_ws), B, T, flags, 0, stream_ptr())
        check(rc, "crk_net_backward_scaled")
        return dx, None, None, None, None, None, None, None, None


def net_ce(net, owner, offset, x, target, dx_scale=1.0, ignore_index=-100):
    if net.dropout > 0:
        raise ValueError("net_ce: nets with dropout go through net_apply + cross_entropy")
    return _NetCEFn.apply(x, owner.flat, net, owner, offset, dx_scale, target, ignore_index, not torch.is_grad_enabled())


def nets_wnorm_bwd(nets):
    arr = (ctypes.c_void_p * len(nets))(*[n.handle for n in nets])
    check(_lib.lib().crk_nets_wnorm_bwd(len(nets), arr, stream_ptr()), "crk_nets_wnorm_bwd")


def nets_prepare(nets, param_ptrs, version, bump_step=None):
    arr = (ctypes.c_void_p * len(nets))(*[n.handle for n in nets])
    par = (ctypes.c_void_p * len(nets))(*param_ptrs)
    check(_lib.lib().crk_nets_prepare(len(nets), arr, par, version, ptr(bump_step), stream_ptr()), "crk_nets_prepare")


def net_apply(net, owner, offset, x, c=None, dx_scale=1.0, out=None):
    ybuf, ycol = out if out is not None else (None, 0)
    emb = getattr(c, "_crk_embed", None) if c is not None else None
    return _NetFn.apply(x, c, owner.flat, net, owner, offset, dx_scale, not torch.is_grad_enabled(), ybuf, ycol, emb)


class _AliasCatFn(torch.autograd.Function):

    @staticmethod
    def forward(ctx, *xs):
        B, T = xs[0].shape[0], xs[0].shape[1]
        W = sum(x.shape[2] for x in xs)
        ctx.widths = [x.shape[2] for x in xs]
        return xs[0].as_strided((B, T, W), (T * W, W, 1))

    @staticmethod
    def backward(ctx, d):
        out, off = [], 0
        for w in ctx.widths:
            out.append(d[..., off: off + w])
            off += w
        return tuple(out)


def cat_channels(xs):
    xs = list(xs)
    if len(xs) > 1 and all(x.dim() == 3 and x.dtype == torch.float32 for x in xs):
        B, T = xs[0].shape[0], xs[0].shape[1]
        W = sum(x.shape[2] for x in xs)
        base, off, ok = xs[0].data_ptr(), 0, xs[0].storage_offset() * 4 + B * T * W * 4 <= xs[0].untyped_storage().nbytes()
        for x in xs:
            ok = ok and x.shape[:2] == (B, T) and x.stride() == (T * W, W, 1) and x.data_ptr() == base + 4 * off
            off += x.shape[2]
        if ok:
            return _AliasCatFn.apply(*xs)
    return torch.cat(xs, dim=-1)


def vq_image_bytes(K, D):
    return int(_lib.lib().crk_vq_image_bytes(int(K), int(D)))


def vq_image_build(codebooks, images):
    for i in range(0, len(codebooks), 4):
        cb, im = codebooks[i: i + 4], images[i: i + 4]
        check(_lib.lib().crk_vq_image_build_multi(len(cb), _parr(cb), _iarr([c.shape[0] for c in cb]), int(cb[0].shape[1]),
                                                  _parr(im), stream_ptr()), "crk_vq_image_build_multi")


def _vq_call(xk, ldx, addk, ldadd, codebook, idx, e, qx, mk=None, commit_out=None, image=None):
    L = _lib.lib()
    B, T, D = xk.shape
    K = codebook.shape[0]
    ldq = qx.stride(1) if qx is not None else D
    xsum = None
    if addk is not None or commit_out is not None or image is not None:
        xsum = torch.empty(B, T, D, device=xk.device, dtype=torch.float32) if addk is not None else None
        rc = L.crk_vq_forward_fused(ptr(xk), ldx, ptr(addk), ldadd, ptr(xsum), D, ptr(codebook), B * T, D, K, ptr(idx), ptr(e), D,
                                    ptr(qx), ldq, ptr(mk), ptr(commit_out),
                                    ptr(_loss_scratch(xk.device)) if commit_out is not None else None, ptr(image), stream_ptr())
        if rc == 0:
            return (xsum, D) if xsum is not None else (xk, ldx)
        if rc != 3:
            check(rc, "crk_vq_forward_fused")
        if addk is not None:
            xsum = xk + addk
            xk, ldx = xsum, D
    check(L.crk_vq_forward(ptr(xk), ldx, ptr(codebook), B * T, D, K, ptr(idx), ptr(e), D, ptr(qx), ldq, stream_ptr()),
          "crk_vq_forward")
    if commit_out is not None:
        check(L.crk_masked_loss_fwd(ptr(xk), ldx, ptr(e), D, 0.0, ptr(mk), B * T, D, 1, ptr(commit_out),
                                    ptr(_loss_scratch(xk.device)), stream_ptr()), "crk_masked_loss_fwd")
    return xk, ldx


class _VQFn(torch.autograd.Function):

    @staticmethod
    def forward(ctx, x, codebook, owner, cb_offset, qbuf=None, qcol=0, want=3, add=None, image=None):
        xk, ldx = _rows(x)
        addk, ldadd = (None, 0) if add is None else _rows(add)
        B, T, D = xk.shape
        K = codebook.shape[0]
        e = torch.empty(B, T, D, device=x.device, dtype=torch.float32) if want & 1 else None
        qx = None
        if want & 2:
            qx = torch.empty(B, T, D, device=x.device, dtype=torch.float32) if qbuf is None else qbuf[..., qcol: qcol + D]
        idx = torch.empty(B, T, device=x.device, dtype=torch.int64)
        xin, _ = _vq_call(xk, ldx, addk, ldadd, codebook, idx, e, qx, image=image)
        ctx.owner, ctx.cb_offset, ctx.K, ctx.D = owner, cb_offset, K, D
        ctx.has_add = add is not None
        ctx.save_for_backward(idx)
        ctx.mark_non_differentiable(idx)
        ctx.set_materialize_grads(False)
        return e, qx, idx, (xin if add is not None else None)

    @staticmethod
    def backward(ctx, de, dqx, _didx, dxin):
        (idx,) = ctx.saved_tensors
        if de is not None and ctx.owner is not None and not ctx.owner.skip_param_grads:
            ctx.owner.grads_clean = False
            g = ctx.owner.grad_flat[ctx.cb_offset: ctx.cb_offset + ctx.K * ctx.D].view(ctx.K, ctx.D)
            g.index_add_(0, idx.reshape(-1), de.reshape(-1, ctx.D))
        dx = dqx if dxin is None else (dxin if dqx is None else dqx + dxin)
        return dx, None, None, None, None, None, None, (dx if ctx.has_add else None), None


def vq_apply(x, codebook, owner=None, cb_offset=0, qx_out=None, want_e=True, want_qx=True, add=None, image=None):
    qbuf, qcol = qx_out if qx_out is not None else (None, 0)
    r = _VQFn.apply(x, codebook, owner, cb_offset, qbuf, qcol, (1 if want_e else 0) | (2 if want_qx else 0), add, image)
    return r if add is not None else r[:3]


VQ_JOIN = True
VQ_IMAGE = True


class _VQCommitFn(torch.autograd.Function):

    @staticmethod
    def forward(ctx, x, codebook, mask, qbuf=None, qcol=0, add=None, alias=False, image=None):
        xk, ldx = _rows(x)
        addk, ldadd = (None, 0) if add is None else _rows(add)
        B, T, D = xk.shape
        e = torch.empty(B, T, D, device=x.device, dtype=torch.float32)
        qx = torch.empty(B, T, D, device=x.device, dtype=torch.float32) if qbuf is None else qbuf[..., qcol: qcol + D]
        idx = torch.empty(B, T, device=x.device, dtype=torch.int64)
        mk = None
        if mask is not None:
            mk = mask.reshape(-1).contiguous()
            mk = mk.view(torch.uint8) if mk.dtype == torch.bool else mk.to(torch.uint8)
            assert mk.numel() == B * T, (mk.numel(), B * T)
        out = _scalars(2, x.device)
        xin, ldin = _vq_call(xk, ldx, addk, ldadd, codebook, idx, e, qx, mk, out, image=image)
        ctx.geom = (B, T, D, ldin)
        ctx.has_m = mk is not None
        ctx.has_add = add is not None
        ctx.save_for_backward(xin, e, mk if mk is not None else out, out)
        ctx.mark_non_differentiable(idx, e)
        ctx.set_materialize_grads(False)
        return (e, qx, idx, out[0], (xin if add is not None else None),
                (x.view_as(x) if alias else None), (qx.view_as(qx) if alias else None))

    @staticmethod
    def backward(ctx, _de, dqx, _didx, dcommit, dxin, dxal=None, dqx2=None):
        if dxin is not None:
            dqx = dxin if dqx is None else dqx + dxin
# ... 415 lines not shown
            dx = torch.empty(N, Dm, device=xk.device, dtype=torch.float32)
            check(L.crk_recon_loss_bwd(ptr(xk), ldx, ptr(yk), ldy, ptr(mk), B, T, Dm, len(ctx.res), ia[0], ia[1], ia[2],
                                       ptr(out), ptr(unit), ptr(gs[0]), ptr(gs[1]), ptr(gs[2]), ptr(dx), Dm, stream_ptr()),
                  "crk_recon_loss_bwd")
            return dx.view(ctx.xshape), None, None, None, None, None
        dx, scale = (unit, g3.contiguous().reshape(1)) if g3 is not None else (None, None)
        dx, scale = _masked_bwd_acc(xk, yk, mk, ctx.geom, out, (g1, g2), dx, scale)
        if scale is not None:
            dx = dx.mul_(scale)
        return dx.view(ctx.xshape), None, None, None, None, None


def recon_loss(x, y, mask, resolutions, windows, logratio=0.0):
    return _ReconFn.apply(x, y, mask, tuple(resolutions), tuple(windows), logratio)


def stft_loss(x, y, resolutions, windows, logratio=0.0):
    return _STFTLossFn.apply(x, y, tuple(resolutions), tuple(windows), logratio)


_ONES = {}
_WCONST = {}


def one_like(t):
    key = (t.device, t.dtype, tuple(t.shape))
    if key not in _ONES:
        _ONES[key] = torch.ones_like(t)
    return _ONES[key]


def _farr(vals):
    return (ctypes.c_float * len(vals))(*[float(v) for v in vals])


class _WeightedSumFn(torch.autograd.Function):

    @staticmethod
    def forward(ctx, weights, constant, *terms):
        ts = [t.reshape(1) if t.is_contiguous() else t.contiguous().reshape(1) for t in terms]
        out = _scalars(1, terms[0].device)
        check(_lib.lib().crk_weighted_sum(len(ts), _parr(ts), _farr(weights), float(constant), ptr(out), stream_ptr()),
              "crk_weighted_sum")
        ctx.weights = tuple(float(w) for w in weights)
        return out[0]

    @staticmethod
    def backward(ctx, g):
        ws = ctx.weights
        one = _ONES.get((g.device, g.dtype, tuple(g.shape)))
        key = (ws, g.device)
        cached = one is not None and g.data_ptr() == one.data_ptr()
        if cached and key not in _WCONST:
            if g.is_cuda and torch.cuda.is_current_stream_capturing():
                cached = False
            else:
                _WCONST[key] = torch.tensor(ws, device=g.device, dtype=torch.float32)
        if cached:
            grads = _WCONST[key]
        else:
            grads = torch.empty(len(ws), device=g.device, dtype=torch.float32)
            check(_lib.lib().crk_weighted_sum_bwd(len(ws), _farr(ws), ptr(g.contiguous().reshape(1)), ptr(grads), stream_ptr()),
                  "crk_weighted_sum_bwd")
        return (None, None) + tuple(grads[i] for i in range(len(ws)))


def weighted_sum(terms, weights, constant=0.0):
    return _WeightedSumFn.apply(tuple(weights), float(constant), *terms)


def _label_runs(idx):
    B, T = idx.shape
    if T > 1 and idx.stride(1) == 0 and (B == 1 or idx.stride(0) == T):
        return idx, T
    return idx.contiguous(), 1


def _concat_embed_fwd(a, b, table, idx):
    L = _lib.lib()
    B, T = idx.shape
    ak, lda = (None, 0) if a is None else _rows(a)
    bk, ldb = (None, 0) if b is None else _rows(b)
    ca = 0 if a is None else a.shape[-1]
    cb = 0 if b is None else b.shape[-1]
    E = table.shape[1]
    out = torch.empty(B, T, ca + cb + E, device=idx.device, dtype=torch.float32)
    ik, run = _label_runs(idx)
    check(L.crk_concat_embed_run(ptr(ak), lda, ca, ptr(bk), ldb, cb, ptr(table), E, ptr(ik), run, B * T, ptr(out),
                                 ca + cb + E, stream_ptr()), "crk_concat_embed_run")
    return out, ik, run, (ca, cb, E)


class _ConcatEmbedFn(torch.autograd.Function):

    @staticmethod
    def forward(ctx, a, b, table, idx, owner, tab_offset, flat):
        out, ik, run, (ca, cb, E) = _concat_embed_fwd(a, b, table, idx)
        B, T = idx.shape
        ctx.geom = (ca, cb, E, table.shape[0], run, B * T)
        ctx.owner, ctx.tab_offset = owner, tab_offset
        ctx.save_for_backward(ik)
        return out

    @staticmethod
    def backward(ctx, dout):
        L = _lib.lib()
        (ik,) = ctx.saved_tensors
        ca, cb, E, rows, run, N = ctx.geom
        dk, ld = _rows(dout)
        if ctx.owner is not None and not ctx.owner.skip_param_grads:
            ctx.owner.grads_clean = False
            g = ctx.owner.grad_flat[ctx.tab_offset: ctx.tab_offset + rows * E]
            scratch = torch.empty(L.crk_embed_bwd_scratch_floats(N, E, rows), device=dk.device, dtype=torch.float32)
            check(L.crk_embed_bwd_run(ptr(dk), ld, ca + cb, E, ptr(ik), run, N, rows, ptr(g), ptr(scratch), stream_ptr()),
                  "crk_embed_bwd_run")
        da = dk[..., :ca] if (ca and ctx.needs_input_grad[0]) else None
        db = dk[..., ca:ca + cb] if (cb and ctx.needs_input_grad[1]) else None
        return da, db, None, None, None, None, None


def concat_embed(a, b, table, idx, owner=None, tab_offset=0, flat=None):
    return _ConcatEmbedFn.apply(a, b, table, idx, owner, tab_offset, flat)


class EmbedCond:
    __slots__ = ("idx", "run", "c0", "E", "rows", "owner", "tab_offset")


def embed_owned_ok(net, a, b, idx):
    if not cfg.cond_sums or idx.dim() != 2:
        return False
    if (a is not None and a.requires_grad) or (b is not None and b.requires_grad):
        return False
    B, T = idx.shape
    return _label_runs(idx)[1] == T and net.embed_grad_supported(B, T)


def concat_embed_owned(a, b, table, idx, owner, tab_offset):
    with torch.no_grad():
        out, ik, run, (ca, cb, E) = _concat_embed_fwd(a, b, table, idx)
    e = EmbedCond()
    e.idx, e.run, e.c0, e.E, e.rows, e.owner, e.tab_offset = ik, run, ca + cb, E, table.shape[0], owner, tab_offset
    out._crk_embed = e
    return out


def adam_step(flat, grad, exp_avg, exp_avg_sq, lr_dev, step_dev, beta1=0.9, beta2=0.999, eps=1e-8, clear_grads=False,
              defer_bump=False):
    check(_lib.lib().crk_adam_step(ptr(flat), ptr(grad), ptr(exp_avg), ptr(exp_avg_sq), flat.numel(), ptr(lr_dev),
                                   ptr(step_dev), beta1, beta2, eps, (1 if clear_grads else 0) | (2 if defer_bump else 0),
                                   stream_ptr()), "crk_adam_step")


def radam_step(flat, grad, exp_avg, exp_avg_sq, lr_dev, step_dev, beta1=0.9, beta2=0.999, eps=1e-8, clear_grads=False,
               defer_bump=False):
    check(_lib.lib().crk_radam_step(ptr(flat), ptr(grad), ptr(exp_avg), ptr(exp_avg_sq), flat.numel(), ptr(lr_dev),
                                    ptr(step_dev), beta1, beta2, eps, (1 if clear_grads else 0) | (2 if defer_bump else 0),
                                    stream_ptr()), "crk_radam_step")


def lamb_tile():
    return int(_lib.lib().crk_lamb_tile())


def lamb_step(flat, grad, exp_avg, exp_avg_sq, upd, tiles, tensors, part, ratio_out, lr_dev, step_dev, beta1=0.9, beta2=0.999,
              eps=1e-6, clear_grads=False, defer_bump=False):
    assert tiles.dtype == torch.int32 and tensors.dtype == torch.int32 and tiles.is_contiguous() and tensors.is_contiguous()
    assert upd.numel() >= flat.numel() and part.numel() >= 2 * tiles.shape[0]
    assert ratio_out is None or ratio_out.numel() >= tensors.shape[0]
    check(_lib.lib().crk_lamb_step(ptr(flat), ptr(grad), ptr(exp_avg), ptr(exp_avg_sq), ptr(upd), ptr(tiles), tiles.shape[0],
                                   ptr(tensors), tensors.shape[0], ptr(part), ptr(ratio_out), ptr(lr_dev), ptr(step_dev),
                                   beta1, beta2, eps, (1 if clear_grads else 0) | (2 if defer_bump else 0), stream_ptr()),
          "crk_lamb_step")


def logmel(raw, T, n_fft, hop, win_length, window, mel_basis, eps=1e-10, mean=None, std=None, center=False):
    L = _lib.lib()
    raw = raw.contiguous()
    B, n = raw.shape
    n_mels = mel_basis.shape[1]
    out = torch.empty(B, T, n_mels, device=raw.device, dtype=torch.float32)
    check(L.crk_logmel_fwd(ptr(raw), n, B, n, T, n_fft, hop, win_length, ptr(window), ptr(mel_basis), n_mels, float(eps),
                           ptr(mean), ptr(std), ptr(out), n_mels, 1 if center else 0, stream_ptr()), "crk_logmel_fwd")
    return out
```

include/crank_hip.h:

```cpp
#ifndef CRANK_HIP_H
#define CRANK_HIP_H
#ifdef __cplusplus
extern "C" {
#endif

#define CRK_OK 0
#define CRK_ERR_ARG 1
#define CRK_ERR_HIP 2
#define CRK_ERR_UNSUPPORTED 3

#define CRK_FLAG_PRECISE 1
#define CRK_FLAG_NO_PARAM_GRAD 2
#define CRK_FLAG_NO_SAVE 4
#define CRK_FLAG_DEFER_WNORM 8

#define CRK_FLAG_SEED_ON_DEVICE 16
#define CRK_FLAG_FWD_PRECISE 32
#define CRK_FLAG_BWD_PLAIN 64

typedef struct crk_net_desc {
  int kind;
  int in_ch, out_ch, kernel_size, layers, stacks;
  int res_ch, gate_ch, skip_ch, aux_ch;
  int conv_ch;
  int causal;
  int use_bias;
  float slope;
  float dropout;
} crk_net_desc;

void* crk_net_create(const crk_net_desc* desc);
void crk_net_destroy(void* net);
long long crk_net_param_count(void* net);
int crk_net_conv_count(void* net);
int crk_net_conv_info(void* net, int i, long long* out9);
long long crk_net_saved_bytes(void* net, int B, int T);
int crk_net_reserve(void* net, int B, int T);
long long crk_net_scratch_bytes(void* net, int B, int T);
int crk_net_forward(void* net, const float* params, unsigned long long version, const float* x, int ldx,
                    const float* c, int ldc, float* y, int ldy, float* saved, int B, int T, int flags,
                    unsigned long long seed, void* stream);
int crk_net_backward(void* net, const float* params, unsigned long long version, float* grads, const float* x,
                     int ldx, const float* c, int ldc, const float* dy, int lddy, float* dx, int lddx, float dx_scale,
                     float* dc, int lddc, const float* saved, int B, int T, int flags, unsigned long long seed,
                     void* stream);
int crk_net_backward_scaled(void* net, const float* params, unsigned long long version, float* grads, const float* x,
                            int ldx, const float* c, int ldc, const float* dy, int lddy, float* dx, int lddx, float dx_scale,
                            float* dc, int lddc, const float* saved, int B, int T, int flags, unsigned long long seed,
                            const float* dy_num, const float* dy_den, void* stream);
int crk_net_embed_grad_supported(void* net, int B, int T, int flags);
int crk_net_backward_embed(void* net, const float* params, unsigned long long version, float* grads, const float* x, int ldx,
                           const float* c, int ldc, const float* dy, int lddy, float* dx, int lddx, float dx_scale,
                           const float* saved, int B, int T, int flags, unsigned long long seed, const long long* idx,
                           long long run, int c0, int E, int n_rows, float* dtable, void* stream);

int crk_seed_next(unsigned long long* state, unsigned long long* out, void* stream);

int crk_nets_wnorm_bwd(int n_nets, void* const* nets, void* stream);
int crk_nets_prepare(int n_nets, void* const* nets, const float* const* params, unsigned long long version,
                     float* bump_step, void* stream);

int crk_vq_forward(const float* x, int ldx, const float* codebook, int N, int D, int K, long long* idx, float* e,
                   int lde, float* qx, int ldq, void* stream);
int crk_vq_forward_fused(const float* x, int ldx, const float* add, int ldadd, float* xsum, int ldsum, const float* codebook,
                         int N, int D, int K, long long* idx, float* e, int lde, float* qx, int ldq,
                         const unsigned char* mask, float* commit_out2, float* scratch, const void* image, void* stream);
long long crk_vq_image_bytes(int K, int D);
int crk_vq_image_build_multi(int nq, const float* const* codebooks, const int* K, int D, void* const* images, void* stream);
long long crk_vq_ema_scratch_bytes(int N, int D, int K);
int crk_vq_ema_stats(const float* x, int ldx, const long long* idx, int N, int D, int K, int* counts, long long* sums,
                     void* scratch, void* stream);
int crk_vq_ema_apply(const int* counts, const long long* sums, float* ema_size, float* ema_w, float* codebook, int D,
                     int K, double decay, double eps, void* stream);
int crk_vq_ema_partial(const float* x, int ldx, const long long* idx, int N, int D, int K, void* scratch, void* stream);
int crk_vq_ema_reduce_multi(int nq, const void* const* scratch, const int* N, const int* D, const int* K,
                            int* const* counts, long long* const* sums, void* stream);
int crk_vq_ema_apply_multi(int nq, const int* const* counts, const long long* const* sums, float* const* ema_size,
                           float* const* ema_w, float* const* codebook, const int* D, const int* K, double decay,
                           double eps, void* stream);
int crk_vq_ema_partial_multi(int nq, const float* const* x, const int* ldx, const long long* const* idx, const int* N,
                             const int* D, const int* K, void* const* scratch, void* stream);
int crk_vq_ema_reduce_size_multi(int nq, const void* const* scratch, const int* N, const int* D, const int* K,
                                 int* const* counts, long long* const* sums, float* const* ema_size, double decay, double eps,
                                 void* stream);
int crk_vq_ema_blend_multi(int nq, const long long* const* sums, float* const* ema_size, float* const* ema_w,
                           float* const* codebook, const int* D, const int* K, double decay, void* stream);
int crk_vq_ema_blend_image_multi(int nq, const long long* const* sums, float* const* ema_size, float* const* ema_w,
                                 float* const* codebook, const int* D, const int* K, double decay, void* const* images,
                                 void* stream);

int crk_loss_scratch_floats(void);
int crk_masked_loss_fwd(const float* x, int ldx, const float* y, int ldy, float yconst, const unsigned char* mask,
                        long long N, int D, int mode, float* out2, float* scratch, void* stream);
int crk_masked_loss_bwd(const float* x, int ldx, const float* y, int ldy, float yconst, const unsigned char* mask,
                        long long N, int D, int mode, const float* stat2, const float* gout, float* dx, int lddx,
                        float* dy, int lddy, void* stream);
int crk_masked_loss_both_fwd(const float* x, int ldx, const float* y, int ldy, const unsigned char* mask, long long N,
                             int D, float* out4, float* scratch, void* stream);
int crk_masked_loss_bwd_acc(const float* x, int ldx, const float* y, int ldy, float yconst, const unsigned char* mask,
                            long long N, int D, int mode, const float* stat2, const float* gout, float* dx, int lddx,
                            float* dy, int lddy, const float* add, int ldadd, const float* add_scale, void* stream);
int crk_vq_commit_bwd(const float* x, int ldx, const float* e, int lde, const unsigned char* mask, long long N, int D,
                      const float* stat2, const float* gout, float* dx, int lddx, float* dsum, int ldsum,
                      const float* a1, int ld1, const float* a2, int ld2, const float* a3, int ld3, void* stream);
int crk_ce_fwd(const float* logits, int ldl, const long long* target, long long N, int C, int ignore_index,
               float* out2, float* dlogits_unscaled, float* scratch, void* stream);
int crk_ce_bwd(float* dlogits_unscaled, long long N, int C, const float* stat2, const float* gout, float* dlogits,
               void* stream);
int crk_stft_loss_fwd(const float* x, int ldx, const float* y, int ldy, int B, int T, int D, int n_fft,
                      int hop_length, int win_length, const float* window, float logratio, float weight,
                      int accumulate, float* out1, float* scratch, void* stream);
int crk_stft_loss_bwd(const float* x, int ldx, const float* y, int ldy, int B, int T, int D, int n_fft,
                      int hop_length, int win_length, const float* window, float logratio, float weight,
                      const float* gout, float* dx, int lddx, void* stream);

int crk_stft_loss_multi_fwd(const float* x, int ldx, const float* y, int ldy, int B, int T, int D, int nres,
                            const int* n_fft, const int* hop_length, const int* win_length, const float* const* windows,
                            float logratio, float* out1, float* scratch, void* stream);
int crk_stft_loss_multi_fwd_grad(const float* x, int ldx, const float* y, int ldy, int B, int T, int D, int nres,
                                 const int* n_fft, const int* hop_length, const int* win_length,
                                 const float* const* windows, float logratio, float* out1, float* dx_unit, int lddx,
                                 float* scratch, void* stream);
int crk_stft_loss_multi_bwd(const float* x, int ldx, const float* y, int ldy, int B, int T, int D, int nres,
                            const int* n_fft, const int* hop_length, const int* win_length, const float* const* windows,
                            float logratio, const float* gout, float* dx, int lddx, void* stream);

int crk_recon_supported(int T, int nres, const int* n_fft, const int* hop_length, const int* win_length);
long long crk_stft_twiddle_floats(int n_fft, int win_length);
int crk_stft_twiddles(int n_fft, int win_length, const float* window, float* table, void* stream);
long long crk_recon_grad_floats(int B, int T, int D, int nres, const int* hop_length, const int* win_length);
int crk_recon_loss_fwd(const float* x, int ldx, const float* y, int ldy, const unsigned char* mask, int B, int T, int D,
                       int nres, const int* n_fft, const int* hop_length, const int* win_length,
                       const float* const* tables, float logratio, float* out5, float* grad, float* scratch,
                       void* stream);
int crk_recon_loss_bwd(const float* x, int ldx, const float* y, int ldy, const unsigned char* mask, int B, int T, int D,
                       int nres, const int* n_fft, const int* hop_length, const int* win_length, const float* out5,
                       const float* grad, const float* g1, const float* g2, const float* g3, float* dx, int lddx,
                       void* stream);

int crk_weighted_sum(int n, const float* const* terms, const float* weights, float constant, float* out, void* stream);
int crk_weighted_sum_bwd(int n, const float* weights, const float* gout, float* grads, void* stream);

int crk_adam_step(float* params, float* grads, float* exp_avg, float* exp_avg_sq, long long n, const float* lr_dev,
                  float* step_dev, float beta1, float beta2, float eps, int clear_grads, void* stream);
int crk_radam_step(float* params, float* grads, float* exp_avg, float* exp_avg_sq, long long n, const float* lr_dev,
                   float* step_dev, double beta1, double beta2, double eps, int clear_grads, void* stream);
int crk_lamb_step(float* params, float* grads, float* exp_avg, float* exp_avg_sq, float* upd, const int* tiles, int n_tiles,
                  const int* tensors, int n_tensors, float* part, float* ratio_out, const float* lr_dev, float* step_dev,
                  double beta1, double beta2, double eps, int clear_grads, void* stream);
int crk_lamb_tile(void);
int crk_concat_embed(const float* a, int lda, int ca, const float* b, int ldb, int cb, const float* table, int E,
                     const long long* idx, long long N, float* out, int ldo, void* stream);
long long crk_embed_bwd_scratch_floats(long long N, int E, int n_rows);
int crk_embed_bwd(const float* dcat, int ld, int c0, int E, const long long* idx, long long N, int n_rows,
                  float* dtable, float* scratch, void* stream);
int crk_concat_embed_run(const float* a, int lda, int ca, const float* b, int ldb, int cb, const float* table, int E,
                         const long long* idx, long long run, long long N, float* out, int ldo, void* stream);
int crk_embed_bwd_run(const float* dcat, int ld, int c0, int E, const long long* idx, long long run, long long N,
                      int n_rows, float* dtable, float* scratch, void* stream);

int crk_logmel_fwd(const float* raw, int ld_raw, int B, int n_samples, int T, int n_fft, int hop, int win_length,
                   const float* window, const float* mel_basis , int n_mels, float eps,
                   const float* mean, const float* std, float* out, int ldo, int center, void* stream);


int crk_scaler_apply(const float* x, int ldx, float* y, int ldy, long long N, int D, const double* mean,
                     const double* scale, int inverse, void* stream);

long long crk_scaler_workspace_bytes(int U, int D);
int crk_scaler_moments(const float* x, int ld, int col0, int D, long long F_total, const long long* utt_start,
                       const long long* utt_start_host, int U, void* workspace, long long workspace_bytes,
                       void* stream);
int crk_scaler_merge(const void* workspace, long long workspace_bytes, int U, int D, const long long* group_start,
                     const int* group_utts, const long long* group_start_host, const int* group_utts_host, int G,
                     double* mean, double* var, long long* count, void* stream);

#define CRK_COLLATE_MAX_STREAMS 8
typedef struct crk_collate_stream {
  const float* src;
  int ld, col0, ncols;
  float* dst;
} crk_collate_stream;
typedef struct crk_collate_desc {
  int n_streams;
  crk_collate_stream streams[CRK_COLLATE_MAX_STREAMS];
  const long long* utt_start;
  const int* utt_spk;
  int n_utt, n_spk;
  const float* lcf0_raw;
  const double* spk_lcf0_mean;
  const double* spk_lcf0_std;
  const float* raw;
  const long long* raw_start;
  int fftl, hop;
} crk_collate_desc;
int crk_collate_batch(const crk_collate_desc* desc, const int* picks, int B, int T, float* cv_lcf0,
                      long long* org_h, long long* cv_h, float* org_onehot, float* cv_onehot,
                      unsigned char* mask, long long* flen, float* raw_out, void* stream);

int crk_decode_f0(const float* lcf0, const float* uv, int B, int T, const int* org_spk, const int* cv_spk,
                  double lcf0_mean, double lcf0_scale, int has_lcf0_scaler, const double* spk_lcf0_mean,
                  const double* spk_lcf0_std, double* cv_lcf0, double* f0, double* normed_lcf0, void* stream);

long long crk_mcd_scratch_bytes(int P, int max_nx, int max_ny, int D, int radius);
int crk_mcd_fastdtw(const double* cv, const long long* cv_off, const double* gt, const long long* gt_off, int P, int D,
                    int radius, int max_nx, int max_ny, double* mcd, int* path_len, int* path_out,
                    long long path_stride, void* scratch, int* status, void* stream);

int crk_prof_enable(int on);
int crk_prof_report(int cls, long long* count, double* total_ms, double* total_flops);
int crk_prof_report_bytes(int cls, double* total_bytes);

int crk_debug_vq_set_f16(int on);
int crk_debug_vq_flags(unsigned long long* host_out3, int reset);

int crk_debug_flush_before(long long bytes);

void* crk_voc_create(int layers, int stacks, int aux_ch, int aux_window, const int* scales, int n_scales, const float* params);
void crk_voc_destroy(void* voc);
long long crk_voc_workspace_bytes(void* voc, int n_utts, int total_frames);
int crk_voc_forward(void* voc, const float* c, const long long* frame_offsets, int n_utts, int total_frames,
                    const float* noise, float* out, void* workspace, long long workspace_bytes, int flags, void* stream);
int crk_voc_upsample(void* voc, const float* c, const long long* frame_offsets, int n_utts, int total_frames, float* out,
                     void* workspace, long long workspace_bytes, void* stream);

void* crk_world_create(int fs, int fftl, double shiftms, double alpha, int order1, int bands, int pulse_capacity);
void crk_world_destroy(void* world);
int crk_world_reserve(void* world, long long max_samples);
long long crk_world_workspace_bytes(void* world, int n_utts, long long total_frames, long long total_samples);
int crk_world_synthesis(void* world, const double* f0, const double* mcep, const double* rmcep, const double* cap,
                        int order1, int bands, const long long* frame_offsets, const long long* sample_offsets, int n_utts,
                        long long total_frames, long long total_samples, long long max_samples, double* y,
                        long long* n_pulses, void* workspace, long long workspace_bytes, void* stream);
int crk_world_frames(void* world, const double* mcep, const double* rmcep, const double* cap, int order1, int bands,
                     long long total_frames, double* sp, double* ap, void* workspace, long long workspace_bytes, void* stream);
int crk_world_pulses(void* world, const double* f0, const long long* frame_offsets, const long long* sample_offsets,
                     int n_utts, int* pulse_pos, double* pulse_shift, unsigned char* pulse_vuv, long long* pulse_count,
                     void* stream);

void* crk_wana_create(int fs, int fftl, double shiftms, double alpha, int order1);
void crk_wana_destroy(void* wana);
int crk_wana_reserve(void* wana, long long max_draws);
long long crk_wana_workspace_bytes(int n_utts, long long total_frames, long long total_samples);
int crk_wana_lowcut(void* wana, const float* x, const double* taps, int n_taps, const long long* sample_offsets, int n_utts,
                    long long total_samples, double* y, void* stream);
int crk_wana_lowcut_tile(void);
int crk_wana_cheaptrick(void* wana, const double* x, const double* f0, const long long* frame_offsets,
                        const long long* sample_offsets, int n_utts, long long total_frames, long long total_samples,
                        long long max_draws, double* sp, void* workspace, long long workspace_bytes, void* stream);
int crk_wana_mcep(void* wana, const double* x, const double* f0, const long long* frame_offsets,
                  const long long* sample_offsets, int n_utts, long long total_frames, long long total_samples,
                  long long max_draws, int order1, double* mcep, double* sp, void* workspace, long long workspace_bytes,
                  void* stream);
int crk_wana_npow(void* wana, const double* sp, const long long* frame_offsets, int n_utts, long long total_frames,
                  double* npow, void* workspace, long long workspace_bytes, void* stream);
int crk_wana_frame_shapes(void* wana, const double* f0, const long long* frame_offsets, int n_utts, long long total_frames,
                          int* shapes, long long* draw_offsets, void* stream);

void* crk_f0_create(int fs, int shiftms, const double* cheby);
void crk_f0_destroy(void* f0);
int crk_f0_reserve(void* f0, long long total_events);
long long crk_f0_workspace_bytes(int n_utts, long long total_samples, long long total_frames, long long total_channels);
int crk_f0_harvest(void* f0h, const double* x, const long long* utt, const double* range, const double* chan_bf,
                   const long long* chan, int n_utts, long long total_samples, long long total_channels,
                   long long total_frames, long long total_events, long long total_out, double* f0, int* status,
                   void* workspace, long long workspace_bytes, void* stream);
int crk_f0_decimate(void* f0h, const double* x, const long long* utt, int n_utts, long long total_samples, double* yd,
                    void* workspace, long long workspace_bytes, void* stream);
int crk_f0_raw_candidates(void* f0h, const double* yd, const long long* utt, const double* range, const double* chan_bf,
                          const long long* chan, int n_utts, long long total_channels, long long total_frames,
                          long long total_events, double* raw, int* status, void* workspace, long long workspace_bytes,
                          void* stream);
int crk_f0_candidates(void* f0h, const double* raw, const long long* utt, int n_utts, long long total_frames, double* cands,
                      void* workspace, long long workspace_bytes, void* stream);
int crk_f0_refine(void* f0h, const double* x, const double* cands, const long long* utt, const double* range, int n_utts,
                  long long total_frames, double* refined, double* scores, void* stream);
int crk_f0_contour(void* f0h, const double* refined, const double* scores, const long long* utt, int n_utts,
                   long long total_frames, double* f0_1ms, void* workspace, long long workspace_bytes, void* stream);
int crk_f0_continuous(const double* f0, const long long* frame_offsets, int n_utts, long long total_frames, float* uv,
                      double* f0_filled, double* cf0, double* lf0, double* lcf0, int* status, void* stream);

int crk_gl_create(int fs, int n_fft, int win_length, int hop, int n_mels, const double* pinv_basis, void** handle);
void crk_gl_destroy(void* gl);
long long crk_gl_workspace_bytes(int n_utts, long long total_frames, long long total_samples);
int crk_gl_linear_spectrum(void* gl, const double* mlfb, long long total_frames, int magnitude, double* S, void* stream);
int crk_gl_run(void* gl, const double* S, const double* angles0, const long long* frame_offsets,
               const long long* sample_offsets, int n_utts, long long total_frames, long long total_samples, int n_iter,
               int clip, double* y, void* workspace, long long workspace_bytes, void* stream);
int crk_gl_stft(void* gl, const double* x, const long long* frame_offsets, const long long* sample_offsets, int n_utts,
                long long total_frames, long long total_samples, double* spec, void* stream);
int crk_gl_istft(void* gl, const double* spec, const long long* frame_offsets, const long long* sample_offsets, int n_utts,
                 long long total_frames, long long total_samples, double* y, void* workspace, long long workspace_bytes,
                 void* stream);

long long crk_debug_alloc_count(void);

int crk_debug_net_paths(void* net, int B, int T);

const char* crk_version(void);

#ifdef __cplusplus
}
#endif
#endif
```

Measured before the change: 22.12 million frames/s.

## Batch speaker-net updates into one multi-model Adam and weight-prep launch

```diff
diff --git a/crank_amd/_lib.py b/crank_amd/_lib.py
--- a/crank_amd/_lib.py
+++ b/crank_amd/_lib.py
@@ -32,6 +32,14 @@
         ("spk_lcf0_mean", c_void_p), ("spk_lcf0_std", c_void_p), ("raw", c_void_p), ("raw_start", c_void_p),
         ("fftl", c_int), ("hop", c_int),
     ]
+
+
+ADAM_MAX_BLOCKS = 4
+
+
+class AdamBlock(ctypes.Structure):
+    _fields_ = [("params", c_void_p), ("grads", c_void_p), ("exp_avg", c_void_p), ("exp_avg_sq", c_void_p),
+                ("n", c_longlong), ("lr_dev", c_void_p), ("step_dev", c_void_p)]
 
 
 P, I, LL, ULL, F, D = c_void_p, c_int, c_longlong, c_ulonglong, c_float, c_double
@@ -47,9 +55,11 @@
     "crk_net_scratch_bytes": (LL, [P, I, I]),
     "crk_debug_alloc_count": (LL, []),
     "crk_debug_net_paths": (I, [P, I, I]),
+    "crk_debug_net_partials": (LL, [P, I, I, P, LL, P]),
     "crk_seed_next": (I, [P, P, P]),
     "crk_nets_wnorm_bwd": (I, [I, P, P]),
     "crk_nets_prepare": (I, [I, P, P, ULL, P, P]),
+    "crk_nets_prepare_models": (I, [I, P, P, P, I, P, P]),
     "crk_net_forward": (I, [P, P, ULL, P, I, P, I, P, I, P, I, I, I, ULL, P]),
     "crk_net_backward": (I, [P, P, ULL, P, P, I, P, I, P, I, P, I, F, P, I, P, I, I, I, ULL, P]),
     "crk_net_backward_scaled": (I, [P, P, ULL, P, P, I, P, I, P, I, P, I, F, P, I, P, I, I, I, ULL, P, P, P]),
@@ -91,6 +101,7 @@
     "crk_stft_loss_fwd": (I, [P, I, P, I, I, I, I, I, I, I, P, F, F, I, P, P, P]),
     "crk_stft_loss_bwd": (I, [P, I, P, I, I, I, I, I, I, I, P, F, F, P, P, I, P]),
     "crk_adam_step": (I, [P, P, P, P, LL, P, P, F, F, F, I, P]),
+    "crk_adam_step_multi": (I, [I, ctypes.POINTER(AdamBlock), F, F, F, I, P]),
     "crk_radam_step": (I, [P, P, P, P, LL, P, P, D, D, D, I, P]),
     "crk_lamb_step": (I, [P, P, P, P, P, P, I, P, I, P, P, P, P, D, D, D, I, P]),
     "crk_lamb_tile": (I, []),
diff --git a/crank_amd/config.py b/crank_amd/config.py
--- a/crank_amd/config.py
+++ b/crank_amd/config.py
@@ -15,7 +15,7 @@
         precision=_get("CRANK_AMD_PRECISION", "bf16"),
         lib_path=_get("CRANK_AMD_LIB") or None,
         default_yaml=_get("CRANK_DEFAULT_YAML") or None,
-        overlap_c=int(_get("CRANK_AMD_OVERLAP_C", "1") or 0),
+        overlap_c=int(_get("CRANK_AMD_OVERLAP_C", "3") or 0),
         separate_ce=_flag("CRANK_AMD_SEPARATE_CE", False),
         separate_commit=_flag("CRANK_AMD_SEPARATE_COMMIT", False),
         recon_dense=_flag("CRANK_AMD_RECON_DENSE", False),
diff --git a/crank_amd/csrc/conv_kernels.h b/crank_amd/csrc/conv_kernels.h
--- a/crank_amd/csrc/conv_kernels.h
+++ b/crank_amd/csrc/conv_kernels.h
@@ -146,7 +146,7 @@
   int B, T, cpg, G;
 };
 struct PwMP { PwP q[CRK_MAX_NETS_PW]; int first[CRK_MAX_NETS_PW + 1]; int n; };
-int launch_pstack_wgrad_multi(const PwMP& m, int total_layers, int max_G, int max_wa, int max_wb, int max_tiles, double flops,
+int launch_pstack_wgrad_multi(const PwMP& m, int total_blocks, int max_wa, int max_wb, int max_tiles, double flops,
                               double bytes, hipStream_t s);
 int pstack_wgrad_supported(int ca, int cb, int wa, int wb, int k, int dil);
 int launch_pstack_wgrad(const PwP& p, int nlayers, int max_wa, int max_wb, bool precise, double flops, hipStream_t s, int max_tiles = 0);
@@ -242,9 +242,10 @@
   uint16_t *whi, *wlo;
   int n_ents, first;
 };
-struct NetRefs { NetRef r[CRK_MAX_NETS]; int n; float* bump; };
+#define CRK_MAX_BUMPS 4
+struct NetRefs { NetRef r[CRK_MAX_NETS]; int n; float* bump[CRK_MAX_BUMPS]; int n_bump; };
 int launch_weight_prep_multi(const NetRefs& R, int total_entries, int nmax, hipStream_t s);
-int launch_step_bump(float* step, hipStream_t s);
+int launch_step_bump(float* const* steps, int n, hipStream_t s);
 int launch_wnorm_bwd_multi(const NetRefs& R, int total_entries, hipStream_t s);
 int launch_weight_prep(const ConvEntry* d_entries, int n_entries, int nmax, const float* params, uint16_t* wprep_hi,
                        uint16_t* wprep_lo, float* norms, hipStream_t s);
diff --git a/crank_amd/csrc/conv_kernels.hip b/crank_amd/csrc/conv_kernels.hip
--- a/crank_amd/csrc/conv_kernels.hip
+++ b/crank_amd/csrc/conv_kernels.hip
@@ -746,12 +746,24 @@
   extern __shared__ unsigned wp_ws[];
   const NetRef& q = R.r[net_of_block(R, blockIdx.x)];
   const ConvEntry e = q.ents[blockIdx.x - q.first];
-  if (R.bump && blockIdx.x == 0 && blockIdx.y == 0 && threadIdx.x == 0) R.bump[0] += 1.f;
+  if (blockIdx.x == 0 && blockIdx.y == 0) {
+#pragma unroll
+    for (int i = 0; i < CRK_MAX_BUMPS; i++)
+      if (i < R.n_bump && (int)threadIdx.x == i) R.bump[i][0] += 1.f;
+  }
   weight_prep_band<BAND>(e, blockIdx.y, q.params, q.whi, q.wlo, q.norms, wp_ws);
 }
-__global__ void step_bump_kernel(float* step) { step[0] += 1.f; }
-int launch_step_bump(float* step, hipStream_t s) {
-  hipLaunchKernelGGL(step_bump_kernel, dim3(1), dim3(1), 0, s, step);
+struct StepBumps { float* p[CRK_MAX_BUMPS]; };
+__global__ void step_bump_kernel(const StepBumps b) {
+#pragma unroll
+  for (int i = 0; i < CRK_MAX_BUMPS; i++)
+    if ((int)threadIdx.x == i) b.p[i][0] += 1.f;
+}
+int launch_step_bump(float* const* steps, int n, hipStream_t s) {
+  if (n < 1 || n > CRK_MAX_BUMPS) return CRK_ERR_ARG;
+  StepBumps b;
+  for (int i = 0; i < CRK_MAX_BUMPS; i++) b.p[i] = steps[i < n ? i : 0];
+  hipLaunchKernelGGL(step_bump_kernel, dim3(1), dim3(n), 0, s, b);
   CRK_CHECK_LAUNCH();
   return CRK_OK;
 }
diff --git a/crank_amd/csrc/loss_kernels.hip b/crank_amd/csrc/loss_kernels.hip
--- a/crank_amd/csrc/loss_kernels.hip
+++ b/crank_amd/csrc/loss_kernels.hip
@@ -1089,6 +1089,56 @@
   return CRK_OK;
 }
 
+#define CRK_ADAM_MAX_BLOCKS 4
+struct crk_adam_block {
+  float *params, *grads, *exp_avg, *exp_avg_sq;
+  long long n;
+  const float* lr_dev;
+  float* step_dev;
+};
+struct AdamBlocks { crk_adam_block b[CRK_ADAM_MAX_BLOCKS]; int first[CRK_ADAM_MAX_BLOCKS + 1]; int n; };
+template <bool CLEAR>
+__global__ __launch_bounds__(256) void adam_multi_kernel(const AdamBlocks A, float beta1, float beta2, float eps) {
+  int r = 0;
+  while (r + 1 < A.n && (int)blockIdx.x >= A.first[r + 1]) r++;
+  const crk_adam_block& q = A.b[r];
+  const AdamCoef c = adam_coef(q.lr_dev, q.step_dev, beta1, beta2, eps);
+  const long nb = A.first[r + 1] - A.first[r], n = (long)q.n;
+  for (long i = (long)((int)blockIdx.x - A.first[r]) * 256 + threadIdx.x; i < n; i += nb * 256)
+    adam_elem<CLEAR>(q.params, q.grads, q.exp_avg, q.exp_avg_sq, i, c);
+}
+struct AdamBumps { float* p[CRK_ADAM_MAX_BLOCKS]; };
+__global__ void adam_bump_multi_kernel(const AdamBumps b) {
+#pragma unroll
+  for (int i = 0; i < CRK_ADAM_MAX_BLOCKS; i++)
+    if ((int)threadIdx.x == i) b.p[i][0] += 1.f;
+}
+extern "C" int crk_adam_step_multi(int n_blocks, const crk_adam_block* blocks, float beta1, float beta2, float eps,
+                                   int clear_grads, void* stream) {
+  if (n_blocks < 1 || n_blocks > CRK_ADAM_MAX_BLOCKS || !blocks) return CRK_ERR_ARG;
+  AdamBlocks A{};
+  AdamBumps B;
+  int total = 0;
+  for (int i = 0; i < n_blocks; i++) {
+    const crk_adam_block& q = blocks[i];
+    if (!q.params || !q.grads || !q.exp_avg || !q.exp_avg_sq || !q.lr_dev || !q.step_dev || q.n < 0) return CRK_ERR_ARG;
+    for (int j = 0; j < i; j++) if (blocks[j].step_dev == q.step_dev) return CRK_ERR_ARG;
+    long b = ((long)q.n + 255) / 256;
+    if (b > 2048) b = 2048;
+    if (b < 1) b = 1;
+    A.b[i] = q; A.first[i] = total;
+    total += (int)b;
+  }
+  A.first[n_blocks] = total; A.n = n_blocks;
+  for (int i = 0; i < CRK_ADAM_MAX_BLOCKS; i++) B.p[i] = blocks[i < n_blocks ? i : 0].step_dev;
+  hipStream_t s = (hipStream_t)stream;
+  if (clear_grads & 1) hipLaunchKernelGGL(adam_multi_kernel<true>, dim3(total), dim3(256), 0, s, A, beta1, beta2, eps);
+  else hipLaunchKernelGGL(adam_multi_kernel<false>, dim3(total), dim3(256), 0, s, A, beta1, beta2, eps);
+  if (!(clear_grads & 2)) hipLaunchKernelGGL(adam_bump_multi_kernel, dim3(1), dim3(n_blocks), 0, s, B);
+  CRK_CHECK_LAUNCH();
+  return CRK_OK;
+}
+
 struct RAdamCoef { float step_size; bool rect; };
 __device__ __forceinline__ RAdamCoef radam_coef(const float* lr_dev, const float* step_dev, double b1, double b2) {
   const double t = (double)step_dev[0] + 1.0;
diff --git a/crank_amd/csrc/net.hip b/crank_amd/csrc/net.hip
--- a/crank_amd/csrc/net.hip
+++ b/crank_amd/csrc/net.hip
@@ -958,6 +958,15 @@
   return (int)r.gen_split | (int)r.x3f << 1 | (int)r.disc_split << 2 | (int)(n->d.kind == 2 && r.fused) << 3;
 }
 
+extern "C" long long crk_debug_net_partials(void* h, int B, int T, float* out, long long cap, void* stream) {
+  Net* n = (Net*)h;
+  const Shape* r = n ? find_shape(n, B, T) : nullptr;
+  if (!r || !n->partials || cap < 0 || (cap > 0 && !out)) return -1;
+  const long long cnt = r->q.need_p < cap ? r->q.need_p : cap;
+  if (cnt > 0 && hipMemcpyAsync(out, n->partials, sizeof(float) * cnt, hipMemcpyDeviceToDevice, (hipStream_t)stream) != hipSuccess) return -1;
+  return r->q.need_p;
+}
+
 static WgradP base_wgrad(const Net* n, int B, int T) {
   WgradP w;
   memset(&w, 0, sizeof(w));
@@ -1066,8 +1075,10 @@
     RUN(pstack2_plan(p, Tb.t[1]));
     RUN(launch_pstack2(p, ps_flops(Tb.t[1], p.L, N), a.s));
   } else RUN(pstack_go(r, 1, p, k.precise, a.s));
-  if (k.want_w) RUN(launch_plain_wgrad(r, plain_wgrad_params(n, r, g16, f16), k.precise, a.s));
-  return CRK_OK;
+  if (!k.want_w) return CRK_OK;
+  const PwP wp = plain_wgrad_params(n, r, g16, f16);
+  if (k.defer_wn && !k.precise) { n->pw_shape = r; n->pw_params = wp; return CRK_OK; }
+  return launch_plain_wgrad(r, wp, k.precise, a.s);
 }
 static int bwd_chain_layers(Net* n, const Shape* r, const Call& k, const BwdIo& a) {
   const crk_net_desc& d = n->d;
@@ -1349,32 +1360,35 @@
 }
 
 static int flush_plain_wgrads(int n_nets, void* const* nets, hipStream_t s) {
-  {
-    PwMP M; memset(&M, 0, sizeof(M));
-    int layers = 0, max_G = 0, max_wa = 0, max_wb = 0, max_tiles = 0;
-    double flops = 0.0, bytes = 0.0;
-    for (int i = 0; i < n_nets; i++) {
-      Net* n = (Net*)nets[i];
-      if (!n) return CRK_ERR_ARG;
-      const Shape* r = n->pw_shape;
-      if (!r) continue;
-      if (M.n == CRK_MAX_NETS_PW) { RUN(flush_pending_plain_wgrad(n, s)); continue; }
-      const PsTables& Tb = r->ps;
-      M.q[M.n] = n->pw_params;
-      M.first[M.n] = layers;
-      layers += Tb.nw;
-      if (n->pw_params.G > max_G) max_G = n->pw_params.G;
-      if (Tb.max_wa > max_wa) max_wa = Tb.max_wa;
-      if (Tb.max_wb > max_wb) max_wb = Tb.max_wb;
-      if (Tb.max_tiles > max_tiles) max_tiles = Tb.max_tiles;
-      flops += Tb.wflops_per_frame * r->B * r->T;
-      bytes += 2.0 * (Tb.max_wa + Tb.max_wb) * (double)r->B * r->T * Tb.nw;
-      M.n++;
-      n->pw_shape = nullptr;
-    }
-    M.first[M.n] = layers;
-    if (M.n > 0) RUN(launch_pstack_wgrad_multi(M, layers, max_G, max_wa, max_wb, max_tiles, flops, bytes, s));
-  }
+  PwMP M; memset(&M, 0, sizeof(M));
+  int blocks = 0, max_wa = 0, max_wb = 0, max_tiles = 0, pending = 0;
+  double flops = 0.0, bytes = 0.0;
+  Net* only = nullptr;
+  for (int i = 0; i < n_nets; i++) {
+    Net* n = (Net*)nets[i];
+    if (!n) return CRK_ERR_ARG;
+    if (n->pw_shape) { pending++; only = n; }
+  }
+  if (pending == 1 && only->d.kind == 2) return flush_pending_plain_wgrad(only, s);
+  for (int i = 0; i < n_nets; i++) {
+    Net* n = (Net*)nets[i];
+    const Shape* r = n->pw_shape;
+    if (!r) continue;
+    if (M.n == CRK_MAX_NETS_PW) { RUN(flush_pending_plain_wgrad(n, s)); continue; }
+    const PsTables& Tb = r->ps;
+    M.q[M.n] = n->pw_params;
+    M.first[M.n] = blocks;
+    blocks += Tb.nw * n->pw_params.G;
+    if (Tb.max_wa > max_wa) max_wa = Tb.max_wa;
+    if (Tb.max_wb > max_wb) max_wb = Tb.max_wb;
+    if (Tb.max_tiles > max_tiles) max_tiles = Tb.max_tiles;
+    flops += Tb.wflops_per_frame * r->B * r->T;
+    bytes += 2.0 * (Tb.max_wa + Tb.max_wb) * (double)r->B * r->T * Tb.nw;
+    M.n++;
+    n->pw_shape = nullptr;
+  }
+  M.first[M.n] = blocks;
+  if (M.n > 0) RUN(launch_pstack_wgrad_multi(M, blocks, max_wa, max_wb, max_tiles, flops, bytes, s));
   return CRK_OK;
 }
 extern "C" int crk_nets_wnorm_bwd(int n_nets, void* const* nets, void* stream) {
@@ -1401,25 +1415,35 @@
   return launch_wnorm_bwd_multi(R, total, s);
 }
 
-extern "C" int crk_nets_prepare(int n_nets, void* const* nets, const float* const* params, unsigned long long version,
-                                float* bump_step, void* stream) {
-  if (n_nets < 0 || (n_nets > 0 && (!nets || !params))) return CRK_ERR_ARG;
+extern "C" int crk_nets_prepare_models(int n_nets, void* const* nets, const float* const* params,
+                                       const unsigned long long* versions, int n_bumps, float* const* bump_steps,
+                                       void* stream) {
+  if (n_nets < 0 || (n_nets > 0 && (!nets || !params || !versions))) return CRK_ERR_ARG;
+  if (n_bumps < 0 || n_bumps > CRK_MAX_BUMPS || (n_bumps > 0 && !bump_steps)) return CRK_ERR_ARG;
+  for (int i = 0; i < n_bumps; i++) if (!bump_steps[i]) return CRK_ERR_ARG;
+  for (int i = 0; i < n_nets; i++) if (!nets[i] || !params[i]) return CRK_ERR_ARG;
   hipStream_t s = (hipStream_t)stream;
   NetRefs R; memset(&R, 0, sizeof(R));
   int total = 0, nmax = 1;
   for (int i = 0; i < n_nets; i++) {
     Net* n = (Net*)nets[i];
-    if (!n || !params[i]) return CRK_ERR_ARG;
-    if (n->prepared_version == version && n->prepared_params == params[i]) continue;
+    if (n->prepared_version == versions[i] && n->prepared_params == params[i]) continue;
     if (net_nmax(n) > nmax) nmax = net_nmax(n);
-    if (R.n == CRK_MAX_NETS) { RUN(ensure_prepared(n, params[i], version, s)); continue; }
+    if (R.n == CRK_MAX_NETS) { RUN(ensure_prepared(n, params[i], versions[i], s)); continue; }
     NetRef& q = R.r[R.n++];
     q.ents = n->d_ents; q.n_ents = (int)n->ents.size(); q.first = total;
     q.params = params[i]; q.whi = n->whi; q.wlo = n->wlo; q.norms = n->norms;
     total += q.n_ents;
-    n->prepared_version = version; n->prepared_params = params[i];
-  }
-  if (R.n == 0) return bump_step ? launch_step_bump(bump_step, s) : CRK_OK;
-  R.bump = bump_step;
+    n->prepared_version = versions[i]; n->prepared_params = params[i];
+  }
+  if (R.n == 0) return n_bumps ? launch_step_bump(bump_steps, n_bumps, s) : CRK_OK;
+  for (int i = 0; i < n_bumps; i++) R.bump[i] = bump_steps[i];
+  R.n_bump = n_bumps;
   return launch_weight_prep_multi(R, total, nmax, s);
 }
+extern "C" int crk_nets_prepare(int n_nets, void* const* nets, const float* const* params, unsigned long long version,
+                                float* bump_step, void* stream) {
+  if (n_nets < 0 || (n_nets > 0 && (!nets || !params))) return CRK_ERR_ARG;
+  const std::vector<unsigned long long> versions((size_t)n_nets + 1, version);
+  return crk_nets_prepare_models(n_nets, nets, params, versions.data(), bump_step ? 1 : 0, &bump_step, stream);
+}
diff --git a/crank_amd/csrc/pstack_kernels.hip b/crank_amd/csrc/pstack_kernels.hip
--- a/crank_amd/csrc/pstack_kernels.hip
+++ b/crank_amd/csrc/pstack_kernels.hip
@@ -675,30 +675,49 @@
   }
   pstack_wgrad_body<PRECISE, MAXT>(p, blockIdx.x, blockIdx.y, smem);
 }
+__device__ __forceinline__ int pw_net_of_block(const PwMP& m, int bx) {
+  int r = 0;
+  while (r + 1 < m.n && bx >= m.first[r + 1]) r++;
+  return r;
+}
 template <int MAXT>
 __global__ __launch_bounds__(256) void pstack_wgrad_multi_kernel(const PwMP m) {
   extern __shared__ __attribute__((aligned(16))) unsigned char smem[];
-  int r = 0;
-  while (r + 1 < m.n && (int)blockIdx.y >= m.first[r + 1]) r++;
+  const int r = pw_net_of_block(m, blockIdx.x);
   const PwP& p = m.q[r];
-  if ((int)blockIdx.x >= p.G) return;
-  pstack_wgrad_body<false, MAXT>(p, blockIdx.x, blockIdx.y - m.first[r], smem);
-}
-int launch_pstack_wgrad_multi(const PwMP& m, int total_layers, int max_G, int max_wa, int max_wb, int max_tiles, double flops,
+  const int local = (int)blockIdx.x - m.first[r], layer = local / p.G;
+  pstack_wgrad_body<false, MAXT>(p, local - layer * p.G, layer, smem);
+}
+__global__ __launch_bounds__(256) void pstack_wgrad_multi_wide_kernel(const PwMP m) {
+  extern __shared__ __attribute__((aligned(16))) unsigned char smem[];
+  const int r = pw_net_of_block(m, blockIdx.x);
+  const PwP& p = m.q[r];
+  const int local = (int)blockIdx.x - m.first[r], layer = local / p.G, g = local - layer * p.G;
+  const PwLayer& Y = p.layers[layer];
+  const int nct = (Y.ca + 31) >> 5;
+  const int per = (nct * ((Y.cb + 31) >> 5) * Y.k + 3) >> 2;
+  const bool sa = (4 % nct) == 0;
+  if (per <= 3) { if (sa) pstack_wgrad_body<false, 3, true>(p, g, layer, smem); else pstack_wgrad_body<false, 3>(p, g, layer, smem); return; }
+  if (per <= 5) { if (sa) pstack_wgrad_body<false, 5, true>(p, g, layer, smem); else pstack_wgrad_body<false, 5>(p, g, layer, smem); return; }
+  if (per <= 6) { if (sa) pstack_wgrad_body<false, 6, true>(p, g, layer, smem); else pstack_wgrad_body<false, 6>(p, g, layer, smem); return; }
+  if (sa) pstack_wgrad_body<false, PW_MAXT, true>(p, g, layer, smem); else pstack_wgrad_body<false, PW_MAXT>(p, g, layer, smem);
+}
+int launch_pstack_wgrad_multi(const PwMP& m, int total_blocks, int max_wa, int max_wb, int max_tiles, double flops,
                               double bytes, hipStream_t s) {
   const int RA = ((max_wa + 31) & ~31) * 2 + 64, RB = ((max_wb + 31) & ~31) * 2 + 64;
   const int lds = PW_FR * RA + (PW_FR + PW_SPAN) * RB;
+  if (total_blocks < 1) return CRK_ERR_ARG;
   static bool attr_set = false;
   if (!attr_set) {
     if (hipFuncSetAttribute((const void*)pstack_wgrad_multi_kernel<2>, hipFuncAttributeMaxDynamicSharedMemorySize, 160 * 1024) != hipSuccess ||
-        hipFuncSetAttribute((const void*)pstack_wgrad_multi_kernel<PW_MAXT>, hipFuncAttributeMaxDynamicSharedMemorySize, 160 * 1024) != hipSuccess)
+        hipFuncSetAttribute((const void*)pstack_wgrad_multi_wide_kernel, hipFuncAttributeMaxDynamicSharedMemorySize, 160 * 1024) != hipSuccess)
       return CRK_ERR_HIP;
     attr_set = true;
   }
   conv_prof_bytes(6, bytes);
   conv_prof_begin(6, flops, s);
-  if (max_tiles <= 8) hipLaunchKernelGGL(pstack_wgrad_multi_kernel<2>, dim3(max_G, total_layers), dim3(256), lds, s, m);
-  else hipLaunchKernelGGL(pstack_wgrad_multi_kernel<PW_MAXT>, dim3(max_G, total_layers), dim3(256), lds, s, m);
+  if (max_tiles <= 8) hipLaunchKernelGGL(pstack_wgrad_multi_kernel<2>, dim3(total_blocks), dim3(256), lds, s, m);
+  else hipLaunchKernelGGL(pstack_wgrad_multi_wide_kernel, dim3(total_blocks), dim3(256), lds, s, m);
   conv_prof_end(6, s);
   CRK_CHECK_LAUNCH();
   return CRK_OK;
diff --git a/crank_amd/net/trainer/trainer_vqvae.py b/crank_amd/net/trainer/trainer_vqvae.py
--- a/crank_amd/net/trainer/trainer_vqvae.py
+++ b/crank_amd/net/trainer/trainer_vqvae.py
@@ -64,9 +64,12 @@
             loss = self.forward_spkradv(batch, loss, phase=phase)
         else:
             self._defer_G_tail = False
-            loss = self.forward_spkradv(batch, loss, phase=phase)
-            if side is None:
-                loss = self.forward_spkrclassifier(batch, loss, phase=phase)
+            if side is None and self._speaker_updates_joinable(batch, phase):
+                loss = self.update_speaker_nets(batch, loss, phase=phase)
+            else:
+                loss = self.forward_spkradv(batch, loss, phase=phase)
+                if side is None:
+                    loss = self.forward_spkrclassifier(batch, loss, phase=phase)
         if self._C_tail is not None:
             tail, self._C_tail = self._C_tail, None
             tail()
@@ -85,11 +88,58 @@
     def _classifier_stream(self, batch, phase):
         if not (phase == "train" and self.conf["use_spkr_classifier"] and not parallel.is_dist()
                 and self._classifier_is_independent() and batch["in_feats"].is_cuda
-                and cfg.overlap_c != 0):
+                and cfg.overlap_c not in (0, 3)):
             return None
         if getattr(self, "_c_stream", None) is None:
             self._c_stream = torch.cuda.Stream(device=batch["in_feats"].device)
         return self._c_stream
+
+    def _speaker_updates_joinable(self, batch, phase):
+        if not (cfg.overlap_c == 3 and phase == "train" and not parallel.is_dist() and batch["in_feats"].is_cuda
+                and self.conf["use_spkradv_training"] and self.conf["use_spkr_classifier"]
+                and getattr(self, "group_stack_maintenance", True)):
+            return False
+        from .utils import FlatAdam
+        opts = [self.optimizer.get(k) for k in ("SPKRADV", "C")]
+        if any(type(o) is not FlatAdam or getattr(o.step, "__func__", None) is not FlatAdam.step or o.grad_reduce_fn is not None
+               for o in opts):
+            return False
+        if any(self.conf["optim"][k]["clip_grad_norm"] != 0 for k in ("SPKRADV", "C")):
+            return False
+        if any(not getattr(self.model[k], "_nets", None) for k in ("SPKRADV", "C")):
+            return False
+        a, b = opts
+        return a.betas == b.betas and a.eps == b.eps and a.clear_grads == b.clear_grads
+
+    def update_speaker_nets(self, batch, loss, phase="train"):
+        from ... import ops
+        from .utils import flat_adam_step_many
+
+        loss = self.forward_spkradv(batch, loss, phase=phase, step=False)
+        loss = self.forward_spkrclassifier(batch, loss, phase=phase, step=False)
+        names = ("C", "SPKRADV")
+        models = [self.model[k] for k in names]
+        for k in names:
+            self.optimizer[k].zero_grad()
+        for m in models:
+            m.defer_wnorm = True
+        try:
+            for k in ("SPKRADV", "C"):
+                torch.autograd.backward(loss[k], _one_like(loss[k]))
+        finally:
+            for m in models:
+                m.defer_wnorm = False
+            if any(getattr(m, "_wnorm_pending", False) for m in models):
+                ops.nets_wnorm_bwd([n for m in models for n, _ in m._nets])
+            for m in models:
+                m._wnorm_pending = False
+                m._keepalive = []
+        opts = [self.optimizer[k] for k in names]
+        flat_adam_step_many(opts, defer_bump=True)
+        ops.nets_prepare_models([n for m in models for n, _ in m._nets],
+                                [m.flat.data_ptr() + 4 * b for m in models for _, b in m._nets],
+                                [m.version for m in models for _ in m._nets], [o.step_dev for o in opts])
+        return loss
 
     def _main_update(self, batch, loss, phase):
         return self.forward_cycle(batch, loss, phase) if self.cycle_flag else self.forward_vqvae(batch, loss, phase)
@@ -246,7 +296,7 @@
         self._discard_grads("C", False)
         return loss
 
-    def forward_spkradv(self, batch, loss, phase="train"):
+    def forward_spkradv(self, batch, loss, phase="train", step=True):
         if not self.conf["use_spkradv_training"]:
             return loss
         enc_h, dec_h, spkrvec = self._cond(batch)
@@ -259,16 +309,16 @@
         encoded = [e[:, er:] for e in outputs["encoded_unmod"]] if er else outputs["encoded_unmod"]
         with torch.set_grad_enabled(grad_on):
             loss["SPKRADV"] = _scaled(self.conf["alpha"]["ce"], self._spkradv_ce(encoded, batch["org_h"][:, er:], detach=True))
-            if phase == "train":
+            if phase == "train" and step:
                 self.step_model(loss, model="SPKRADV")
         return loss
 
-    def forward_spkrclassifier(self, batch, loss, phase="train"):
+    def forward_spkrclassifier(self, batch, loss, phase="train", step=True):
         if not self.conf["use_spkr_classifier"]:
             return loss
         loss["C_real"] = self._classify_ce(batch["in_feats"], batch["org_h"])
         loss.add("C", self.conf["alpha"]["ce"], loss["C_real"])
-        if phase == "train":
+        if phase == "train" and step:
             self.step_model(loss, model="C")
         return loss
 
diff --git a/crank_amd/net/trainer/utils.py b/crank_amd/net/trainer/utils.py
--- a/crank_amd/net/trainer/utils.py
+++ b/crank_amd/net/trainer/utils.py
@@ -84,6 +84,21 @@
     def _update(self, m, defer_bump):
         ops.adam_step(m.flat.data, m.grad_flat, self.exp_avg, self.exp_avg_sq, self.lr_dev, self.step_dev,
                       self.betas[0], self.betas[1], self.eps, clear_grads=self.clear_grads, defer_bump=defer_bump)
+
+
+def flat_adam_step_many(opts, defer_bump=False):
+    first = opts[0]
+    assert all(type(o) is FlatAdam and o.betas == first.betas and o.eps == first.eps and o.clear_grads == first.clear_grads
+               for o in opts)
+    for o in opts:
+        o.reduce_grads()
+        o._reduced = False
+    ops.adam_step_multi([(o.model.flat.data, o.model.grad_flat, o.exp_avg, o.exp_avg_sq, o.lr_dev, o.step_dev) for o in opts],
+                        first.betas[0], first.betas[1], first.eps, clear_grads=first.clear_grads, defer_bump=defer_bump)
+    for o in opts:
+        if o.clear_grads:
+            o.model.grads_clean = True
+        o.model.touch(by_optimizer=True)
 
 
 class FlatRAdam(FlatAdam):
diff --git a/crank_amd/ops.py b/crank_amd/ops.py
--- a/crank_amd/ops.py
+++ b/crank_amd/ops.py
@@ -294,6 +294,15 @@
     check(_lib.lib().crk_nets_wnorm_bwd(len(nets), arr, stream_ptr()), "crk_nets_wnorm_bwd")
 
 
+def nets_prepare_models(nets, param_ptrs, versions, bump_steps=()):
+    n = len(nets)
+    arr = (ctypes.c_void_p * n)(*[x.handle for x in nets])
+    par = (ctypes.c_void_p * n)(*param_ptrs)
+    ver = (ctypes.c_ulonglong * n)(*versions)
+    bumps = (ctypes.c_void_p * max(len(bump_steps), 1))(*[ptr(b) for b in bump_steps])
+    check(_lib.lib().crk_nets_prepare_models(n, arr, par, ver, len(bump_steps), bumps, stream_ptr()), "crk_nets_prepare_models")
+
+
 def nets_prepare(nets, param_ptrs, version, bump_step=None):
     arr = (ctypes.c_void_p * len(nets))(*[n.handle for n in nets])
     par = (ctypes.c_void_p * len(nets))(*param_ptrs)
@@ -1015,6 +1024,15 @@
                                    stream_ptr()), "crk_adam_step")
 
 
+def adam_step_multi(blocks, beta1=0.9, beta2=0.999, eps=1e-8, clear_grads=False, defer_bump=False):
+    rec = (_lib.AdamBlock * len(blocks))()
+    for r, (flat, grad, m, v, lr_dev, step_dev) in zip(rec, blocks):
+        r.params, r.grads, r.exp_avg, r.exp_avg_sq = ptr(flat), ptr(grad), ptr(m), ptr(v)
+        r.n, r.lr_dev, r.step_dev = flat.numel(), ptr(lr_dev), ptr(step_dev)
+    check(_lib.lib().crk_adam_step_multi(len(blocks), rec, beta1, beta2, eps, (1 if clear_grads else 0) | (2 if defer_bump else 0),
+                                         stream_ptr()), "crk_adam_step_multi")
+
+
 def radam_step(flat, grad, exp_avg, exp_avg_sq, lr_dev, step_dev, beta1=0.9, beta2=0.999, eps=1e-8, clear_grads=False,
                defer_bump=False):
     check(_lib.lib().crk_radam_step(ptr(flat), ptr(grad), ptr(exp_avg), ptr(exp_avg_sq), flat.numel(), ptr(lr_dev),
diff --git a/include/crank_hip.h b/include/crank_hip.h
--- a/include/crank_hip.h
+++ b/include/crank_hip.h
@@ -59,6 +59,8 @@
 int crk_nets_wnorm_bwd(int n_nets, void* const* nets, void* stream);
 int crk_nets_prepare(int n_nets, void* const* nets, const float* const* params, unsigned long long version,
                      float* bump_step, void* stream);
+int crk_nets_prepare_models(int n_nets, void* const* nets, const float* const* params, const unsigned long long* versions,
+                            int n_bumps, float* const* bump_steps, void* stream);
 
 int crk_vq_forward(const float* x, int ldx, const float* codebook, int N, int D, int K, long long* idx, float* e,
                    int lde, float* qx, int ldq, void* stream);
@@ -143,6 +145,15 @@
 
 int crk_adam_step(float* params, float* grads, float* exp_avg, float* exp_avg_sq, long long n, const float* lr_dev,
                   float* step_dev, float beta1, float beta2, float eps, int clear_grads, void* stream);
+#define CRK_ADAM_MAX_BLOCKS 4
+typedef struct crk_adam_block {
+  float *params, *grads, *exp_avg, *exp_avg_sq;
+  long long n;
+  const float* lr_dev;
+  float* step_dev;
+} crk_adam_block;
+int crk_adam_step_multi(int n_blocks, const crk_adam_block* blocks, float beta1, float beta2, float eps, int clear_grads,
+                        void* stream);
 int crk_radam_step(float* params, float* grads, float* exp_avg, float* exp_avg_sq, long long n, const float* lr_dev,
                    float* step_dev, double beta1, double beta2, double eps, int clear_grads, void* stream);
 int crk_lamb_step(float* params, float* grads, float* exp_avg, float* exp_avg_sq, float* upd, const int* tiles, int n_tiles,
@@ -296,6 +307,7 @@
 long long crk_debug_alloc_count(void);
 
 int crk_debug_net_paths(void* net, int B, int T);
+long long crk_debug_net_partials(void* net, int B, int T, float* out, long long cap, void* stream);
 
 const char* crk_version(void);
 
```

Result: faster. 22.44 million frames/s, median of 6 (+1.4%).
